# dmjovan/NeRF-Workspaces-Explorer

Hardware: AMD Instinct MI355X
Metric: ray-samples/sec (800x800, 192 samples, 8x256 MLP) (higher is better)
Workload: dtype f16x3 (split-fp16 MFMA, fp32 accumulate)

## Files before the change

include/nwe.h:

```cpp
#ifndef NWE_H
#define NWE_H

#include <stdint.h>

#ifdef __cplusplus
extern "C" {
#endif

typedef struct nwe_ctx nwe_ctx;

enum {
    NWE_OK = 0,
    NWE_ERR_INVALID = 1,
    NWE_ERR_UNSUPPORTED = 2,
    NWE_ERR_HIP = 3,
    NWE_ERR_STATE = 4
};

enum { NWE_NET_COARSE = 0, NWE_NET_FINE = 1 };

enum {
    NWE_PREC_F16X3 = 0,
    NWE_PREC_F16X1 = 1,
    NWE_PREC_F32 = 2
// ... 63 lines not shown
    float *raw;
    float *sigma;
    uint32_t *flags;
} nwe_point_outputs;

int nwe_query_points(nwe_ctx *ctx, int which, const float *points_dev, int64_t n_points, const float *dirs_dev,
                     int64_t points_per_dir, int precision, const nwe_point_outputs *out, void *stream);
float nwe_last_query_ms(nwe_ctx *ctx);
int nwe_debug_set_query_steps(nwe_ctx *ctx, int steps);

int nwe_to8b(nwe_ctx *ctx, const float *rgb_dev, uint8_t *out_dev, int64_t n, void *stream);

int64_t nwe_flops_per_eval(const nwe_ctx *ctx, int which);

float nwe_last_kernel_ms(nwe_ctx *ctx);

int nwe_last_launch_parts(nwe_ctx *ctx, float *ms2, int64_t *rays2);


int64_t nwe_packed_bytes(const nwe_ctx *ctx, int which);
int nwe_packed_copy(const nwe_ctx *ctx, int which, void *host_dst, int64_t bytes);
int64_t nwe_packed_bias_count(const nwe_ctx *ctx, int which);
int nwe_packed_bias_copy(const nwe_ctx *ctx, int which, float *host_dst, int64_t count);
float nwe_packed_scale(const nwe_ctx *ctx, int which);
int nwe_packed_colour_finite(const nwe_ctx *ctx, int which);

int nwe_debug_set_fine_depths(nwe_ctx *ctx, const float *z_dev);

int nwe_debug_set_raw(nwe_ctx *ctx, const float *raw_coarse_dev, const float *raw_fine_dev);
int nwe_debug_set_coarse_weights(nwe_ctx *ctx, const float *weights_dev);

int nwe_debug_set_fold(nwe_ctx *ctx, int on);

int nwe_set_white_background(nwe_ctx *ctx, int on);

int nwe_set_early_termination(nwe_ctx *ctx, float min_transmittance);
float nwe_get_early_termination(const nwe_ctx *ctx);

int nwe_set_shared_coarse(nwe_ctx *ctx, int k);
int nwe_get_shared_coarse(const nwe_ctx *ctx);

int nwe_set_separate_passes(nwe_ctx *ctx, int on);
int nwe_get_separate_passes(const nwe_ctx *ctx);

int nwe_set_occupancy(nwe_ctx *ctx, const float *lo, const float *hi, const int *res, const uint32_t *bits, int bits_on_device);
int nwe_clear_occupancy(nwe_ctx *ctx);
int nwe_get_occupancy(const nwe_ctx *ctx, float *lo, float *hi, int *res, float *inv, int64_t *occupied_cells);
int nwe_occupancy_copy(const nwe_ctx *ctx, uint32_t *host_words, int64_t n_words);
int nwe_build_occupancy(nwe_ctx *ctx, const float *lo, const float *hi, const int *res, int probes, float threshold, int dilate,
                        int precision, void *stream);

int nwe_set_coarse_grid(nwe_ctx *ctx, const float *lo, const float *hi, const int *res, const float *sigma, int on_device);
int nwe_clear_coarse_grid(nwe_ctx *ctx);
int nwe_get_coarse_grid(const nwe_ctx *ctx, float *lo, float *hi, int *res, float *inv);
int nwe_coarse_grid_copy(nwe_ctx *ctx, float *host_values, int64_t n_values);
int nwe_bake_coarse_grid(nwe_ctx *ctx, const float *lo, const float *hi, const int *res, int precision, void *stream);
int nwe_coarse_grid_weights(nwe_ctx *ctx, const float *c2w, int n_poses, int H, int W, float fx, float fy, float cx, float cy,
                            float near, float far, int row_begin, int row_end, float *sigma_out_dev, float *weights_out_dev,
                            void *stream);

typedef struct nwe_grid_outputs {
    uint64_t struct_bytes;
    float *rgb;
    float *depth;
    float *acc;
    float *weights_coarse;
    float *z_fine;
    float *raw_fine;
    uint32_t *flags;
} nwe_grid_outputs;
int nwe_set_radiance_grid(nwe_ctx *ctx, const float *lo, const float *hi, const int *res, const float *raw, int on_device);
int nwe_clear_radiance_grid(nwe_ctx *ctx);
int nwe_get_radiance_grid(const nwe_ctx *ctx, float *lo, float *hi, int *res, float *inv);
int nwe_radiance_grid_copy(nwe_ctx *ctx, float *host_values, int64_t n_values);
int nwe_bake_radiance_grid(nwe_ctx *ctx, const float *lo, const float *hi, const int *res, int which, const float *dir3_host,
                           int precision, void *stream);
int nwe_render_grid(nwe_ctx *ctx, const float *c2w, int n_poses, int H, int W, float fx, float fy, float cx, float cy, float near,
                    float far, int row_begin, int row_end, const nwe_grid_outputs *out, void *stream);
float nwe_last_grid_ms(nwe_ctx *ctx);

typedef struct nwe_sparse_outputs {
    uint64_t struct_bytes;
    float *rgb;
    float *depth;
    float *acc;
    float *weights_coarse;
    float *z_fine;
    float *weights_grid;
    uint8_t *selected;
    float *raw_fine;
    uint32_t *flags;
} nwe_sparse_outputs;
int nwe_render_sparse(nwe_ctx *ctx, const float *c2w, int n_poses, int H, int W, float fx, float fy, float cx, float cy, float near,
                      float far, int row_begin, int row_end, int which, int precision, float min_weight, int dilate,
                      const nwe_sparse_outputs *out, void *stream);
int nwe_debug_set_sparse_chunk(nwe_ctx *ctx, int rays);
float nwe_last_sparse_ms(nwe_ctx *ctx);
int nwe_last_sparse_samples(nwe_ctx *ctx, int64_t *out2);

int nwe_last_coarse_launch(nwe_ctx *ctx, float *ms, int64_t *rays);

int nwe_last_ray_evaluations(nwe_ctx *ctx, int64_t *out2);

int nwe_set_train_tables(nwe_ctx *ctx, const float *t_rand_dev, const float *noise_coarse_dev, const float *noise_fine_dev,
                         const float *u_sorted_dev);

int nwe_debug_set_decomposition(nwe_ctx *ctx, int mode);
int nwe_debug_last_plan(const nwe_ctx *ctx);

int nwe_debug_set_work_queue(nwe_ctx *ctx, int mode);
int nwe_debug_get_work_queue(const nwe_ctx *ctx);
int nwe_debug_get_work_queue_backfill(const nwe_ctx *ctx);
unsigned nwe_debug_queue_grid(unsigned items);
#define NWE_PLAN_HOOK_COARSE_WEIGHTS 1u
#define NWE_PLAN_HOOK_OTHER 2u
typedef struct nwe_plan_stage {
    int32_t active;
    int32_t role;
    int64_t n_rays;
    int32_t n_importance;
    int32_t net;
    int32_t variant;
    int32_t plan;
    int32_t n_launches;
    int32_t fork;
    int64_t ray_first[2], rays[2];
    int32_t split[2];
    uint32_t items[2], grid[2];
    int32_t tail;
    uint32_t tail_items;
} nwe_plan_stage;
typedef struct nwe_plan_report {
    uint64_t struct_bytes;
    int32_t separate, share, full;
    int32_t coarse_launch;
    int32_t may_queue, need_side;
    int32_t need_evals, coarse_flags;
    int32_t share_k, reserved;
    int64_t table_elems;
    int64_t evals_full, evals_run;
    int64_t share_rays;
    nwe_plan_stage coarse, main;
} nwe_plan_report;
int nwe_debug_plan(nwe_ctx *ctx, int n_poses, int H, int W, int row_begin, int row_end, int64_t n_rays, const nwe_outputs *out,
                   unsigned hooks, int precision, int cus, nwe_plan_report *report);
int nwe_debug_last_queue(nwe_ctx *ctx, unsigned *items2, unsigned *grid2, unsigned *taken2, int *side_stream);
int nwe_debug_get_work_queue_tail(const nwe_ctx *ctx);
int nwe_debug_last_tail(nwe_ctx *ctx, unsigned *stolen);
int nwe_debug_last_tail_rest(nwe_ctx *ctx, unsigned *rendered);

int nwe_debug_set_colour_skip(nwe_ctx *ctx, int mode);
int nwe_debug_get_colour_skip(const nwe_ctx *ctx);

int nwe_debug_set_packet_blocks(nwe_ctx *ctx, int on);
int nwe_debug_last_packet_blocks(const nwe_ctx *ctx);
int nwe_debug_packet_pixels(int64_t first, int64_t n, int W, int32_t *pixels);

int nwe_debug_set_stamps(nwe_ctx *ctx, unsigned long long *per_wave_dev);

int nwe_selftest(nwe_ctx *ctx, int32_t *report8);

#ifdef __cplusplus
}
#endif
#endif
```

nerf-workspaces-explorer_amd/_lib.py:

```python
from __future__ import annotations

import ctypes as C
import os

_HERE = os.path.dirname(os.path.abspath(__file__))
LIB_PATH = os.environ.get("NWE_LIB") or os.path.join(_HERE, "libnwe_hip.so")

NWE_OK, NWE_ERR_INVALID, NWE_ERR_UNSUPPORTED, NWE_ERR_HIP, NWE_ERR_STATE = 0, 1, 2, 3, 4
NET_COARSE, NET_FINE = 0, 1
PREC_F16X3, PREC_F16X1, PREC_F32 = 0, 1, 2
PRECISIONS = {"f16x3": PREC_F16X3, "f16x1": PREC_F16X1, "f32": PREC_F32}

OUTPUT_FIELDS = ("rgb", "depth", "acc", "disp", "z_std", "rgb_coarse", "depth_coarse", "acc_coarse", "disp_coarse",
                 "raw_coarse", "raw_fine", "z_fine", "weights_coarse", "sample_cond", "sample_amp", "sample_switch", "feat_map", "flags")

SYMBOLS = ("nwe_create", "nwe_destroy", "nwe_last_error", "nwe_set_network", "nwe_set_sampling", "nwe_render", "nwe_render_tiled",
           "nwe_create_rays", "nwe_render_rays", "nwe_to8b", "nwe_flops_per_eval", "nwe_last_kernel_ms", "nwe_packed_bytes",
           "nwe_packed_copy", "nwe_packed_bias_count", "nwe_packed_bias_copy", "nwe_packed_scale",
           "nwe_debug_set_fine_depths", "nwe_debug_set_raw", "nwe_debug_set_coarse_weights", "nwe_debug_set_fold", "nwe_set_train_tables", "nwe_set_white_background", "nwe_debug_set_decomposition", "nwe_debug_last_plan", "nwe_debug_set_stamps", "nwe_selftest",
           "nwe_last_warning", "nwe_debug_peer_access", "nwe_set_network_no_view_dirs", "nwe_last_launch_parts",
           "nwe_set_early_termination", "nwe_get_early_termination", "nwe_last_ray_evaluations",
           "nwe_set_shared_coarse", "nwe_get_shared_coarse", "nwe_last_coarse_launch",
           "nwe_set_separate_passes", "nwe_get_separate_passes",
           "nwe_debug_set_work_queue", "nwe_debug_get_work_queue", "nwe_debug_get_work_queue_backfill", "nwe_debug_queue_grid", "nwe_debug_last_queue",
           "nwe_debug_get_work_queue_tail", "nwe_debug_last_tail", "nwe_debug_last_tail_rest",
           "nwe_query_points", "nwe_last_query_ms", "nwe_debug_set_query_steps",
           "nwe_packed_colour_finite", "nwe_debug_set_colour_skip", "nwe_debug_get_colour_skip", "nwe_debug_plan",
           "nwe_set_occupancy", "nwe_clear_occupancy", "nwe_get_occupancy", "nwe_occupancy_copy", "nwe_build_occupancy",
           "nwe_set_coarse_grid", "nwe_clear_coarse_grid", "nwe_get_coarse_grid", "nwe_coarse_grid_copy", "nwe_bake_coarse_grid",
           "nwe_coarse_grid_weights",
           "nwe_set_radiance_grid", "nwe_clear_radiance_grid", "nwe_get_radiance_grid", "nwe_radiance_grid_copy", "nwe_bake_radiance_grid",
           "nwe_render_grid", "nwe_last_grid_ms",
           "nwe_render_sparse", "nwe_debug_set_sparse_chunk", "nwe_last_sparse_ms", "nwe_last_sparse_samples",
           "nwe_debug_set_packet_blocks", "nwe_debug_last_packet_blocks", "nwe_debug_packet_pixels")


class Outputs(C.Structure):
    _fields_ = [("struct_bytes", C.c_uint64)] + [(name, C.c_void_p) for name in OUTPUT_FIELDS]

    def __init__(self, **kw):
        super().__init__(struct_bytes=C.sizeof(Outputs), **kw)


POINT_OUTPUT_FIELDS = ("raw", "sigma", "flags")
NWE_FLAG_RAW = 1 << 8


class PointOutputs(C.Structure):
    _fields_ = [("struct_bytes", C.c_uint64)] + [(name, C.c_void_p) for name in POINT_OUTPUT_FIELDS]

    def __init__(self, **kw):
        super().__init__(struct_bytes=C.sizeof(PointOutputs), **kw)


GRID_OUTPUT_FIELDS = ("rgb", "depth", "acc", "weights_coarse", "z_fine", "raw_fine", "flags")


class GridOutputs(C.Structure):
    _fields_ = [("struct_bytes", C.c_uint64)] + [(name, C.c_void_p) for name in GRID_OUTPUT_FIELDS]

    def __init__(self, **kw):
        super().__init__(struct_bytes=C.sizeof(GridOutputs), **kw)


SPARSE_OUTPUT_FIELDS = ("rgb", "depth", "acc", "weights_coarse", "z_fine", "weights_grid", "selected", "raw_fine", "flags")


class SparseOutputs(C.Structure):
    _fields_ = [("struct_bytes", C.c_uint64)] + [(name, C.c_void_p) for name in SPARSE_OUTPUT_FIELDS]

    def __init__(self, **kw):
        super().__init__(struct_bytes=C.sizeof(SparseOutputs), **kw)


PLAN_HOOK_COARSE_WEIGHTS, PLAN_HOOK_OTHER = 1, 2


class PlanStage(C.Structure):
    _fields_ = [("active", C.c_int32), ("role", C.c_int32), ("n_rays", C.c_int64), ("n_importance", C.c_int32), ("net", C.c_int32),
                ("variant", C.c_int32), ("plan", C.c_int32), ("n_launches", C.c_int32), ("fork", C.c_int32),
                ("ray_first", C.c_int64 * 2), ("rays", C.c_int64 * 2), ("split", C.c_int32 * 2), ("items", C.c_uint32 * 2),
                ("grid", C.c_uint32 * 2), ("tail", C.c_int32), ("tail_items", C.c_uint32)]


class PlanReport(C.Structure):
    _fields_ = [("struct_bytes", C.c_uint64)] + [(name, C.c_int32) for name in (
        "separate", "share", "full", "coarse_launch", "may_queue", "need_side", "need_evals", "coarse_flags", "share_k", "reserved")] + [
        (name, C.c_int64) for name in ("table_elems", "evals_full", "evals_run", "share_rays")] + [("coarse", PlanStage), ("main", PlanStage)]

    def __init__(self):
        super().__init__(struct_bytes=C.sizeof(PlanReport))


_lib = None


def build_hint() -> str:
    return ("build it with `make -C nerf-workspaces-explorer_amd/csrc` (or `python -c 'import __graft_entry__ as g; "
            "g.build()'`); the render path has no CPU or torch fallback")


def load() -> C.CDLL:
    global _lib
    if _lib is not None:
        return _lib
    if not os.path.exists(LIB_PATH):
        raise RuntimeError(f"HIP extension {LIB_PATH} is missing: {build_hint()}")
    lib = C.CDLL(LIB_PATH)
    P, I, F, I64 = C.c_void_p, C.c_int, C.c_float, C.c_int64
    sig = {
        "nwe_create": (I, [C.POINTER(P), I]),
        "nwe_destroy": (None, [P]),
        "nwe_last_error": (C.c_char_p, [P]),
        "nwe_set_network": (I, [P, I, I, I, I, I, I, C.POINTER(P), C.POINTER(P)]),
        "nwe_set_network_no_view_dirs": (I, [P, I, I, I, I, I, I, C.POINTER(P), C.POINTER(P)]),
        "nwe_set_sampling": (I, [P, P, P, I, P, I]),
        "nwe_render": (I, [P, P, I, I, I, F, F, F, F, F, F, I, I, I, C.POINTER(Outputs), P]),
        "nwe_render_tiled": (I, [C.POINTER(P), I, P, I, I, I, F, F, F, F, F, F, I, P, P, P, P, P]),
        "nwe_create_rays": (I, [P, P, I, I, I, F, F, F, F, F, F, I, I, P, P]),
        "nwe_render_rays": (I, [P, P, I64, I, C.POINTER(Outputs), P]),
        "nwe_to8b": (I, [P, P, P, I64, P]),
        "nwe_flops_per_eval": (I64, [P, I]),
        "nwe_last_kernel_ms": (F, [P]),
        "nwe_last_launch_parts": (I, [P, C.POINTER(F), C.POINTER(I64)]),
        "nwe_packed_bytes": (I64, [P, I]),
        "nwe_packed_copy": (I, [P, I, P, I64]),
        "nwe_packed_bias_count": (I64, [P, I]),
        "nwe_packed_bias_copy": (I, [P, I, P, I64]),
        "nwe_packed_scale": (F, [P, I]),
        "nwe_debug_set_fine_depths": (I, [P, P]),
        "nwe_debug_set_raw": (I, [P, P, P]),
        "nwe_debug_set_coarse_weights": (I, [P, P]),
        "nwe_debug_set_fold": (I, [P, I]),
        "nwe_set_train_tables": (I, [P, P, P, P, P]),
        "nwe_set_white_background": (I, [P, I]),
        "nwe_debug_set_decomposition": (I, [P, I]),
        "nwe_debug_last_plan": (I, [P]),
        "nwe_debug_set_stamps": (I, [P, P]),
        "nwe_selftest": (I, [P, C.POINTER(C.c_int32)]),
        "nwe_last_warning": (C.c_char_p, [P]),
        "nwe_debug_peer_access": (I, [P, P]),
        "nwe_set_early_termination": (I, [P, F]),
        "nwe_get_early_termination": (F, [P]),
        "nwe_last_ray_evaluations": (I, [P, C.POINTER(I64)]),
        "nwe_set_shared_coarse": (I, [P, I]),
        "nwe_get_shared_coarse": (I, [P]),
        "nwe_last_coarse_launch": (I, [P, C.POINTER(F), C.POINTER(I64)]),
        "nwe_set_separate_passes": (I, [P, I]),
        "nwe_get_separate_passes": (I, [P]),
        "nwe_debug_set_work_queue": (I, [P, I]),
        "nwe_debug_get_work_queue": (I, [P]),
        "nwe_debug_get_work_queue_backfill": (I, [P]),
        "nwe_debug_queue_grid": (C.c_uint, [C.c_uint]),
        "nwe_debug_last_queue": (I, [P, C.POINTER(C.c_uint), C.POINTER(C.c_uint), C.POINTER(C.c_uint), C.POINTER(I)]),
        "nwe_debug_get_work_queue_tail": (I, [P]),
        "nwe_debug_last_tail": (I, [P, C.POINTER(C.c_uint)]),
        "nwe_debug_last_tail_rest": (I, [P, C.POINTER(C.c_uint)]),
        "nwe_query_points": (I, [P, I, P, I64, P, I64, I, C.POINTER(PointOutputs), P]),
        "nwe_last_query_ms": (F, [P]),
        "nwe_debug_set_query_steps": (I, [P, I]),
        "nwe_packed_colour_finite": (I, [P, I]),
        "nwe_debug_set_colour_skip": (I, [P, I]),
        "nwe_debug_get_colour_skip": (I, [P]),
        "nwe_debug_set_packet_blocks": (I, [P, I]),
        "nwe_debug_last_packet_blocks": (I, [P]),
        "nwe_debug_packet_pixels": (I, [I64, I64, I, P]),
        "nwe_debug_plan": (I, [P, I, I, I, I, I, I64, C.POINTER(Outputs), C.c_uint, I, I, C.POINTER(PlanReport)]),
        "nwe_set_occupancy": (I, [P, C.POINTER(F), C.POINTER(F), C.POINTER(I), P, I]),
        "nwe_clear_occupancy": (I, [P]),
        "nwe_get_occupancy": (I, [P, C.POINTER(F), C.POINTER(F), C.POINTER(I), C.POINTER(F), C.POINTER(I64)]),
        "nwe_occupancy_copy": (I, [P, P, I64]),
        "nwe_build_occupancy": (I, [P, C.POINTER(F), C.POINTER(F), C.POINTER(I), I, F, I, I, P]),
        "nwe_set_coarse_grid": (I, [P, C.POINTER(F), C.POINTER(F), C.POINTER(I), P, I]),
        "nwe_clear_coarse_grid": (I, [P]),
        "nwe_get_coarse_grid": (I, [P, C.POINTER(F), C.POINTER(F), C.POINTER(I), C.POINTER(F)]),
        "nwe_coarse_grid_copy": (I, [P, P, I64]),
        "nwe_bake_coarse_grid": (I, [P, C.POINTER(F), C.POINTER(F), C.POINTER(I), I, P]),
        "nwe_coarse_grid_weights": (I, [P, P, I, I, I, F, F, F, F, F, F, I, I, P, P, P]),
        "nwe_set_radiance_grid": (I, [P, C.POINTER(F), C.POINTER(F), C.POINTER(I), P, I]),
        "nwe_clear_radiance_grid": (I, [P]),
        "nwe_get_radiance_grid": (I, [P, C.POINTER(F), C.POINTER(F), C.POINTER(I), C.POINTER(F)]),
        "nwe_radiance_grid_copy": (I, [P, P, I64]),
        "nwe_bake_radiance_grid": (I, [P, C.POINTER(F), C.POINTER(F), C.POINTER(I), I, C.POINTER(F), I, P]),
        "nwe_render_grid": (I, [P, P, I, I, I, F, F, F, F, F, F, I, I, C.POINTER(GridOutputs), P]),
        "nwe_last_grid_ms": (F, [P]),
        "nwe_render_sparse": (I, [P, P, I, I, I, F, F, F, F, F, F, I, I, I, I, F, I, C.POINTER(SparseOutputs), P]),
        "nwe_debug_set_sparse_chunk": (I, [P, I]),
        "nwe_last_sparse_ms": (F, [P]),
        "nwe_last_sparse_samples": (I, [P, C.POINTER(I64)]),
    }
    for name, (res, args) in sig.items():
        fn = getattr(lib, name)
        fn.restype, fn.argtypes = res, args
    _lib = lib
    return lib
```

nerf-workspaces-explorer_amd/csrc/nwe_abi.hip:

```cpp
#include <algorithm>
#include <cmath>
#include <cstdlib>
#include <cstring>
#include <string>
#include <vector>

#include "nwe_check.h"
#include "nwe_host.h"
#include "nwe_pack.h"

using namespace nwe;

namespace {

template <class H, hipError_t (*Release)(H)>
struct Owned {
    H h = nullptr;
    Owned() = default;
    Owned(Owned&& o) noexcept : h(o.h) { o.h = nullptr; }
    ~Owned() { reset(); }
    void reset() { if (h) (void)Release(h); h = nullptr; }
    operator H() const { return h; }
};
using Event = Owned<hipEvent_t, hipEventDestroy>;
using Stream = Owned<hipStream_t, hipStreamDestroy>;

template <class T>
struct DevBuf {
    Owned<void*, hipFree> mem;
    size_t cap = 0;
    T* get() const { return static_cast<T*>(mem.h); }
    hipError_t reserve(size_t count) {
        if (count <= cap) return hipSuccess;
        mem.reset(); cap = 0;
        const hipError_t e = hipMalloc(&mem.h, count * sizeof(T));
        if (e == hipSuccess) cap = count; else mem.h = nullptr;
        return e;
    }
};

struct NetState : NetDesc {
    int64_t flops = 0;
    Packed p;
    NetF32 f32 = {};
    NetMfma mf = {};
    DevBuf<float> d_blob, d_bias;
    DevBuf<uint8_t> d_stream;
};

struct Slot {
    DevBuf<float> poses;
    Event ev0, ev1;
    bool used = false;
};

struct RenderSlot : Slot {
    Event ev_mid;
    bool has_mid = false;
    int64_t rays_first = 0, rays_total = 0;
    DevBuf<unsigned long long> evals;
    bool term = false;
    int64_t evals_full = 0;
    DevBuf<float> share_w;
    DevBuf<uint32_t> coarse_flags;
    Event ev_share;
    bool has_share = false;
    int64_t share_rays = 0, evals_run = 0;
    DevBuf<unsigned> queue;
    Stream side;
    Event ev_fork, ev_join;
    unsigned q_items[2] = {0, 0}, q_grid[2] = {0, 0};
    bool side_used = false;
    unsigned tail_items = 0;
};

struct GridBox {
    float lo[3] = {}, hi[3] = {}, inv[3] = {};
    int res[3] = {};
    int64_t cells = 0;
    GridBox() = default;
    GridBox(const float* lo_, const float* hi_, const int* res_) : cells((int64_t)res_[0] * res_[1] * res_[2]) {
        for (int i = 0; i < 3; ++i) {
            lo[i] = lo_[i]; hi[i] = hi_[i]; res[i] = res_[i];
            inv[i] = (float)res[i] / (hi[i] - lo[i]);
        }
    }
    void read(float* lo_, float* hi_, int* res_, float* inv_) const {
        for (int i = 0; i < 3; ++i) {
            if (lo_) lo_[i] = lo[i];
            if (hi_) hi_[i] = hi[i];
            if (res_) res_[i] = res[i];
            if (inv_) inv_[i] = inv[i];
        }
    }
};

struct Occupancy {
    bool set = false;
    GridBox box;
    int64_t occupied = 0;
    std::vector<uint32_t> bits;
};

struct CoarseGridState {
    bool set = false;
    GridBox box;
    std::vector<float> host;
};

using RadianceGridState = CoarseGridState;

thread_local std::string g_create_error;

}

struct nwe_ctx {
    int device = -1;
    bool host_only = false;
    int cus = 256;
    NetState net[2];
    DevBuf<float> d_t;
    int ns = 0, ni = 0;
    static constexpr int kSlots = 4;
    RenderSlot slots[kSlots];
    Slot rays_slot;
    int next_slot = 0, last_slot = -1;
    Slot query_slots[kSlots];
    int next_query = 0, last_query = -1;
    int query_steps = 0;
    Slot grid_slots[kSlots];
    int next_grid = 0, last_grid = -1;
    Slot sparse_slots[kSlots];
    int next_sparse = 0, last_sparse = -1;
    int64_t sparse_selected = 0, sparse_total = 0;
    int sparse_chunk = 0;
    DevBuf<uint8_t> d_sparse_scratch;
    Owned<void*, hipHostFree> sparse_word;
    const float* dbg_z_fine = nullptr;
    const float *dbg_raw_c = nullptr, *dbg_raw_f = nullptr, *dbg_w = nullptr;
    int fold = 1;
    DevBuf<float> tile_buf;
    DevBuf<uint32_t> tile_flags;
    Stream tile_stream;
    Event tile_done;
    Event frame_ready;
    DevBuf<uint32_t> flag_parts;
    int peer_access = -2;
    std::string warn;
    int white_bkgd = 0;
    float min_trans = 0.f;
    int share_k = 1;
    int separate = 0;
    Occupancy occ;
    DevBuf<uint32_t> d_occ_bits, d_occ_tmp;
    DevBuf<OccGrid> d_occ;
    DevBuf<float> d_occ_scratch;
    CoarseGridState cgrid;
    DevBuf<float> d_cgrid;
    RadianceGridState rgrid;
    DevBuf<float> d_rgrid;
    int decomposition = -1;
    int work_queue = -1;
    bool backfill = true;
    bool tail = true;
    int colour_skip = 1;
    int last_plan = -1;
    bool packet_blocks = true;
    int last_packet_blocks = 0;
    unsigned long long* stamps = nullptr;
    const float *trn_t = nullptr, *trn_nc = nullptr, *trn_nf = nullptr, *trn_u = nullptr;
    std::string err;
};

namespace {

int fail(nwe_ctx* c, int code, const std::string& msg) {
    if (c) c->err = msg; else g_create_error = msg;
    return code;
}

struct DeviceGuard {
    int prev = -1;
    DeviceGuard() { if (hipGetDevice(&prev) != hipSuccess) { prev = -1; (void)hipGetLastError(); } }
    ~DeviceGuard() { if (prev >= 0) (void)hipSetDevice(prev); }
    DeviceGuard(const DeviceGuard&) = delete;
    DeviceGuard& operator=(const DeviceGuard&) = delete;
};

#define HIPCHK(ctx, expr)                                                                                       \
    do {                                                                                                        \
        const hipError_t e_ = (expr);                                                                           \
        if (e_ != hipSuccess) return fail(ctx, NWE_ERR_HIP, std::string(#expr) + ": " + hipGetErrorString(e_)); \
    } while (0)
#define ON_DEVICE(c) DeviceGuard guard; HIPCHK(c, hipSetDevice(c->device))
#define TRY(call) do { const int rc_ = (call); if (rc_) return rc_; } while (0)
#define CHECK(c, check) do { const Refusal r_ = (check); if (r_) return fail(c, r_.code, r_.text); } while (0)

ContextDesc describe_context(const nwe_ctx* c) {
    ContextDesc d;
    for (int i = 0; i < 2; ++i) d.net[i] = c->net[i];
    d.ns = c->ns; d.ni = c->ni; d.host_only = c->host_only;
    d.min_trans = c->min_trans; d.share_k = c->share_k; d.separate = c->separate != 0;
    d.occ.set = c->occ.set; d.cgrid.set = c->cgrid.set; d.rgrid.set = c->rgrid.set;
    for (int i = 0; i < 3; ++i) { d.occ.res[i] = c->occ.box.res[i]; d.cgrid.res[i] = c->cgrid.box.res[i]; d.rgrid.res[i] = c->rgrid.box.res[i]; }
    d.stamps = c->stamps != nullptr;
    d.decomposition = c->decomposition; d.queue_mode = c->work_queue;
    d.backfill = c->backfill; d.tail = c->tail; d.packet_blocks = c->packet_blocks;
    return d;
}
struct MaybeContext {
    ContextDesc d;
    const ContextDesc* p = nullptr;
    explicit MaybeContext(const nwe_ctx* c) { if (c) { d = describe_context(c); p = &d; } }
};

__global__ void to8b_kernel(const float* __restrict__ x, uint8_t* __restrict__ y, int64_t n) {
    const int64_t i = (int64_t)blockIdx.x * blockDim.x + threadIdx.x;
    if (i < n) {
        const float v = 255.f * fminf(fmaxf(x[i], 0.f), 1.f);
        y[i] = (uint8_t)(int)v;
    }
}

__global__ void or_flags_kernel(const uint32_t* __restrict__ parts, int n, uint32_t* __restrict__ out) {
    uint32_t f = 0;
    for (int i = 0; i < n; ++i) f |= parts[i];
    if (f) atomicOr(out, f);
}

__global__ void or_masked_flags_kernel(const uint32_t* __restrict__ word, uint32_t mask, uint32_t* __restrict__ out) {
    const uint32_t f = *word & mask;
    if (f) atomicOr(out, f);
}

__global__ void create_rays_kernel(RenderArgs a, float* __restrict__ out) {
    const int64_t i = (int64_t)blockIdx.x * blockDim.x + threadIdx.x;
    if (i >= a.n_rays) return;
    const Ray r = load_ray(a, i);
    float* o = out + i * 11;
    o[0] = r.ox; o[1] = r.oy; o[2] = r.oz; o[3] = r.dx; o[4] = r.dy; o[5] = r.dz;
    o[6] = r.near; o[7] = r.far; o[8] = r.vx; o[9] = r.vy; o[10] = r.vz;
}

int prepare_slot(nwe_ctx* c, Slot& s) {
    if (!s.ev0)
        for (Event* e : {&s.ev0, &s.ev1}) HIPCHK(c, hipEventCreate(&e->h));
    if (s.used) HIPCHK(c, hipEventSynchronize(s.ev1));
    s.used = false;
    return NWE_OK;
}
int prepare_slot(nwe_ctx* c, RenderSlot& s) {
    if (!s.ev_mid)
        for (Event* e : {&s.ev_mid, &s.ev_share}) HIPCHK(c, hipEventCreate(&e->h));
    s.has_mid = s.has_share = false;
    return prepare_slot(c, static_cast<Slot&>(s));
}

template <class Queue>
int record_launch(nwe_ctx* c, Slot& s, hipStream_t stream, Queue&& queue) {
    HIPCHK(c, hipEventRecord(s.ev0, stream));
    TRY(queue());
    HIPCHK(c, hipGetLastError());
    HIPCHK(c, hipEventRecord(s.ev1, stream));
    s.used = true;
    return NWE_OK;
}

int wait_for_launches(nwe_ctx* c) {
    for (RenderSlot& s : c->slots)
        if (s.used) HIPCHK(c, hipEventSynchronize(s.ev1));
    if (c->rays_slot.used) HIPCHK(c, hipEventSynchronize(c->rays_slot.ev1));
    for (Slot& s : c->query_slots)
        if (s.used) HIPCHK(c, hipEventSynchronize(s.ev1));
    for (Slot& s : c->grid_slots)
        if (s.used) HIPCHK(c, hipEventSynchronize(s.ev1));
    for (Slot& s : c->sparse_slots)
        if (s.used) HIPCHK(c, hipEventSynchronize(s.ev1));
    return NWE_OK;
}

struct HookReset {
    nwe_ctx* c;
    ~HookReset() {
        if (!c) return;
        c->dbg_z_fine = c->dbg_raw_c = c->dbg_raw_f = c->dbg_w = nullptr;
        c->trn_t = c->trn_nc = c->trn_nf = c->trn_u = nullptr;
    }
};

int upload_poses(nwe_ctx* c, Slot& s, const float* c2w, int n_poses, hipStream_t stream) {
    HIPCHK(c, s.poses.reserve((size_t)std::max(n_poses, 64) * 16));
    HIPCHK(c, hipMemcpyAsync(s.poses.get(), c2w, (size_t)n_poses * 16 * sizeof(float), hipMemcpyHostToDevice, stream));
    return NWE_OK;
}

RenderArgs camera_args(const Camera& m, const float* poses_dev) {
    RenderArgs a = {};
    a.poses = poses_dev;
    a.H = m.H; a.W = m.W; a.row_begin = m.row_begin; a.rows = m.row_end - m.row_begin;
    a.n_rays = (int64_t)m.n_poses * a.rows * m.W;
    a.fx = m.fx; a.fy = m.fy; a.cx = m.cx; a.cy = m.cy; a.near = m.near; a.far = m.far;
    return a;
}

#ifdef NWE_STAMPS
constexpr bool kStampedBuild = true;
#else
constexpr bool kStampedBuild = false;
#endif

void context_args(const nwe_ctx* ctx, RenderArgs& a) {
    a.white_bkgd = ctx->white_bkgd;
    a.t_vals = ctx->d_t.get();
    if (a.t_vals) { a.omt_vals = a.t_vals + kMaxSamples; a.u_vals = a.omt_vals + kMaxSamples; }
    a.n_samples = ctx->ns; a.n_importance = ctx->ni;
    a.stamps = ctx->stamps;
    a.min_trans = ctx->min_trans;
}

CallDesc describe_call(const ContextDesc& ctx, const RenderArgs& a, int precision) {
    CallDesc d;
    d.n_rays = a.n_rays;
    RenderArgs consumer = a;
    consumer.share = kShareConsumer | ctx.share_k << 8;
    d.n_rep = share_n_rep(consumer, share_grid(consumer));
    d.n_samples = a.n_samples; d.n_importance = a.n_importance;
    d.mfma = precision != NWE_PREC_F32;
    d.term = a.min_trans > 0.f;
    d.occ = ctx.occ.set;
    d.share_k = ctx.share_k; d.separate = ctx.separate;
    d.baked = ctx.cgrid.set;
    RenderArgs unstamped = a;
    unstamped.stamps = nullptr;
    d.lean = mfma_is_lean(unstamped); d.stamps = a.stamps != nullptr; d.stamped_build = kStampedBuild;
    d.w_in = a.w_in != nullptr;
    d.want_weights_coarse = a.out.weights_coarse != nullptr; d.want_flags = a.out.flags != nullptr;
    for (int i = 0; i < 2; ++i)
        for (int v = 0; v < kVariants; ++v) d.built[i][v] = ctx.net[i].set && ctx.net[i].mfma_ok && ctx.net[i].built[v];
    d.decomposition = ctx.decomposition; d.queue_mode = ctx.queue_mode;
    d.backfill = ctx.backfill; d.tail = ctx.tail;
    if (!a.rays) { d.rows = a.rows; d.width = a.W; }
    d.packet_blocks = ctx.packet_blocks;
    return d;
}

int provide(nwe_ctx* ctx, RenderSlot& slot, const CallPlan& p, hipStream_t stream) {
    if (p.need_evals) {
        HIPCHK(ctx, slot.evals.reserve(1));
        HIPCHK(ctx, hipMemsetAsync(slot.evals.get(), 0, sizeof(unsigned long long), stream));
    }
    HIPCHK(ctx, slot.share_w.reserve((size_t)p.table_elems));
    if (p.coarse_flags) {
        HIPCHK(ctx, slot.coarse_flags.reserve(1));
        HIPCHK(ctx, hipMemsetAsync(slot.coarse_flags.get(), 0, sizeof(uint32_t), stream));
    }
    if (p.may_queue) HIPCHK(ctx, slot.queue.reserve(4));
    for (RenderSlot& s : ctx->slots) {
        if (!p.need_side || s.side) continue;
        int least = 0, greatest = 0;
        HIPCHK(ctx, hipDeviceGetStreamPriorityRange(&least, &greatest));
        HIPCHK(ctx, hipStreamCreateWithPriority(&s.side.h, hipStreamNonBlocking, least));
        for (Event* e : {&s.ev_fork, &s.ev_join}) HIPCHK(ctx, hipEventCreateWithFlags(&e->h, hipEventDisableTiming));
    }
    return NWE_OK;
}

RenderArgs stage_args(const CallPlan& p, const RenderSlot& slot, RenderArgs& a) {
    RenderArgs prod = {};
    if (p.need_evals) a.evals = slot.evals.get();
    if (p.main.role != kShareOff) a.share = p.main.role | p.share_k << 8;
    if (p.share) a.share_w = slot.share_w.get();
    if (p.coarse.active) {
        prod = a;
        prod.share = p.coarse.role | p.share_k << 8; prod.n_rays = p.coarse.n_rays; prod.n_importance = p.coarse.n_importance;
        prod.out = {};
        if (p.share) {
            if (p.share_k == 1) prod.out.flags = a.out.flags;
        } else {
            float* table = a.out.weights_coarse ? a.out.weights_coarse : slot.share_w.get();
            prod.z_fine_in = prod.raw_in_f = prod.noise_f = prod.u_rand = nullptr;
            prod.out.struct_bytes = a.out.struct_bytes;
            prod.out.raw_coarse = a.out.raw_coarse; prod.out.weights_coarse = table;
            prod.out.rgb_coarse = a.out.rgb_coarse; prod.out.depth_coarse = a.out.depth_coarse;
            prod.out.acc_coarse = a.out.acc_coarse; prod.out.disp_coarse = a.out.disp_coarse;
            if (p.coarse_flags) prod.out.flags = slot.coarse_flags.get();
            a.w_in = table;
        }
    }
    if (p.full) {
        a.raw_in_c = a.noise_c = nullptr;
        a.out.raw_coarse = a.out.weights_coarse = a.out.rgb_coarse = a.out.depth_coarse = a.out.acc_coarse = a.out.disp_coarse = nullptr;
    }
    return prod;
}

CoarseGrid coarse_grid_args(const nwe_ctx* ctx) {
    CoarseGrid g = {};
    const GridBox& box = ctx->cgrid.box;
    for (int i = 0; i < 3; ++i) { g.lo[i] = box.lo[i]; g.inv[i] = box.inv[i]; g.res[i] = box.res[i]; }
    g.sigma = ctx->d_cgrid.get();
    return g;
}

int launch(nwe_ctx* ctx, const ContextDesc& desc, RenderSlot& slot, RenderArgs& a, int precision, hipStream_t stream) {
    context_args(ctx, a);
    if (a.n_rays <= 0) return NWE_OK;
    const CallPlan p = plan_call(describe_call(desc, a, precision), ctx->cus);
    const bool mfma = precision != NWE_PREC_F32, three_pass = precision == NWE_PREC_F16X3;
    TRY(provide(ctx, slot, p, stream));
    const RenderArgs prod = stage_args(p, slot, a);
    if (p.occ) a.occ = ctx->d_occ.get();
    if (p.blocks) a.ray_cols |= kPacketBlocksBit;
    ctx->last_packet_blocks = p.blocks ? 1 : 0;
    const NetState &nc = ctx->net[0], &nf = ctx->net[ctx->ni > 0 ? 1 : 0];
    const auto with_skip = [&](const NetState& n) {
        NetMfma m = n.mf;
        m.colour_skip = ctx->colour_skip == 2 || (ctx->colour_skip == 1 && n.p.colour_finite) ? 1 : 0;
        return m;
    };
    const NetMfma mf[2] = {with_skip(nc), with_skip(nf)};
    const auto run = [&](const StagePlan& s, const RenderArgs& args, const LaunchResources& res, LaunchReport* report) {
        if (!mfma) {
            if (p.occ) launch_render_f32_occ(args, nc.f32, nf.f32, stream); else launch_render_f32(args, nc.f32, nf.f32, stream);
            return true;
        }
        return launch_render_mfma(args, mf[s.net < 0 ? 0 : s.net], mf[s.net < 0 ? 1 : s.net], three_pass, s.pass, res, stream, report);
    };
    const int rc = record_launch(ctx, slot, stream, [&]() -> int {
        const PassPlan& pass = p.main.pass;
        slot.has_mid = false; slot.rays_total = a.n_rays;
        slot.rays_first = mfma ? pass.launch[0].rays : a.n_rays;
        for (int i = 0; i < 2; ++i) { slot.q_grid[i] = pass.launch[i].grid; slot.q_items[i] = pass.launch[i].grid ? pass.launch[i].items : 0; }
        slot.side_used = false; slot.tail_items = pass.tail_items;
        slot.term = p.need_evals;
        slot.evals_full = p.evals_full; slot.evals_run = p.evals_run; slot.share_rays = p.share_rays;
        const char* shapes_differ = "coarse and fine networks must have the same shape for the MFMA kernel";
        LaunchReport report;
        if (p.baked) {
            launch_coarse_grid_weights(a, coarse_grid_args(ctx), slot.share_w.get(), nullptr, nullptr, stream);
            HIPCHK(ctx, hipEventRecord(slot.ev_share, stream));
            slot.has_share = true;
        } else if (p.coarse.active) {
            if (!run(p.coarse, prod, LaunchResources{}, &report)) return fail(ctx, NWE_ERR_UNSUPPORTED, shapes_differ);
            if (p.full && prod.out.flags)
                hipLaunchKernelGGL(or_masked_flags_kernel, dim3(1), dim3(1), 0, stream, prod.out.flags,
                                   ~(uint32_t)(NWE_FLAG_RGB | NWE_FLAG_DEPTH | NWE_FLAG_ACC | NWE_FLAG_DISP), a.out.flags);
            HIPCHK(ctx, hipEventRecord(slot.ev_share, stream));
            slot.has_share = true;
        }
        LaunchResources res;
        res.mid = slot.ev_mid;
        if (p.may_queue) {
            HIPCHK(ctx, hipMemsetAsync(slot.queue.get(), 0, 4 * sizeof(unsigned), stream));
            res.counters = slot.queue.get();
            res.side = slot.side; res.fork = slot.ev_fork; res.join = slot.ev_join;
        }
        report = {};
        if (!run(p.main, a, res, &report)) {
            if (!report.side_used) return fail(ctx, NWE_ERR_UNSUPPORTED, shapes_differ);
            (void)hipStreamSynchronize(slot.side);
            return fail(ctx, NWE_ERR_HIP, std::string("work queue: joining the side stream: ") + hipGetErrorString(hipGetLastError()));
        }
        if (mfma) ctx->last_plan = pass.plan;
        slot.side_used = report.side_used; slot.has_mid = report.mid_recorded;
        return NWE_OK;
    });
    if (rc) return rc;
    ctx->last_slot = (int)(&slot - ctx->slots);
    ctx->next_slot = (ctx->last_slot + 1) % nwe_ctx::kSlots;
    return NWE_OK;
}

int render_rows(nwe_ctx* c, const Camera& m, int precision, const nwe_outputs* out, hipStream_t stream) {
    const MaybeContext desc(c);
    CHECK(c, check_ready(desc.p, out, precision, true));
    CHECK(c, check_camera(m));
    ON_DEVICE(c);
    RenderSlot& slot = c->slots[c->next_slot];
    TRY(prepare_slot(c, slot));
    TRY(upload_poses(c, slot, m.c2w, m.n_poses, stream));
    RenderArgs a = camera_args(m, slot.poses.get());
    CHECK(c, check_ray_count(a.n_rays, false));
    a.out = *out;
    return launch(c, desc.d, slot, a, precision, stream);
}

int can_access_peer(int from, int to, hipError_t* err = nullptr) {
    int can = 0;
    const hipError_t e = hipDeviceCanAccessPeer(&can, from, to);
    if (err) *err = e;
    if (e != hipSuccess) { (void)hipGetLastError(); return -1; }
    return can ? 1 : 0;
}


int tile_resources(nwe_ctx* c, size_t floats) {
    if (!c->tile_stream) {
        HIPCHK(c, hipStreamCreateWithFlags(&c->tile_stream.h, hipStreamNonBlocking));
        HIPCHK(c, hipEventCreateWithFlags(&c->tile_done.h, hipEventDisableTiming));
        HIPCHK(c, c->tile_flags.reserve(1));
    }
    if (c->tile_buf.cap < floats) HIPCHK(c, hipStreamSynchronize(c->tile_stream));
    HIPCHK(c, c->tile_buf.reserve(floats));
    return NWE_OK;
}

void probe_peer_access(nwe_ctx* c, nwe_ctx* c0, int i) {
    if (c->peer_access != -2) return;
    c->peer_access = 1;
    if (c->device == c0->device) return;
    hipError_t e = hipSuccess;
    const int can = can_access_peer(c->device, c0->device, &e);
    if (can == 1) {
        e = hipDeviceEnablePeerAccess(c0->device, 0);
        if (e == hipErrorPeerAccessAlreadyEnabled) { (void)hipGetLastError(); e = hipSuccess; }
    }
    const std::string tile = "tile " + std::to_string(i) + ": ", from = std::to_string(c->device), to = std::to_string(c0->device);
    if (e != hipSuccess) {
        (void)hipGetLastError();
        c->peer_access = -1;
        c0->warn += tile + "peer access device " + from + " -> " + to + " not enabled (" + hipGetErrorString(e) + "), copies are staged; ";
    } else if (can == 0) {
        c->peer_access = 0;
        c0->warn += tile + "device " + from + " cannot access device " + to + " directly, copies are staged; ";
    }
}

struct Frame { float *rgb, *depth, *acc; };

struct RecordOnExit {
    nwe_ctx* c;
    ~RecordOnExit() { if (c->tile_done && c->tile_stream && hipEventRecord(c->tile_done, c->tile_stream) != hipSuccess) (void)hipGetLastError(); }
};

int queue_tile(nwe_ctx* c, nwe_ctx* c0, int i, const Camera& m, int precision, const Frame& f) {
    HIPCHK(c, hipSetDevice(c->device));
    RecordOnExit record_on_exit{c};
    const size_t px = (size_t)(m.row_end - m.row_begin) * m.W;
    TRY(tile_resources(c, (size_t)m.n_poses * px * 5));
    probe_peer_access(c, c0, i);
    HIPCHK(c, hipStreamWaitEvent(c->tile_stream, c0->frame_ready, 0));
    if (px == 0) return NWE_OK;
    HIPCHK(c, hipMemsetAsync(c->tile_flags.get(), 0, sizeof(uint32_t), c->tile_stream));
    float* t_rgb = c->tile_buf.get();
    float* t_depth = t_rgb + (size_t)m.n_poses * px * 3;
    float* t_acc = t_depth + (size_t)m.n_poses * px;
    nwe_outputs o = {};
    o.struct_bytes = sizeof(nwe_outputs);
    o.rgb = f.rgb ? t_rgb : nullptr; o.depth = f.depth ? t_depth : nullptr; o.acc = f.acc ? t_acc : nullptr;
    o.flags = c->tile_flags.get();
    TRY(render_rows(c, m, precision, &o, c->tile_stream));
    auto copy = [&](void* dst, const void* src, size_t bytes) { return hipMemcpyPeerAsync(dst, c0->device, src, c->device, bytes, c->tile_stream); };
    for (int p = 0; p < m.n_poses; ++p) {
        const size_t dst_px = ((size_t)p * m.H + m.row_begin) * m.W, src_px = (size_t)p * px;
        if (f.rgb) HIPCHK(c, copy(f.rgb + dst_px * 3, t_rgb + src_px * 3, px * 3 * sizeof(float)));
        if (f.depth) HIPCHK(c, copy(f.depth + dst_px, t_depth + src_px, px * sizeof(float)));
        if (f.acc) HIPCHK(c, copy(f.acc + dst_px, t_acc + src_px, px * sizeof(float)));
    }
    HIPCHK(c, copy(c0->flag_parts.get() + i, c->tile_flags.get(), sizeof(uint32_t)));
    return NWE_OK;
}

template <class T>
int upload(nwe_ctx* c, DevBuf<T>& dst, const std::vector<T>& src) {
    HIPCHK(c, dst.reserve(src.size()));
    HIPCHK(c, hipMemcpy(dst.get(), src.data(), src.size() * sizeof(T), hipMemcpyHostToDevice));
    return NWE_OK;
}

int set_network(nwe_ctx* c, int which, const NetShape& shape, const float* const* w, const float* const* b) {
    NetState& n = c->net[which];
    n.set = false;
    static_cast<NetShape&>(n) = shape;
    if (n.skip < -1 || n.skip >= n.D - 1) n.skip = -1;
    n.flops = algo_flops(n);
    pack_f32(n.p, n, w, b);
    n.f32 = n.p.f32;
    n.form = n.in_dir == 0 ? kFormNoViewDirs : (c->fold != 0 ? kFormFolded : kFormReference);
    n.mfma_ok = mfma_supported(n.D, n.W, n.in_xyz, n.in_dir, n.skip, n.form);
    for (int v = 0; v < kVariants; ++v) n.built[v] = mfma_variant_built(n.D, n.W, n.skip, n.form, v);
    if (n.mfma_ok) pack_mfma(n.p, n, n.form, w, b); else { n.p.stream.clear(); n.p.bias_tab.clear(); n.p.n_chunks = 0; }
    n.mf = {};
    n.mf.D = n.D; n.mf.W = n.W; n.mf.skip = n.skip; n.mf.form = n.form;
    n.mf.n_tiles = (int)(n.p.stream.size() / kTileBytes);
    n.mf.n_chunks = n.mfma_ok ? n.p.n_chunks : 0;
    n.mf.inv_scale = 1.f / n.p.w_scale;
    if (!c->host_only) {
        ON_DEVICE(c);
        TRY(wait_for_launches(c));
        TRY(upload(c, n.d_blob, n.p.blob));
        if (n.mfma_ok) {
            TRY(upload(c, n.d_stream, n.p.stream));
            TRY(upload(c, n.d_bias, n.p.bias_tab));
        }
        n.f32.blob = n.d_blob.get();
        n.mf.stream = n.mfma_ok ? n.d_stream.get() : nullptr;
        n.mf.bias = n.mfma_ok ? n.d_bias.get() : nullptr;
    }
    n.set = true;
    c->occ.set = false;
    if (which == NWE_NET_COARSE) c->cgrid = CoarseGridState{};
    c->rgrid = RadianceGridState{};
    return NWE_OK;
}

const NetState* set_net(const nwe_ctx* c, int which) { return c && which >= 0 && which <= 1 && c->net[which].set ? &c->net[which] : nullptr; }

template <class T>
int copy_out(const std::vector<T>* v, void* host_dst, int64_t count) {
    if (!v || !host_dst || count != (int64_t)v->size()) return NWE_ERR_INVALID;
    std::memcpy(host_dst, v->data(), (size_t)count * sizeof(T));
    return NWE_OK;
}

template <class Set>
int set_on(nwe_ctx* c, Set&& set) { if (!c) return NWE_ERR_INVALID; set(); return NWE_OK; }

constexpr float kMinPartMs = 1e-5f;

const RenderSlot* last_render(const nwe_ctx* c) { return c->host_only || c->last_slot < 0 || !c->slots[c->last_slot].used ? nullptr : &c->slots[c->last_slot]; }


int64_t occ_words(int64_t cells) { return (cells + 31) / 32; }

int install_occupancy(nwe_ctx* c, const GridBox& box, std::vector<uint32_t>&& words) {
    Occupancy g;
    g.box = box;
    if (box.cells & 31) words.back() &= (1u << (box.cells & 31)) - 1u;
    for (const uint32_t w : words) g.occupied += __builtin_popcount(w);
    g.bits = std::move(words);
    if (!c->host_only) {
        c->occ.set = false;
        HIPCHK(c, c->d_occ_bits.reserve(g.bits.size()));
        HIPCHK(c, c->d_occ.reserve(1));
        HIPCHK(c, hipMemcpy(c->d_occ_bits.get(), g.bits.data(), g.bits.size() * sizeof(uint32_t), hipMemcpyHostToDevice));
        OccGrid d = {};
        for (int i = 0; i < 3; ++i) { d.lo[i] = box.lo[i]; d.inv[i] = box.inv[i]; d.res[i] = box.res[i]; }
        d.bits = c->d_occ_bits.get();
        HIPCHK(c, hipMemcpy(c->d_occ.get(), &d, sizeof(d), hipMemcpyHostToDevice));
    }
    g.set = true;
    c->occ = std::move(g);
    return NWE_OK;
}


void install_grid(CoarseGridState& slot, const GridBox& box, std::vector<float>&& host) {
    CoarseGridState g;
    g.box = box;
    g.host = std::move(host);
    g.set = true;
    slot = std::move(g);
}
void install_coarse_grid(nwe_ctx* c, const GridBox& box, std::vector<float>&& host) { install_grid(c->cgrid, box, std::move(host)); }

int set_values_grid(nwe_ctx* c, CoarseGridState& slot, DevBuf<float>& dev, const GridBox& box, int per_cell, const float* values, bool on_device) {
    const size_t count = (size_t)box.cells * per_cell;
    if (c->host_only) {
        install_grid(slot, box, std::vector<float>(values, values + count));
        return NWE_OK;
    }
    ON_DEVICE(c);
    TRY(wait_for_launches(c));
    slot = CoarseGridState{};
    HIPCHK(c, dev.reserve(count));
    HIPCHK(c, hipMemcpy(dev.get(), values, count * sizeof(float), on_device ? hipMemcpyDeviceToDevice : hipMemcpyHostToDevice));
    install_grid(slot, box, {});
    return NWE_OK;
}
int clear_values_grid(nwe_ctx* c, CoarseGridState& slot) {
    if (!c->host_only && slot.set) {
        ON_DEVICE(c);
        TRY(wait_for_launches(c));
    }
    slot = CoarseGridState{};
    return NWE_OK;
}
int copy_values_grid(nwe_ctx* c, const CoarseGridState& slot, const DevBuf<float>& dev, float* host_values, int64_t n_values) {
    if (c->host_only) return copy_out(&slot.host, host_values, n_values);
    ON_DEVICE(c);
    HIPCHK(c, hipMemcpy(host_values, dev.get(), (size_t)n_values * sizeof(float), hipMemcpyDeviceToHost));
    return NWE_OK;
}

RadianceGrid radiance_grid_args(const nwe_ctx* ctx) {
    RadianceGrid g = {};
    const GridBox& box = ctx->rgrid.box;
    for (int i = 0; i < 3; ++i) { g.lo[i] = box.lo[i]; g.inv[i] = box.inv[i]; g.res[i] = box.res[i]; }
    g.rows = reinterpret_cast<const float4*>(ctx->d_rgrid.get());
    return g;
}


struct Lattice {
    OccBuild b;
    int per_cell;
    int chunk_cells;
};

Lattice probe_lattice(const GridBox& box, int probes) {
    Lattice l = {};
    for (int i = 0; i < 3; ++i) {
        l.b.lo[i] = box.lo[i]; l.b.res[i] = box.res[i];
        l.b.step[i] = (float)(((double)box.hi[i] - (double)box.lo[i]) / (double)box.res[i]);
    }
    l.b.probes = probes;
    l.per_cell = probes * probes * probes;
    l.chunk_cells = (int)std::min<int64_t>(box.cells, std::max(1, (1 << 20) / l.per_cell));
    return l;
}

template <class SigmaOf, class Done>
int query_lattice(nwe_ctx* c, const NetState& n, const Lattice& l, int64_t cells, float* points, int precision, hipStream_t stream,
                  SigmaOf&& sigma_of, Done&& done) {
    for (int64_t first = 0; first < cells; first += l.chunk_cells) {
        const int count = (int)std::min<int64_t>(l.chunk_cells, cells - first);
        launch_occ_probe_points(l.b, first, count, points, stream);
        QueryArgs q = {};
        q.points = points; q.sigma = sigma_of(first); q.n_points = count * l.per_cell; q.points_per_dir = 1; q.density_only = 1;
        if (precision == NWE_PREC_F32) launch_query_f32(q, n.f32, c->query_steps, c->cus, stream);
        else if (!launch_query_mfma(q, n.mf, precision == NWE_PREC_F16X3, c->query_steps, c->cus, stream))
            return fail(c, NWE_ERR_UNSUPPORTED, "no MFMA query kernel in this build for this network shape; use NWE_PREC_F32");
        done(q.sigma, first, count);
    }
    return NWE_OK;
}

float elapsed_ms(nwe_ctx* c, const Slot& s, const char* who) {
    DeviceGuard guard;
    hipError_t e = hipSetDevice(c->device);
    if (e == hipSuccess) e = hipEventSynchronize(s.ev1);
    float ms = -1.f;
    if (e == hipSuccess) e = hipEventElapsedTime(&ms, s.ev0, s.ev1);
    if (e != hipSuccess) { c->err = std::string(who) + ": " + hipGetErrorString(e); (void)hipGetLastError(); return -1.f; }
    return ms;
}

int env_switch(const char* name) {
    const char* e = std::getenv(name);
    return e && (e[0] == '0' || e[0] == '1') && !e[1] ? e[0] - '0' : -1;
}

}

extern "C" {

int nwe_create(nwe_ctx** out, int device) {
    if (!out) return fail(nullptr, NWE_ERR_INVALID, "out is null");
    nwe_ctx* c = new nwe_ctx();
    c->device = device;
    c->host_only = device < 0;
    if (const int v = env_switch("NWE_WORK_QUEUE"); v >= 0) c->work_queue = v;
    if (env_switch("NWE_WORK_QUEUE_BACKFILL") == 0) c->backfill = false;
    if (const int v = env_switch("NWE_WORK_QUEUE_TAIL"); v >= 0) c->tail = v == 1;
    if (const int v = env_switch("NWE_COLOUR_SKIP"); v >= 0) c->colour_skip = v;
    if (const int v = env_switch("NWE_PACKET_BLOCKS"); v >= 0) c->packet_blocks = v == 1;
    if (!c->host_only) {
        const hipError_t e = hipSetDevice(device);
        if (e != hipSuccess) { delete c; return fail(nullptr, NWE_ERR_HIP, std::string("nwe_create: ") + hipGetErrorString(e)); }
        int cus = 0;
        if (hipDeviceGetAttribute(&cus, hipDeviceAttributeMultiprocessorCount, device) == hipSuccess && cus > 0) c->cus = cus;
        else (void)hipGetLastError();
    }
    *out = c;
    return NWE_OK;
}

void nwe_destroy(nwe_ctx* c) {
    if (!c) return;
    if (c->host_only) { delete c; return; }
    DeviceGuard guard;
    (void)hipSetDevice(c->device);
    (void)wait_for_launches(c);
    if (c->tile_stream) (void)hipStreamSynchronize(c->tile_stream);
    delete c;
}

const char* nwe_last_error(const nwe_ctx* c) { return c ? c->err.c_str() : g_create_error.c_str(); }

int nwe_set_network(nwe_ctx* c, int which, int depth, int width, int in_xyz, int in_dir, int skip_layer,
                    const float* const* w, const float* const* b) {
    CHECK(c, check_network(!c || !w || !b, which, depth, width, in_xyz, in_dir, 0, true, w, b));
    return set_network(c, which, NetShape{depth, width, in_xyz, in_dir, skip_layer, 0}, w, b);
}

int nwe_set_network_no_view_dirs(nwe_ctx* c, int which, int depth, int width, int in_xyz, int skip_layer, int output_ch,
                                 const float* const* w, const float* const* b) {
    CHECK(c, check_network(!c || !w || !b, which, depth, width, in_xyz, 0, output_ch, false, w, b));
    return set_network(c, which, NetShape{depth, width, in_xyz, 0, skip_layer, output_ch}, w, b);
}

int nwe_set_sampling(nwe_ctx* c, const float* t_vals, const float* one_minus_t, int n_samples, const float* u,
                     int n_importance) {
    CHECK(c, check_sampling(!c, t_vals, one_minus_t, n_samples, u, n_importance));
    c->ns = n_samples; c->ni = n_importance;
    if (c->host_only) return NWE_OK;
    ON_DEVICE(c);
    HIPCHK(c, c->d_t.reserve(2 * kMaxSamples + kMaxImportance));
    TRY(wait_for_launches(c));
    float* d_t = c->d_t.get();
    HIPCHK(c, hipMemcpy(d_t, t_vals, n_samples * sizeof(float), hipMemcpyHostToDevice));
    HIPCHK(c, hipMemcpy(d_t + kMaxSamples, one_minus_t, n_samples * sizeof(float), hipMemcpyHostToDevice));
    if (n_importance > 0) HIPCHK(c, hipMemcpy(d_t + 2 * kMaxSamples, u, n_importance * sizeof(float), hipMemcpyHostToDevice));
    return NWE_OK;
}

int nwe_render(nwe_ctx* c, const float* c2w, int n_poses, int H, int W, float fx, float fy, float cx, float cy, float near,
               float far, int row_begin, int row_end, int precision, const nwe_outputs* out, void* stream) {
    return render_rows(c, Camera{c2w, n_poses, H, W, fx, fy, cx, cy, near, far, row_begin, row_end}, precision, out, (hipStream_t)stream);
}

int nwe_render_tiled(nwe_ctx* const* ctxs, int n_ctx, const float* c2w, int n_poses, int H, int W, float fx, float fy, float cx,
                     float cy, float near, float far, int precision, float* rgb_dev, float* depth_dev, float* acc_dev,
                     uint32_t* flags_dev, void* stream_) {
    if (!ctxs || n_ctx < 1 || !ctxs[0]) return fail(nullptr, NWE_ERR_INVALID, "nwe_render_tiled: no contexts");
    nwe_ctx* c0 = ctxs[0];
    for (int i = 0; i < n_ctx; ++i)
        if (!ctxs[i] || ctxs[i]->host_only) return fail(c0, NWE_ERR_INVALID, "nwe_render_tiled: null or host-only context");
    Camera m{c2w, n_poses, H, W, fx, fy, cx, cy, near, far, 0, H};
    CHECK(c0, check_camera(m, kCameraOfTiled));
    m.row_end = 0;
    hipStream_t stream0 = (hipStream_t)stream_;
    DeviceGuard guard;
    c0->warn.clear();
    HIPCHK(c0, hipSetDevice(c0->device));
    if (!c0->frame_ready) HIPCHK(c0, hipEventCreateWithFlags(&c0->frame_ready.h, hipEventDisableTiming));
    HIPCHK(c0, c0->flag_parts.reserve(n_ctx));
    HIPCHK(c0, hipMemsetAsync(c0->flag_parts.get(), 0, (size_t)n_ctx * sizeof(uint32_t), stream0));
    HIPCHK(c0, hipEventRecord(c0->frame_ready, stream0));
    const int base = H / n_ctx, extra = H % n_ctx;
    int rc_all = NWE_OK;
    for (int i = 0; i < n_ctx && rc_all == NWE_OK; ++i) {
        m.row_begin = m.row_end;
        m.row_end += base + (i < extra ? 1 : 0);
        rc_all = queue_tile(ctxs[i], c0, i, m, precision, Frame{rgb_dev, depth_dev, acc_dev});
        if (rc_all != NWE_OK && ctxs[i] != c0) c0->err = "tile " + std::to_string(i) + ": " + ctxs[i]->err;
    }
    (void)hipSetDevice(c0->device);
    for (int i = 0; i < n_ctx; ++i)
        if (ctxs[i]->tile_done) (void)hipStreamWaitEvent(stream0, ctxs[i]->tile_done, 0);
    if (rc_all != NWE_OK) return rc_all;
    if (flags_dev) {
        hipLaunchKernelGGL(or_flags_kernel, dim3(1), dim3(1), 0, stream0, c0->flag_parts.get(), n_ctx, flags_dev);
        HIPCHK(c0, hipGetLastError());
    }
    return NWE_OK;
}

int nwe_create_rays(nwe_ctx* c, const float* c2w, int n_poses, int H, int W, float fx, float fy, float cx, float cy, float near,
                    float far, int row_begin, int row_end, float* rays_out_dev, void* stream_) {
    CHECK(c, check_on_device(c && !c->host_only));
    const Camera m{c2w, n_poses, H, W, fx, fy, cx, cy, near, far, row_begin, row_end};
    if (!rays_out_dev) return fail(c, NWE_ERR_INVALID, "bad pose / image / row range");
    CHECK(c, check_camera(m, kCameraOfCreateRays));
    hipStream_t stream = (hipStream_t)stream_;
    ON_DEVICE(c);
    Slot& slot = c->rays_slot;
    TRY(prepare_slot(c, slot));
    TRY(upload_poses(c, slot, c2w, n_poses, stream));
    const RenderArgs a = camera_args(m, slot.poses.get());
    if (a.n_rays == 0) return NWE_OK;
    return record_launch(c, slot, stream, [&]() -> int {
        hipLaunchKernelGGL(create_rays_kernel, dim3((unsigned)((a.n_rays + 255) / 256)), dim3(256), 0, stream, a, rays_out_dev);
        return NWE_OK;
    });
}

int nwe_query_points(nwe_ctx* c, int which, const float* points_dev, int64_t n_points, const float* dirs_dev, int64_t points_per_dir,
                     int precision, const nwe_point_outputs* out, void* stream_) {
    CHECK(c, check_query(MaybeContext(c).p, which, points_dev, n_points, dirs_dev, points_per_dir, precision, out));
    const NetState& net = c->net[which];
    if (n_points == 0) return NWE_OK;
    hipStream_t stream = (hipStream_t)stream_;
    ON_DEVICE(c);
    Slot& slot = c->query_slots[c->next_query];
    TRY(prepare_slot(c, slot));
    QueryArgs a = {};
    a.points = points_dev; a.dirs = dirs_dev; a.raw = out->raw; a.sigma = out->sigma; a.flags = out->flags;
    a.n_points = (int)n_points;
    a.points_per_dir = (int)std::min(points_per_dir, n_points);
    a.density_only = out->raw ? 0 : 1;
    TRY(record_launch(c, slot, stream, [&]() -> int {
        if (precision == NWE_PREC_F32) launch_query_f32(a, net.f32, c->query_steps, c->cus, stream);
        else if (!launch_query_mfma(a, net.mf, precision == NWE_PREC_F16X3, c->query_steps, c->cus, stream))
            return fail(c, NWE_ERR_UNSUPPORTED, "no MFMA query kernel in this build for this network shape; use NWE_PREC_F32");
        return NWE_OK;
    }));
    c->last_query = (int)(&slot - c->query_slots);
    c->next_query = (c->last_query + 1) % nwe_ctx::kSlots;
    return NWE_OK;
}

float nwe_last_query_ms(nwe_ctx* c) {
    if (!c || c->host_only || c->last_query < 0 || !c->query_slots[c->last_query].used) return -1.f;
    return elapsed_ms(c, c->query_slots[c->last_query], "nwe_last_query_ms");
}

int nwe_debug_set_query_steps(nwe_ctx* c, int steps) { return set_on(steps < 0 || steps > kQueryMaxSteps ? nullptr : c, [&] { c->query_steps = steps; }); }

int nwe_render_rays(nwe_ctx* c, const float* rays_dev, int64_t n_rays, int precision, const nwe_outputs* out, void* stream) {
    HookReset hooks{c};
    const MaybeContext desc(c);
    CHECK(c, check_ready(desc.p, out, precision, false));
    CHECK(c, check_ray_count(n_rays, true, !rays_dev));
    if (n_rays == 0) return NWE_OK;
    ON_DEVICE(c);
    RenderSlot& slot = c->slots[c->next_slot];
    TRY(prepare_slot(c, slot));
    RenderArgs a = {};
    a.rays = rays_dev; a.n_rays = n_rays; a.W = 1; a.rows = 1;
    a.ray_cols = c->net[0].in_dir == 0 ? 8 : 11;
    a.z_fine_in = c->dbg_z_fine; a.raw_in_c = c->dbg_raw_c; a.raw_in_f = c->dbg_raw_f; a.w_in = c->dbg_w;
    a.t_rand = c->trn_t; a.noise_c = c->trn_nc; a.noise_f = c->trn_nf; a.u_rand = c->trn_u;
    a.out = *out;
    return launch(c, desc.d, slot, a, precision, (hipStream_t)stream);
}

int nwe_to8b(nwe_ctx* c, const float* rgb_dev, uint8_t* out_dev, int64_t n, void* stream) {
    if (!c || c->host_only || !rgb_dev || !out_dev || n < 0) return fail(c, NWE_ERR_INVALID, "bad argument");
    if (n == 0) return NWE_OK;
    ON_DEVICE(c);
    hipLaunchKernelGGL(to8b_kernel, dim3((unsigned)((n + 255) / 256)), dim3(256), 0, (hipStream_t)stream, rgb_dev, out_dev, n);
    HIPCHK(c, hipGetLastError());
    return NWE_OK;
}

float nwe_last_kernel_ms(nwe_ctx* c) {
    const RenderSlot* s = c ? last_render(c) : nullptr;
    return s ? elapsed_ms(c, *s, "nwe_last_kernel_ms") : -1.f;
}

int nwe_last_launch_parts(nwe_ctx* c, float* ms2, int64_t* rays2) {
    if (!c || !ms2 || !rays2) return NWE_ERR_INVALID;
    ms2[0] = ms2[1] = -1.f; rays2[0] = rays2[1] = 0;
    const RenderSlot* s = last_render(c);
    if (!s) return fail(c, NWE_ERR_STATE, "nothing has been launched");
    ON_DEVICE(c);
    HIPCHK(c, hipEventSynchronize(s->ev1));
    rays2[0] = s->rays_first; rays2[1] = s->rays_total - s->rays_first;
    const hipEvent_t begin = s->has_share ? s->ev_share : s->ev0;
    if (s->has_mid) {
        HIPCHK(c, hipEventElapsedTime(&ms2[0], begin, s->ev_mid));
        HIPCHK(c, hipEventElapsedTime(&ms2[1], s->ev_mid, s->ev1));
        for (int i = 0; i < 2; ++i) ms2[i] = std::max(ms2[i], kMinPartMs);
    } else {
        HIPCHK(c, hipEventElapsedTime(&ms2[0], begin, s->ev1));
    }
    return NWE_OK;
}

int nwe_last_coarse_launch(nwe_ctx* c, float* ms, int64_t* rays) {
    if (!c || !ms || !rays) return NWE_ERR_INVALID;
    *ms = -1.f; *rays = 0;
    const RenderSlot* s = last_render(c);
    if (!s) return fail(c, NWE_ERR_STATE, "nothing has been launched");
    if (!s->has_share) return NWE_OK;
    ON_DEVICE(c);
    HIPCHK(c, hipEventSynchronize(s->ev1));
    HIPCHK(c, hipEventElapsedTime(ms, s->ev0, s->ev_share));
    *rays = s->share_rays;
    return NWE_OK;
}

int nwe_last_ray_evaluations(nwe_ctx* c, int64_t* out2) {
    if (!c || !out2) return NWE_ERR_INVALID;
    out2[0] = out2[1] = 0;
    const RenderSlot* s = last_render(c);
    if (!s) return fail(c, NWE_ERR_STATE, "nothing has been launched");
    ON_DEVICE(c);
    HIPCHK(c, hipEventSynchronize(s->ev1));
    out2[0] = s->evals_run; out2[1] = s->evals_full;
    if (s->term) {
        unsigned long long ran = 0;
        HIPCHK(c, hipMemcpy(&ran, s->evals.get(), sizeof(ran), hipMemcpyDeviceToHost));
        out2[0] = (int64_t)ran;
    }
    return NWE_OK;
}

int64_t nwe_flops_per_eval(const nwe_ctx* c, int which) { const NetState* n = set_net(c, which); return n ? n->flops : 0; }
int64_t nwe_packed_bytes(const nwe_ctx* c, int which) { const NetState* n = set_net(c, which); return n ? (int64_t)n->p.stream.size() : 0; }
int64_t nwe_packed_bias_count(const nwe_ctx* c, int which) { const NetState* n = set_net(c, which); return n ? (int64_t)n->p.bias_tab.size() : 0; }
float nwe_packed_scale(const nwe_ctx* c, int which) { const NetState* n = set_net(c, which); return n ? n->p.w_scale : 0.f; }
int nwe_packed_colour_finite(const nwe_ctx* c, int which) { const NetState* n = set_net(c, which); return n ? (n->p.colour_finite ? 1 : 0) : -1; }

int nwe_packed_copy(const nwe_ctx* c, int which, void* host_dst, int64_t bytes) { const NetState* n = set_net(c, which); return copy_out(n ? &n->p.stream : nullptr, host_dst, bytes); }
int nwe_packed_bias_copy(const nwe_ctx* c, int which, float* host_dst, int64_t count) { const NetState* n = set_net(c, which); return copy_out(n ? &n->p.bias_tab : nullptr, host_dst, count); }

int nwe_debug_set_fine_depths(nwe_ctx* c, const float* z_dev) { return set_on(c, [&] { c->dbg_z_fine = z_dev; }); }
int nwe_debug_set_raw(nwe_ctx* c, const float* raw_coarse_dev, const float* raw_fine_dev) { return set_on(c, [&] { c->dbg_raw_c = raw_coarse_dev; c->dbg_raw_f = raw_fine_dev; }); }
int nwe_debug_set_coarse_weights(nwe_ctx* c, const float* weights_dev) { return set_on(c, [&] { c->dbg_w = weights_dev; }); }
int nwe_debug_set_fold(nwe_ctx* c, int on) { return set_on(c, [&] { c->fold = on ? 1 : 0; }); }
int nwe_debug_set_decomposition(nwe_ctx* c, int mode) { return set_on(mode < -1 || mode > 2 ? nullptr : c, [&] { c->decomposition = mode; }); }
int nwe_debug_set_work_queue(nwe_ctx* c, int mode) { return set_on(mode < -1 || mode > 1 ? nullptr : c, [&] { c->work_queue = mode; }); }
int nwe_debug_get_work_queue(const nwe_ctx* c) { return c ? c->work_queue : -2; }
int nwe_debug_set_colour_skip(nwe_ctx* c, int mode) { return set_on(mode < 0 || mode > 2 ? nullptr : c, [&] { c->colour_skip = mode; }); }
int nwe_debug_get_colour_skip(const nwe_ctx* c) { return c ? c->colour_skip : -1; }
int nwe_debug_set_packet_blocks(nwe_ctx* c, int on) { return set_on(on < 0 || on > 1 ? nullptr : c, [&] { c->packet_blocks = on != 0; }); }
int nwe_debug_last_packet_blocks(const nwe_ctx* c) { return c ? c->last_packet_blocks : -1; }
int nwe_debug_packet_pixels(int64_t first, int64_t n, int W, int32_t* pixels) {
    if (first < 0 || n < 0 || first + n > INT32_MAX || W < 1 || W > (INT32_MAX / kBlockH) || (n > 0 && !pixels)) return NWE_ERR_INVALID;
    for (int64_t i = 0; i < n; ++i) pixels[i] = packet_block_pixel((int)(first + i), W);
    return NWE_OK;
}
int nwe_debug_get_work_queue_backfill(const nwe_ctx* c) { return c ? (c->backfill ? 1 : 0) : -1; }
unsigned nwe_debug_queue_grid(unsigned items) { return queue_grid(items); }
int nwe_debug_plan(nwe_ctx* c, int n_poses, int H, int W, int row_begin, int row_end, int64_t n_rays, const nwe_outputs* out,
                   unsigned hooks, int precision, int cus, nwe_plan_report* report) {
    const bool pinhole = n_rays < 0;
    const MaybeContext desc(c);
    CHECK(c, check_ready(desc.p, out, precision, pinhole, true));
    if (!report || report->struct_bytes != sizeof(nwe_plan_report))
        return fail(c, NWE_ERR_INVALID, "nwe_plan_report.struct_bytes != sizeof(nwe_plan_report): the caller was built against another version of include/nwe.h");
    if (cus < 1) return fail(c, NWE_ERR_INVALID, "cus must be at least 1");
    *report = {};
    report->struct_bytes = sizeof(nwe_plan_report);
    static const float somewhere = 0.f;
    RenderArgs a = {};
    if (pinhole) {
        const Camera m{&somewhere, n_poses, H, W, 1.f, 1.f, 0.f, 0.f, 0.f, 0.f, row_begin, row_end};
        CHECK(c, check_camera(m));
        a = camera_args(m, &somewhere);
    } else {
        a.rays = &somewhere; a.n_rays = n_rays; a.W = 1; a.rows = 1;
        if (hooks & NWE_PLAN_HOOK_COARSE_WEIGHTS) a.w_in = &somewhere;
        if (hooks & NWE_PLAN_HOOK_OTHER) a.z_fine_in = &somewhere;
    }
    CHECK(c, check_ray_count(a.n_rays, !pinhole));
    a.out = *out;
    context_args(c, a);
    if (a.n_rays <= 0) return NWE_OK;
    const CallPlan p = plan_call(describe_call(desc.d, a, precision), cus);
    c->last_packet_blocks = p.blocks ? 1 : 0;
    report->separate = p.separate; report->share = p.share; report->full = p.full; report->coarse_launch = p.coarse_launch;
    report->may_queue = p.may_queue; report->need_side = p.need_side; report->need_evals = p.need_evals;
    report->coarse_flags = p.coarse_flags; report->share_k = p.share_k;
    report->table_elems = p.table_elems; report->evals_full = p.evals_full; report->evals_run = p.evals_run; report->share_rays = p.share_rays;
    const StagePlan* stages[2] = {&p.coarse, &p.main};
    for (int i = 0; i < 2; ++i) {
        const StagePlan& s = *stages[i];
        nwe_plan_stage& r = i == 0 ? report->coarse : report->main;
        if (!s.active) continue;
        r.active = 1; r.role = s.role; r.n_rays = s.n_rays; r.n_importance = s.n_importance; r.net = s.net;
        if (p.baked && i == 0) {
            r.variant = r.plan = -1; r.n_launches = 1;
            continue;
        }
        if (precision == NWE_PREC_F32) continue;
        const NetState &nc = c->net[0], &nf = c->net[1];
        if (!s.pass.ok || (s.net < 0 && s.n_importance > 0 && (nf.D != nc.D || nf.W != nc.W || nf.skip != nc.skip || nf.form != nc.form)))
            return fail(c, NWE_ERR_UNSUPPORTED, "coarse and fine networks must have the same shape for the MFMA kernel");
        r.variant = s.pass.variant; r.plan = s.pass.plan; r.n_launches = s.pass.n_launches;
        for (int l = 0; l < 2; ++l) {
            const LaunchPlan& q = s.pass.launch[l];
            r.ray_first[l] = q.ray_first; r.rays[l] = q.rays; r.split[l] = q.split; r.items[l] = q.items; r.grid[l] = q.grid;
        }
        r.fork = s.pass.fork; r.tail = s.pass.tail; r.tail_items = s.pass.tail_items;
    }
    return NWE_OK;
}
int nwe_debug_last_queue(nwe_ctx* c, unsigned* items2, unsigned* grid2, unsigned* taken2, int* side_stream) {
    if (!c || !items2 || !grid2 || !taken2) return NWE_ERR_INVALID;
    for (int i = 0; i < 2; ++i) items2[i] = grid2[i] = taken2[i] = 0;
    if (side_stream) *side_stream = 0;
    const RenderSlot* s = last_render(c);
    if (!s) return fail(c, NWE_ERR_STATE, "nothing has been launched");
    ON_DEVICE(c);
    HIPCHK(c, hipEventSynchronize(s->ev1));
    unsigned taken[2] = {0, 0};
    if (s->q_grid[0] || s->q_grid[1]) HIPCHK(c, hipMemcpy(taken, s->queue.get(), sizeof(taken), hipMemcpyDeviceToHost));
    for (int i = 0; i < 2; ++i) { items2[i] = s->q_items[i]; grid2[i] = s->q_grid[i]; taken2[i] = s->q_grid[i] ? taken[i] : 0; }
    if (side_stream) *side_stream = s->side_used ? 1 : 0;
    return NWE_OK;
}
int nwe_debug_get_work_queue_tail(const nwe_ctx* c) { return c ? (c->tail ? 1 : 0) : -1; }
static int last_tail(nwe_ctx* c, unsigned* out, int which) {
    if (!c || !out) return NWE_ERR_INVALID;
    *out = 0;
    const RenderSlot* s = last_render(c);
    if (!s) return fail(c, NWE_ERR_STATE, "nothing has been launched");
    if (!s->tail_items) return NWE_OK;
    ON_DEVICE(c);
    HIPCHK(c, hipEventSynchronize(s->ev1));
    unsigned word = 0;
    HIPCHK(c, hipMemcpy(&word, s->queue.get() + 2 + which, sizeof(word), hipMemcpyDeviceToHost));
    *out = which == 0 ? std::min(word, s->tail_items) : word;
    return NWE_OK;
}
int nwe_debug_last_tail(nwe_ctx* c, unsigned* stolen) { return last_tail(c, stolen, 0); }
int nwe_debug_last_tail_rest(nwe_ctx* c, unsigned* rendered) { return last_tail(c, rendered, 1); }
int nwe_debug_set_stamps(nwe_ctx* c, unsigned long long* per_wave_dev) { return set_on(c, [&] { c->stamps = per_wave_dev; }); }
int nwe_set_white_background(nwe_ctx* c, int on) { return set_on(c, [&] { c->white_bkgd = on ? 1 : 0; }); }
int nwe_set_early_termination(nwe_ctx* c, float min_transmittance) {
    if (!c) return NWE_ERR_INVALID;
    CHECK(c, check_early_termination(min_transmittance));
    c->min_trans = min_transmittance > 0.f ? min_transmittance : 0.f;
    return NWE_OK;
}
float nwe_get_early_termination(const nwe_ctx* c) { return c ? c->min_trans : -1.f; }
int nwe_set_shared_coarse(nwe_ctx* c, int k) {
    if (!c) return NWE_ERR_INVALID;
    CHECK(c, check_shared_coarse(k));
    c->share_k = k;
    return NWE_OK;
}
int nwe_get_shared_coarse(const nwe_ctx* c) { return c ? c->share_k : -1; }
int nwe_set_separate_passes(nwe_ctx* c, int on) {
    if (!c) return NWE_ERR_INVALID;
    CHECK(c, check_separate_passes(on));
    c->separate = on;
    return NWE_OK;
}
int nwe_get_separate_passes(const nwe_ctx* c) { return c ? c->separate : -1; }
int nwe_set_occupancy(nwe_ctx* c, const float* lo, const float* hi, const int* res, const uint32_t* bits, int bits_on_device) {
    if (!c) return NWE_ERR_INVALID;
    CHECK(c, check_set_grid(kOccupancyGrid, lo, hi, res, bits, bits_on_device != 0, c->host_only));
    const GridBox box(lo, hi, res);
    std::vector<uint32_t> words((size_t)occ_words(box.cells));
    if (c->host_only) {
        std::memcpy(words.data(), bits, words.size() * sizeof(uint32_t));
        return install_occupancy(c, box, std::move(words));
    }
    ON_DEVICE(c);
    TRY(wait_for_launches(c));
    if (bits_on_device) HIPCHK(c, hipMemcpy(words.data(), bits, words.size() * sizeof(uint32_t), hipMemcpyDeviceToHost));
    else std::memcpy(words.data(), bits, words.size() * sizeof(uint32_t));
    return install_occupancy(c, box, std::move(words));
}

int nwe_clear_occupancy(nwe_ctx* c) {
    if (!c) return NWE_ERR_INVALID;
    if (!c->host_only && c->occ.set) {
        ON_DEVICE(c);
        TRY(wait_for_launches(c));
    }
    c->occ = Occupancy{};
    return NWE_OK;
}

int nwe_get_occupancy(const nwe_ctx* c, float* lo, float* hi, int* res, float* inv, int64_t* occupied_cells) {
    if (!c) return NWE_ERR_INVALID;
    if (!c->occ.set) return NWE_ERR_STATE;
    c->occ.box.read(lo, hi, res, inv);
    if (occupied_cells) *occupied_cells = c->occ.occupied;
    return NWE_OK;
}

int nwe_occupancy_copy(const nwe_ctx* c, uint32_t* host_words, int64_t n_words) {
    if (!c) return NWE_ERR_INVALID;
    if (!c->occ.set) return NWE_ERR_STATE;
    return copy_out(&c->occ.bits, host_words, n_words);
}

int nwe_build_occupancy(nwe_ctx* c, const float* lo, const float* hi, const int* res, int probes, float threshold, int dilate,
                        int precision, void* stream_) {
    CHECK(c, check_build_occupancy(MaybeContext(c).p, lo, hi, res, probes, threshold, dilate, precision));
    hipStream_t stream = (hipStream_t)stream_;
    ON_DEVICE(c);
    TRY(wait_for_launches(c));
    const GridBox box(lo, hi, res);
    const Lattice l = probe_lattice(box, probes);
    const int64_t words = occ_words(box.cells);
    HIPCHK(c, c->d_occ_scratch.reserve((size_t)l.chunk_cells * l.per_cell * 4));
    HIPCHK(c, c->d_occ_tmp.reserve((size_t)words * 2));
    float* points = c->d_occ_scratch.get();
    float* sigma = points + (size_t)l.chunk_cells * l.per_cell * 3;
    uint32_t* buf[2] = {c->d_occ_tmp.get(), c->d_occ_tmp.get() + words};
    HIPCHK(c, hipMemsetAsync(buf[0], 0, (size_t)words * sizeof(uint32_t), stream));
    for (const NetState& n : c->net)
        if (n.set)
            TRY(query_lattice(c, n, l, box.cells, points, precision, stream, [&](int64_t) { return sigma; }, [&](const float* s, int64_t first, int count) {
                launch_occ_reduce_bits(s, first, count, l.per_cell, threshold, buf[0], stream);
            }));
    int cur = 0;
    for (int d = 0; d < dilate; ++d, cur ^= 1)
        launch_occ_dilate(buf[cur], buf[cur ^ 1], res, stream);
    HIPCHK(c, hipGetLastError());
    std::vector<uint32_t> host((size_t)words);
    HIPCHK(c, hipMemcpyAsync(host.data(), buf[cur], (size_t)words * sizeof(uint32_t), hipMemcpyDeviceToHost, stream));
    HIPCHK(c, hipStreamSynchronize(stream));
    return install_occupancy(c, box, std::move(host));
}

int nwe_set_coarse_grid(nwe_ctx* c, const float* lo, const float* hi, const int* res, const float* sigma, int on_device) {
    if (!c) return NWE_ERR_INVALID;
    CHECK(c, check_set_grid(kCoarseGrid, lo, hi, res, sigma, on_device != 0, c->host_only));
// ... 262 lines not shown
```

nerf-workspaces-explorer_amd/csrc/nwe_check.h:

```cpp
#pragma once
#include <stdint.h>
#include <string>

#include "../../include/nwe.h"
#include "nwe_pack.h"
#include "nwe_plan.h"

namespace nwe {

struct Refusal {
    int code = NWE_OK;
    std::string text;
    explicit operator bool() const { return code != NWE_OK; }
};


struct NetDesc : NetShape {
    bool set = false;
    int form = kFormFolded;
    bool mfma_ok = false;
    bool built[kVariants] = {};
};

struct GridDesc {
    bool set = false;
    int res[3] = {};
};

struct ContextDesc {
    NetDesc net[2];
    int ns = 0, ni = 0;
    bool host_only = false;
    float min_trans = 0.f;
    int share_k = 1;
    bool separate = false;
    GridDesc occ, cgrid;
    GridDesc rgrid;
    bool stamps = false;
    int decomposition = -1, queue_mode = -1;
    bool backfill = true, tail = true, packet_blocks = true;
};


Refusal check_ready(const ContextDesc* d, const nwe_outputs* out, int precision, bool pinhole, bool planning = false);

struct Camera { const float* c2w; int n_poses, H, W; float fx, fy, cx, cy, near, far; int row_begin, row_end; };
enum CameraOf { kCameraOfRender, kCameraOfTiled, kCameraOfCreateRays };
Refusal check_camera(const Camera& m, CameraOf entry = kCameraOfRender);

Refusal check_ray_count(int64_t n_rays, bool ray_list, bool null_rays = false);

Refusal check_precision(int precision);
Refusal no_mfma_kernel();
Refusal check_on_device(bool have_device);


Refusal check_network(bool null_args, int which, int depth, int width, int in_xyz, int in_dir, int output_ch, bool view_dirs,
                      const float* const* w, const float* const* b);
Refusal check_sampling(bool null_ctx, const float* t_vals, const float* one_minus_t, int n_samples, const float* u, int n_importance);
Refusal check_early_termination(float min_transmittance);
Refusal check_shared_coarse(int k);
Refusal check_separate_passes(int on);

Refusal check_query(const ContextDesc* d, int which, const float* points, int64_t n_points, const float* dirs, int64_t points_per_dir,
                    int precision, const nwe_point_outputs* out);


struct GridKind {
    const char* word;
    int max_res;
    bool finite_inv;
    const char* values;
    const char* from_host;
};
extern const GridKind kOccupancyGrid, kCoarseGrid, kRadianceGrid;

Refusal check_grid_box(const GridKind& kind, const float* lo, const float* hi, const int* res);
Refusal check_set_grid(const GridKind& kind, const float* lo, const float* hi, const int* res, const void* values, bool on_device, bool host_only);
Refusal check_build_occupancy(const ContextDesc* d, const float* lo, const float* hi, const int* res, int probes, float threshold, int dilate,
                              int precision);
Refusal check_bake_coarse_grid(const ContextDesc* d, const float* lo, const float* hi, const int* res, int precision);
Refusal check_bake_radiance_grid(const ContextDesc* d, const float* lo, const float* hi, const int* res, int which, const float* dir3,
                                 int precision);
Refusal check_render_grid(const ContextDesc* d, const nwe_grid_outputs* out, const Camera& m);
Refusal check_render_sparse(const ContextDesc* d, const nwe_sparse_outputs* out, const Camera& m, int which, int precision, float min_weight,
                            int dilate);
constexpr int kSparseMaxDilate = 8;

}
```

nerf-workspaces-explorer_amd/csrc/nwe_device.h:

```cpp
#pragma once
#include <hip/hip_runtime.h>
#include <stdint.h>

#include "../../include/nwe.h"
#include "nwe_plan.h"

namespace nwe {

struct OccGrid {
    float lo[3], inv[3];
    int res[3];
    int pad;
    const uint32_t* bits;
};

struct RenderArgs {
    const float* rays;
    int ray_cols;
    unsigned queue_items;
    const float* poses;
    int64_t n_rays;
    int64_t ray_first;
    int H, W, row_begin, rows;
    float fx, fy, cx, cy, near, far;
    const float* t_vals;
    const float* omt_vals;
    const float* u_vals;
    const float* z_fine_in;
    const float* raw_in_c;
    const float* raw_in_f;
    union {
        const float* w_in;
        unsigned* tail;
    };
    const float* t_rand;
    const float* noise_c;
    const float* noise_f;
    const float* u_rand;
    int white_bkgd;
    int n_samples, n_importance;
    union {
        unsigned long long* stamps;
        const OccGrid* occ;
    };
    nwe_outputs out;
    float min_trans;
    int share;
    union {
        unsigned long long* evals;
        float* share_w;
        unsigned* queue;
    };
};
static_assert(sizeof(RenderArgs) == 360, "RenderArgs must not grow: every kernel's argument offsets and scalar loads depend on it");

constexpr int kStampWords = 14;

__host__ __device__ inline int share_role(const RenderArgs& a) { return a.share & 0xff; }

struct ShareGrid { int k, br0, nbr, nbc; };
__host__ __device__ inline ShareGrid share_grid(const RenderArgs& a) {
    ShareGrid g;
    g.k = a.share >> 8;
    g.br0 = a.row_begin / g.k;
    g.nbr = (a.row_begin + a.rows - 1) / g.k - g.br0 + 1;
    g.nbc = (a.W + g.k - 1) / g.k;
    return g;
}
__host__ __device__ inline int share_n_rep(const RenderArgs& a, const ShareGrid& g) {
    return share_role(a) == kShareProducer ? (int)a.n_rays : (int)(a.n_rays / ((int64_t)a.rows * a.W)) * g.nbr * g.nbc;
}

struct Ray {
    float ox, oy, oz, dx, dy, dz, near, far, vx, vy, vz, dnorm;
};

__device__ __forceinline__ float norm3(float x, float y, float z) {
    return __builtin_sqrtf(__fmaf_rn(z, z, __fmaf_rn(y, y, __fmul_rn(x, x))));
}

struct RaySeed {
    int pose;
    float x, y;
};

__device__ __forceinline__ RaySeed seed_ray(const RenderArgs& a, int64_t idx) {
    RaySeed s;
    if (a.rays) { s.pose = (int)idx; s.x = s.y = 0.f; return s; }
    const int per_pose = a.rows * a.W;
    s.pose = (int)(idx / per_pose);
    const int rem = (int)(idx - (int64_t)s.pose * per_pose);
    const int h = a.row_begin + rem / a.W, w = rem % a.W;
    s.x = __fdiv_rn(__fsub_rn((float)w, a.cx), a.fx);
    s.y = __fdiv_rn(__fsub_rn((float)h, a.cy), a.fy);
    return s;
}

__host__ __device__ inline void share_rep_pixel(const RenderArgs& a, int64_t idx, int* pose, int* h, int* w) {
    const ShareGrid g = share_grid(a);
    const int per_pose = g.nbr * g.nbc;
    *pose = (int)(idx / per_pose);
    const int rem = (int)(idx - (int64_t)*pose * per_pose);
    const int br = g.br0 + rem / g.nbc, bc = rem % g.nbc;
    const int rh = br * g.k + g.k / 2, rw = bc * g.k + g.k / 2;
    *h = rh < a.H - 1 ? rh : a.H - 1;
    *w = rw < a.W - 1 ? rw : a.W - 1;
}
__device__ __forceinline__ RaySeed seed_rep_ray(const RenderArgs& a, int64_t idx) {
    RaySeed s;
    int h, w;
    share_rep_pixel(a, idx, &s.pose, &h, &w);
    s.x = __fdiv_rn(__fsub_rn((float)w, a.cx), a.fx);
    s.y = __fdiv_rn(__fsub_rn((float)h, a.cy), a.fy);
    return s;
}

template <bool SHARE>
__device__ __forceinline__ RaySeed seed_of(const RenderArgs& a, int64_t idx) {
    if constexpr (SHARE) {
        if (share_role(a) == kShareProducer) return seed_rep_ray(a, idx);
    }
    return seed_ray(a, idx);
}

__host__ __device__ inline int share_rep_of(const RenderArgs& a, int64_t idx) {
    const ShareGrid g = share_grid(a);
    const int per_pose = a.rows * a.W;
    const int pose = (int)(idx / per_pose);
    const int rem = (int)(idx - (int64_t)pose * per_pose);
    const int h = a.row_begin + rem / a.W, w = rem % a.W;
    return (pose * g.nbr + (h / g.k - g.br0)) * g.nbc + w / g.k;
}

template <bool VIEW>
__device__ __forceinline__ Ray make_ray(const RenderArgs& a, const RaySeed& s) {
    Ray r;
    r.vx = r.vy = r.vz = 0.f;
    if (a.rays) {
        const float* p = a.rays + (int64_t)s.pose * a.ray_cols;
        r.ox = p[0]; r.oy = p[1]; r.oz = p[2];
        r.dx = p[3]; r.dy = p[4]; r.dz = p[5];
        r.near = p[6]; r.far = p[7];
        if (VIEW && a.ray_cols > 8) { r.vx = p[8]; r.vy = p[9]; r.vz = p[10]; }
    } else {
        const float* m = a.poses + s.pose * 16;
        r.dx = __fadd_rn(__fadd_rn(__fadd_rn(__fmul_rn(m[0], s.x), __fmul_rn(m[1], s.y)), m[2]), 0.f);
        r.dy = __fadd_rn(__fadd_rn(__fadd_rn(__fmul_rn(m[4], s.x), __fmul_rn(m[5], s.y)), m[6]), 0.f);
        r.dz = __fadd_rn(__fadd_rn(__fadd_rn(__fmul_rn(m[8], s.x), __fmul_rn(m[9], s.y)), m[10]), 0.f);
        r.ox = m[3]; r.oy = m[7]; r.oz = m[11];
        r.near = a.near; r.far = a.far;
        if (VIEW) {
            const float n = norm3(r.dx, r.dy, r.dz);
            r.vx = __fdiv_rn(r.dx, n); r.vy = __fdiv_rn(r.dy, n); r.vz = __fdiv_rn(r.dz, n);
        }
    }
    r.dnorm = norm3(r.dx, r.dy, r.dz);
    return r;
}

__device__ __forceinline__ Ray load_ray(const RenderArgs& a, int64_t idx) { return make_ray<true>(a, seed_ray(a, idx)); }

__device__ __forceinline__ float coarse_z(const Ray& r, float t, float omt) {
    return __fadd_rn(__fmul_rn(r.near, omt), __fmul_rn(r.far, t));
}

struct CoarseDepths {
    const float* t_tab; const float* omt_tab;
    const float* jitter;
    int row;
    int ns;
    __device__ __forceinline__ float base(const Ray& r, int i) const { return coarse_z(r, t_tab[i], omt_tab[i]); }
    __device__ __forceinline__ float z(const Ray& r, int i) const {
        const float zi = base(r, i);
        if (!jitter) return zi;
        const float lower = i > 0 ? __fmul_rn(.5f, __fadd_rn(zi, base(r, i - 1))) : zi;
        const float upper = i + 1 < ns ? __fmul_rn(.5f, __fadd_rn(base(r, i + 1), zi)) : zi;
        return __fadd_rn(lower, __fmul_rn(__fsub_rn(upper, lower), jitter[(int64_t)row * ns + i]));
    }
};

__device__ __forceinline__ void point_at(const Ray& r, float z, float& px, float& py, float& pz) {
    px = __fadd_rn(r.ox, __fmul_rn(r.dx, z));
    py = __fadd_rn(r.oy, __fmul_rn(r.dy, z));
    pz = __fadd_rn(r.oz, __fmul_rn(r.dz, z));
}

__device__ __forceinline__ bool occ_empty(const OccGrid* g, float px, float py, float pz) {
    const float cx = floorf(__fmul_rn(__fsub_rn(px, g->lo[0]), g->inv[0]));
    const float cy = floorf(__fmul_rn(__fsub_rn(py, g->lo[1]), g->inv[1]));
    const float cz = floorf(__fmul_rn(__fsub_rn(pz, g->lo[2]), g->inv[2]));
    const int rx = g->res[0], ry = g->res[1], rz = g->res[2];
    bool empty = false;
    if (cx >= 0.f && cx < (float)rx && cy >= 0.f && cy < (float)ry && cz >= 0.f && cz < (float)rz) {
        const int cell = ((int)cx * ry + (int)cy) * rz + (int)cz;
        empty = ((g->bits[cell >> 5] >> (cell & 31)) & 1u) == 0u;
    }
// ... 239 lines not shown
```

nerf-workspaces-explorer_amd/csrc/nwe_host.h:

```cpp
#pragma once
#include <hip/hip_runtime.h>
#include <stdint.h>

#include "nwe_device.h"
#include "nwe_pack.h"
#include "nwe_plan.h"

namespace nwe {

void launch_render_f32(const RenderArgs& a, const NetF32& nc, const NetF32& nf, hipStream_t stream);
void launch_render_f32_occ(const RenderArgs& a, const NetF32& nc, const NetF32& nf, hipStream_t stream);

bool mfma_supported(int D, int W, int in_xyz, int in_dir, int skip, int form);
struct LaunchResources {
    hipEvent_t mid = nullptr;
    unsigned* counters = nullptr;
    hipStream_t side = nullptr;
    hipEvent_t fork = nullptr, join = nullptr;
};
struct LaunchReport {
    bool mid_recorded = false, side_used = false;
};
bool launch_render_mfma(const RenderArgs& a, const NetMfma& nc, const NetMfma& nf, bool three_pass, const PassPlan& plan,
                        const LaunchResources& res, hipStream_t stream, LaunchReport* out);

bool mfma_variant_built(int D, int W, int skip, int form, int variant);

bool mfma_is_lean(const RenderArgs& a);

struct QueryArgs {
    const float* points;
    const float* dirs;
    float* raw;
    float* sigma;
    uint32_t* flags;
    int n_points;
    int points_per_dir;
    int steps;
    int density_only;
};

constexpr int kQueryPacket = 128;
constexpr int kQueryPacketF32 = 16;
constexpr int kQueryMaxSteps = 256;

int query_steps(int64_t packets, int forced, int cus);
void launch_query_f32(const QueryArgs& a, const NetF32& net, int forced_steps, int cus, hipStream_t stream);
bool launch_query_mfma(const QueryArgs& a, const NetMfma& net, bool three_pass, int forced_steps, int cus, hipStream_t stream);

struct OccBuild {
    float lo[3], step[3];
    int res[3];
    int probes;
};
void launch_occ_probe_points(const OccBuild& b, int64_t first, int n_cells, float* points, hipStream_t stream);
void launch_occ_reduce_bits(const float* sigma, int64_t first, int n_cells, int per_cell, float threshold, uint32_t* bits, hipStream_t stream);
void launch_occ_dilate(const uint32_t* src, uint32_t* dst, const int* res, hipStream_t stream);

struct CoarseGrid {
    float lo[3], inv[3];
    int res[3];
    int pad;
    const float* sigma;
};
void launch_coarse_grid_weights(const RenderArgs& a, const CoarseGrid& g, float* table, float* sigma, float* weights, hipStream_t stream);

struct RadianceGrid {
    float lo[3], inv[3];
    int res[3];
    int pad;
    const float4* rows;
};
constexpr int kGridThreads = 64;
void launch_radiance_grid_render(const RenderArgs& a, const RadianceGrid& g, hipStream_t stream);

constexpr int64_t kSparseChunkSamples = (int64_t)1 << 22;
struct SparseChunk {
    int64_t first;
    int count;
    int S;
    float min_weight;
    int dilate;
    float* z;
    float4* row_grid;
    uint8_t* mask;
    uint32_t* offsets;
    uint32_t* total;
    float* points;
    float* dirs;
    const float4* rows;
    float *weights_coarse, *z_fine, *weights_grid, *raw_fine;
    uint8_t* selected;
};
void launch_sparse_mark(const RenderArgs& a, const RadianceGrid& g, const SparseChunk& c, hipStream_t stream);
void launch_sparse_scan(const SparseChunk& c, hipStream_t stream);
void launch_sparse_emit(const RenderArgs& a, const SparseChunk& c, hipStream_t stream);
void launch_sparse_composite(const RenderArgs& a, const SparseChunk& c, hipStream_t stream);

int run_selftest(int32_t* report8, hipStream_t stream);

}
```

nerf-workspaces-explorer_amd/csrc/nwe_kernel_mfma.hip:

```cpp
#include "nwe_mfma_kernels.h"
#include "nwe_mfma_query.h"

namespace nwe {

#define NWE_DECLARE_SHAPE(W_, D_, SKIP_, FORM_)                                                                                   \
    NWE_EXTERN_SHAPE_LAUNCHER(W_, D_, SKIP_, FORM_, kVariantPlain) NWE_EXTERN_SHAPE_LAUNCHER(W_, D_, SKIP_, FORM_, kVariantTerm)   \
    NWE_EXTERN_SHAPE_LAUNCHER(W_, D_, SKIP_, FORM_, kVariantShare) NWE_EXTERN_SHAPE_LAUNCHER(W_, D_, SKIP_, FORM_, kVariantOcc)    \
    NWE_EXTERN_SHAPE_LAUNCHER(W_, D_, SKIP_, FORM_, kVariantTail)                                                                \
    NWE_EXTERN_SHAPE_QUERY_LAUNCHER(W_, D_, SKIP_, FORM_)
NWE_SHAPES(NWE_DECLARE_SHAPE)
#undef NWE_DECLARE_SHAPE

constexpr bool linked(int variant) {
#if !defined(NWE_ONLY_HEADLINE)
    return true;
#elif defined(NWE_DIAG_TAIL)
    return variant == kVariantPlain || variant == kVariantTail;
#else
    return variant == kVariantPlain;
#endif
}
#ifdef NWE_ONLY_HEADLINE
constexpr bool kQueryLinked = false;
#else
constexpr bool kQueryLinked = true;
#endif

using QueryLauncher = void (*)(QueryArgs, const NetMfma&, bool, unsigned, hipStream_t);

template <int W, int D, int SKIP, int FORM, int VARIANT>
constexpr RenderLauncher render_launcher() {
    if constexpr (linked(VARIANT) && variant_built(VARIANT, FORM)) return launch_one<W, D, SKIP, FORM, VARIANT>;
    else return nullptr;
}
template <int W, int D, int SKIP, int FORM>
constexpr QueryLauncher query_launcher() {
    if constexpr (kQueryLinked) return launch_one_query<W, D, SKIP, FORM>;
    else return nullptr;
}

struct ShapeRow {
    int W, D, skip, form, n_chunks;
    RenderLauncher render[kVariants];
    QueryLauncher query;
};
#define NWE_SHAPE_ROW(W_, D_, SKIP_, FORM_)                                                                                  \
    {W_, D_, SKIP_, FORM_, Shape<W_, D_>::n_chunks(FORM_),                                                                   \
     {render_launcher<W_, D_, SKIP_, FORM_, kVariantPlain>(), render_launcher<W_, D_, SKIP_, FORM_, kVariantTerm>(),         \
      render_launcher<W_, D_, SKIP_, FORM_, kVariantShare>(), render_launcher<W_, D_, SKIP_, FORM_, kVariantOcc>(),          \
      render_launcher<W_, D_, SKIP_, FORM_, kVariantTail>()},                                                               \
     query_launcher<W_, D_, SKIP_, FORM_>()},
static_assert(kVariantPlain == 0 && kVariantTerm == 1 && kVariantShare == 2 && kVariantOcc == 3 && kVariantTail == 4 && kVariants == 5,
              "a row lists its launchers in the order of Variant");
static const ShapeRow kShapes[] = {NWE_SHAPES(NWE_SHAPE_ROW)};
#undef NWE_SHAPE_ROW

static const ShapeRow* find_shape(int D, int W, int skip, int form) {
    for (const ShapeRow& r : kShapes)
        if (r.W == W && r.D == D && r.skip == skip && r.form == form) return &r;
    return nullptr;
}

bool mfma_supported(int D, int W, int in_xyz, int in_dir, int skip, int form) {
    if (in_xyz != 63 || in_dir != (form == kFormNoViewDirs ? 0 : 27)) return false;
    return find_shape(D, W, skip, form) != nullptr;
}

bool mfma_variant_built(int D, int W, int skip, int form, int variant) {
    const ShapeRow* shape = find_shape(D, W, skip, form);
    return shape && variant >= 0 && variant < kVariants && shape->render[variant];
}

bool mfma_is_lean(const RenderArgs& a) { return is_lean(a); }

bool launch_render_mfma(const RenderArgs& a, const NetMfma& nc, const NetMfma& nf, bool three_pass, const PassPlan& p,
                        const LaunchResources& res, hipStream_t stream, LaunchReport* out) {
    if (!p.ok) return false;
    if (a.n_importance > 0 && (nf.D != nc.D || nf.W != nc.W || nf.skip != nc.skip || nf.form != nc.form)) return false;
    if (a.n_samples > kSplitMaxSamples) return false;
    const ShapeRow* shape = find_shape(nc.D, nc.W, nc.skip, nc.form);
    if (!shape) return false;
    const RenderLauncher launch = shape->render[p.tail ? kVariantTail : p.variant];
    if (!launch) return false;
    if (nc.n_chunks != shape->n_chunks || (a.n_importance > 0 && nf.n_chunks != shape->n_chunks)) return false;
    const auto dealt = [&](int i) {
        RenderArgs q = a;
        if (p.launch[i].grid) q.queue = res.counters + i;
        return q;
    };
    const auto issue = [&](const RenderArgs& q, int i, hipStream_t s) {
        launch(q, nc, nf, three_pass, p.launch[i].split, p.launch[i].ray_first, p.launch[i].rays, s);
    };
    if (p.n_launches == 1) {
        issue(dealt(0), 0, stream);
        return true;
    }
    RenderArgs first = dealt(0), second = dealt(1);
#ifdef NWE_STAMPS
    if (second.stamps) second.stamps += (size_t)p.launch[0].items * kWaves * kStampWords;
#endif
    if (p.tail) {
        first.tail = second.tail = res.counters + 2;
        second.share = kTailSecond;
    }
    hipStream_t second_stream = stream;
    const auto fork = [&] {
        if (res.side && hipEventRecord(res.fork, stream) == hipSuccess && hipStreamWaitEvent(res.side, res.fork, 0) == hipSuccess)
            second_stream = res.side;
    };
    if (p.fork == kForkFront) fork();
    issue(first, 0, stream);
    if (res.mid) out->mid_recorded = hipEventRecord(res.mid, stream) == hipSuccess;
    if (p.fork == kForkBehind) fork();
    issue(second, 1, second_stream);
    if (second_stream != stream) {
        out->side_used = true;
        if (hipEventRecord(res.join, second_stream) != hipSuccess || hipStreamWaitEvent(stream, res.join, 0) != hipSuccess) return false;
    }
    return true;
}


int query_steps(int64_t packets, int forced, int cus) {
    if (forced > 0) return forced < kQueryMaxSteps ? forced : kQueryMaxSteps;
    const int64_t steps = packets / (8 * (int64_t)cus);
    return (int)(steps < 1 ? 1 : (steps > kQueryMaxSteps ? kQueryMaxSteps : steps));
}

bool launch_query_mfma(const QueryArgs& a_in, const NetMfma& net, bool three_pass, int forced_steps, int cus, hipStream_t stream) {
    const ShapeRow* shape = find_shape(net.D, net.W, net.skip, net.form);
    if (!shape || !shape->query || net.n_chunks != shape->n_chunks) return false;
    if (a_in.n_points <= 0) return true;
    QueryArgs a = a_in;
    const int64_t packets = ((int64_t)a.n_points + kQueryPacket - 1) / kQueryPacket;
    a.steps = query_steps(packets, forced_steps, cus);
    shape->query(a, net, three_pass, (unsigned)((packets + a.steps - 1) / a.steps), stream);
    return true;
}

}
```

nerf-workspaces-explorer_amd/csrc/nwe_mfma_render.h:

```cpp
#pragma once
#include "nwe_mfma_eval.h"

namespace nwe {

template <int W, int D, bool SPLIT>
struct Smem {
    using S = Shape<W, D>;
    static constexpr int WBYTES = (SPLIT ? kSplitMaxSamples : kWaves * kPacketMaxSamples) * kRaysPerWave * 4;
    static constexpr int CHUNKS = 2 * S::CHUNK_BYTES;
    static constexpr int BOFF = CHUNKS;
    static constexpr int BIAS_BYTES = ((S::N_CHUNKS * 32 * 4 + 255) / 256) * 256;
    static constexpr int WOFF = BOFF + 2 * BIAS_BYTES;
    static constexpr int TOFF = WOFF + WBYTES;
    static constexpr int XOFF = TOFF + (2 * kMaxSamples + kMaxImportance) * 4;
    static constexpr int LOFF = XOFF + (SPLIT ? 2 * kWaves * kRaysPerWave * 16 : 0);
    static constexpr int GOFF = LOFF + 3 * 2 * kTileBytes;
    static constexpr int KOFF = GOFF + kWaves * 2 * S::KD * kTileBytes;
    static constexpr int TOTAL = KOFF + kWaves * 4;
    static_assert(XOFF % 16 == 0 && LOFF % 16 == 0 && GOFF % 16 == 0 && KOFF % 16 == 0 && TOTAL % 16 == 0 && TOTAL <= 160 * 1024, "LDS budget");
};

__host__ __device__ inline bool is_lean(const RenderArgs& a) {
    const nwe_outputs& o = a.out;
    return !o.raw_coarse && !o.raw_fine && !o.z_fine && !o.weights_coarse && !o.disp && !o.z_std && !o.rgb_coarse && !o.depth_coarse &&
           !o.acc_coarse && !o.disp_coarse && !o.sample_cond && !o.sample_amp && !o.sample_switch && !o.feat_map && !a.z_fine_in && !a.raw_in_c &&
           !a.raw_in_f && !a.w_in && !a.t_rand && !a.noise_c && !a.noise_f && !a.u_rand && !a.stamps && !a.rays;
}

__device__ __forceinline__ bool store_raw(float* raw, float rr, float rg, float rb, float rs) {
    *reinterpret_cast<float4*>(raw) = make_float4(rr, rg, rb, rs);
    return bad(rr) || bad(rg) || bad(rb) || bad(rs);
}
__device__ __forceinline__ void read_raw(const float* raw_in, int64_t at, float& rr, float& rg, float& rb, float& rs) {
    const float4 v = *reinterpret_cast<const float4*>(raw_in + at * 4);
    rr = v.x; rg = v.y; rb = v.z; rs = v.w;
}

#define NWE_PRIME_STREAM()                                                   \
    {                                                                        \
        wk.start(net.stream, bias);                                          \
        wk.begin(S::N_L0, 0, 0);                                             \
        _Pragma("unroll") for (int i = 0; i < S::N_L0; ++i) wk.piece(i);     \
        wk.begin(S::N_L0, 1, 1);                                             \
        _Pragma("unroll") for (int i = 0; i < S::N_L0; ++i) wk.piece(i);     \
    }
#define NWE_EVAL_POINT(Z, BEHIND_READS)                                                                                            \
    {                                                                                                                              \
        float px, py, pz;                                                                                                          \
        point_at(ray, Z, px, py, pz);                                                                                              \
        h8 Ghi[S::KG], Glo[S::KG];                                                                                                 \
                                                         \
        encode<5, S::KG, X3>(__fdiv_rn(px, 10.f), __fdiv_rn(py, 10.f), __fdiv_rn(pz, 10.f), half, Ghi, Glo);                       \
        NWE_STAMP(const unsigned long long t1 = __builtin_amdgcn_s_memtime(); st_enc += t1 - t0;)                                  \
        wk.template sync<false>();                                                                                                 \
        Frags F;                                                                                                                   \
        _Pragma("unroll") for (int k = 0; k < PD; ++k) {                                                                           \
            F.hi[k] = *reinterpret_cast<const h8*>(wk.cur() + lane * 16 + (2 * k) * kTileBytes);                                   \
            if (X3) F.lo[k] = *reinterpret_cast<const h8*>(wk.cur() + lane * 16 + (2 * k + 1) * kTileBytes);                       \
        }                                                                                                                          \
        BEHIND_READS                                                                                                               \
        NWE_STAMP(const unsigned long long t2 = __builtin_amdgcn_s_memtime(); wk.st_t0 = t2; st_sync += t2 - t1;)                  \
        mlp_eval<W, D, SKIP, X3, FORM, CSKIP>(wk, F, lane, net.inv_scale, Ghi, Glo, gd_lds, dot_tab, density_only, rr, rg, rb, rs, \
                                              skip_word);                                                                          \
        NWE_STAMP(st_mlp += __builtin_amdgcn_s_memtime() - t2;)                                                                    \
    }

constexpr int kVoteBytes = 2 * kWaves * 4;

template <int W, int D, int SKIP, bool X3, bool SPLIT, int FORM, bool LEAN, bool TERM = false, bool SHARE = false>
__global__ void __launch_bounds__(256) render_mfma_kernel(RenderArgs a_in, NetMfma nc, NetMfma nf) {
    static_assert(!TERM || (LEAN && FORM != kFormReference), "early termination: lean kernels of the product formulations only");
    static_assert(!SHARE || (LEAN && !TERM && FORM != kFormReference), "shared coarse pass: lean kernels of the product formulations, not with TERM");
    RenderArgs a = a_in;
    if constexpr (LEAN) {
        a.out.raw_coarse = a.out.raw_fine = a.out.z_fine = a.out.weights_coarse = nullptr;
        a.out.disp = a.out.z_std = a.out.rgb_coarse = a.out.depth_coarse = a.out.acc_coarse = a.out.disp_coarse = nullptr;
        a.out.sample_cond = a.out.sample_amp = a.out.sample_switch = a.out.feat_map = nullptr;
        a.z_fine_in = a.raw_in_c = a.raw_in_f = a.w_in = a.t_rand = a.noise_c = a.noise_f = a.u_rand = nullptr;
        a.stamps = nullptr; a.rays = nullptr;
    }
    using S = Shape<W, D>;
    using SM = Smem<W, D, SPLIT>;
    __shared__ __attribute__((aligned(16))) char smem[SM::TOTAL + (TERM && !SPLIT ? kVoteBytes : 0)];

    static_assert(SM::CHUNKS >= 4 && SM::BOFF >= SM::CHUNKS && SM::WOFF > SM::BOFF && SM::TOFF > SM::BOFF && SM::GOFF > SM::BOFF,
                  "the ticket's word lies in the chunk buffers, below every region the prologue writes in front of its barrier");
    unsigned item = blockIdx.x;
    if constexpr (!TERM && !SHARE) {
        if (a.queue) {
            unsigned* s_item = reinterpret_cast<unsigned*>(smem);
            if (threadIdx.x == 0) *s_item = atomicAdd(a.queue, 1u);
            __syncthreads();
            const unsigned ticket = *s_item;
            if (ticket >= a.queue_items) return;
            item = __builtin_amdgcn_readfirstlane(ticket);
        }
    }

    NWE_STAMP(const unsigned stamp_item = item;)
#include "nwe_mfma_render_item.h"
}

constexpr int kTailOff = 0, kTailSecond = 3;
constexpr unsigned kTailSplit = 0x80000000u, kTailNone = ~0u;
template <int W, int D, int SKIP, bool X3, int FORM, bool LEAN>
__global__ void __launch_bounds__(256) render_mfma_tail_kernel(RenderArgs a_in, NetMfma nc, NetMfma nf) {
    RenderArgs a = a_in;
    unsigned* const tail = a.tail;
    const bool second = a.share == kTailSecond;
    a.w_in = nullptr; a.share = kShareOff;
    if constexpr (LEAN) {
        a.out.raw_coarse = a.out.raw_fine = a.out.z_fine = a.out.weights_coarse = nullptr;
        a.out.disp = a.out.z_std = a.out.rgb_coarse = a.out.depth_coarse = a.out.acc_coarse = a.out.disp_coarse = nullptr;
        a.out.sample_cond = a.out.sample_amp = a.out.sample_switch = a.out.feat_map = nullptr;
        a.z_fine_in = a.raw_in_c = a.raw_in_f = a.t_rand = a.noise_c = a.noise_f = a.u_rand = nullptr;
        a.stamps = nullptr; a.rays = nullptr;
    }
    using SP = Smem<W, D, false>;
    using SS = Smem<W, D, true>;
    __shared__ __attribute__((aligned(16))) char smem[SP::TOTAL > SS::TOTAL ? SP::TOTAL : SS::TOTAL];
    static_assert(SS::CHUNKS >= 4 && SS::BOFF >= SS::CHUNKS && SS::WOFF > SS::BOFF && SS::TOFF > SS::BOFF && SS::GOFF > SS::BOFF &&
                  SP::CHUNKS >= 4 && SP::BOFF >= SP::CHUNKS && SP::WOFF > SP::BOFF && SP::TOFF > SP::BOFF && SP::GOFF > SP::BOFF,
                  "the ticket's word lies in the chunk buffers, below every region either prologue writes in front of its barrier");

    const int64_t split_first = second ? a.ray_first : a.ray_first + (int64_t)a.queue_items * (kWaves * kRaysPerWave);
    unsigned* s_item = reinterpret_cast<unsigned*>(smem);
    if (threadIdx.x == 0) {
        unsigned t;
        if (!second) {
            t = atomicAdd(a.queue, 1u);
            if (t >= a.queue_items) {
                const unsigned items1 = (unsigned)((a.n_rays - split_first + kRaysPerWave - 1) / kRaysPerWave);
                const unsigned s = atomicAdd(tail, 1u);
                t = s < items1 ? kTailSplit | s : kTailNone;
            }
        } else {
            t = a.queue ? atomicAdd(a.queue, 1u) : blockIdx.x;
            const unsigned n = a.queue ? a.queue_items : gridDim.x;
            t = t < n && t >= *tail ? kTailSplit | t : kTailNone;
            if (t != kTailNone) atomicAdd(tail + 1, 1u);
        }
        *s_item = t;
    }
    __syncthreads();
    const unsigned ticket = *s_item;
    if (ticket == kTailNone) return;
    const unsigned t = __builtin_amdgcn_readfirstlane(ticket);
    using S = Shape<W, D>;
    constexpr bool TERM = false, SHARE = false;
    if (t & kTailSplit) {
        constexpr bool SPLIT = true;
        using SM = SS;
        const unsigned item = t & ~kTailSplit;
        NWE_STAMP(const unsigned stamp_item = second ? item : a.queue_items + item;)
        a.ray_first = split_first;
#include "nwe_mfma_render_item.h"
    } else {
        constexpr bool SPLIT = false;
        using SM = SP;
        const unsigned item = t;
        NWE_STAMP(const unsigned stamp_item = item;)
#include "nwe_mfma_render_item.h"
    }
}
template <int W, int D, int SKIP, bool X3, bool SPLIT, int FORM>
__global__ void __launch_bounds__(256) render_mfma_occ_kernel(RenderArgs a_in, NetMfma nc, NetMfma nf) {
    static_assert(FORM != kFormReference, "occupancy grid: lean kernels of the product formulations only");
    constexpr bool LEAN = true, TERM = false, SHARE = false;
    RenderArgs a = a_in;
    const OccGrid* const occ = a_in.occ;
    a.out.raw_coarse = a.out.raw_fine = a.out.z_fine = a.out.weights_coarse = nullptr;
    a.out.disp = a.out.z_std = a.out.rgb_coarse = a.out.depth_coarse = a.out.acc_coarse = a.out.disp_coarse = nullptr;
    a.out.sample_cond = a.out.sample_amp = a.out.sample_switch = a.out.feat_map = nullptr;
    a.z_fine_in = a.raw_in_c = a.raw_in_f = a.w_in = a.t_rand = a.noise_c = a.noise_f = a.u_rand = nullptr;
    a.stamps = nullptr; a.rays = nullptr;
    using S = Shape<W, D>;
    using SM = Smem<W, D, SPLIT>;
    __shared__ __attribute__((aligned(16))) char smem[SM::TOTAL + kVoteBytes];
    const unsigned item = blockIdx.x;
    NWE_STAMP(const unsigned stamp_item = item;)
#define NWE_ITEM_OCC
#include "nwe_mfma_render_item.h"
#undef NWE_ITEM_OCC
}
#undef NWE_PRIME_STREAM
#undef NWE_EVAL_POINT

#ifdef NWE_STAMPS
constexpr bool kTailLean = false;
#else
constexpr bool kTailLean = true;
#endif

using RenderKernel = void (*)(RenderArgs, NetMfma, NetMfma);
using RenderLauncher = void (*)(RenderArgs, const NetMfma&, const NetMfma&, bool, bool, int64_t, int64_t, hipStream_t);

template <int W, int D, int SKIP, int FORM, int VARIANT>
void launch_one(RenderArgs a, const NetMfma& nc, const NetMfma& nf, bool three_pass, bool split, int64_t ray_first, int64_t rays,
                hipStream_t stream) {
    if constexpr (variant_built(VARIANT, FORM)) {
        if (rays <= 0) return;
        a.ray_first = ray_first;
        const unsigned items = mfma_workgroups(rays, split);
        const bool queued = (VARIANT == kVariantPlain || VARIANT == kVariantTail) && a.queue;
        if (queued) a.queue_items = items;
        const unsigned grid = queued ? queue_grid(items) : items;
        RenderKernel kernel;
        if constexpr (VARIANT == kVariantPlain) {
#define NWE_KERNEL(X3_, SPLIT_, LEAN_) render_mfma_kernel<W, D, SKIP, X3_, SPLIT_, FORM, LEAN_>
            const RenderKernel kernels[8] = {
                NWE_KERNEL(true, true, true),  NWE_KERNEL(true, true, false),  NWE_KERNEL(true, false, true),  NWE_KERNEL(true, false, false),
                NWE_KERNEL(false, true, true), NWE_KERNEL(false, true, false), NWE_KERNEL(false, false, true), NWE_KERNEL(false, false, false)};
#undef NWE_KERNEL
            kernel = kernels[(three_pass ? 0 : 4) + (split ? 0 : 2) + (is_lean(a) ? 0 : 1)];
        } else if constexpr (VARIANT == kVariantTail) {
            const RenderKernel kernels[2] = {render_mfma_tail_kernel<W, D, SKIP, true, FORM, kTailLean>,
                                             render_mfma_tail_kernel<W, D, SKIP, false, FORM, kTailLean>};
            kernel = kernels[three_pass ? 0 : 1];
        } else if constexpr (VARIANT == kVariantOcc) {
#define NWE_KERNEL(X3_, SPLIT_) render_mfma_occ_kernel<W, D, SKIP, X3_, SPLIT_, FORM>
            const RenderKernel kernels[4] = {NWE_KERNEL(true, true), NWE_KERNEL(true, false), NWE_KERNEL(false, true), NWE_KERNEL(false, false)};
#undef NWE_KERNEL
            kernel = kernels[(three_pass ? 0 : 2) + (split ? 0 : 1)];
        } else {
#define NWE_KERNEL(X3_, SPLIT_) render_mfma_kernel<W, D, SKIP, X3_, SPLIT_, FORM, true, VARIANT == kVariantTerm, VARIANT == kVariantShare>
            const RenderKernel kernels[4] = {NWE_KERNEL(true, true), NWE_KERNEL(true, false), NWE_KERNEL(false, true), NWE_KERNEL(false, false)};
#undef NWE_KERNEL
            kernel = kernels[(three_pass ? 0 : 2) + (split ? 0 : 1)];
        }
        hipLaunchKernelGGL(kernel, dim3(grid), dim3(256), 0, stream, a, nc, nf);
    }
}

}
```

nerf-workspaces-explorer_amd/csrc/nwe_mfma_render_item.h:

```cpp
    const int lane = threadIdx.x & 63;
    const int wave = __builtin_amdgcn_readfirstlane(threadIdx.x >> 6);
    const int half = lane >> 5;
    const int ns = a.n_samples, ni = a.n_importance;

    float* s_t = reinterpret_cast<float*>(smem + SM::TOFF);
    float* s_omt = s_t + kMaxSamples;
    float* s_u = s_omt + kMaxSamples;
    for (int i = threadIdx.x; i < ns; i += 256) { s_t[i] = a.t_vals[i]; s_omt[i] = a.omt_vals[i]; }
    for (int i = threadIdx.x; i < ni; i += 256) s_u[i] = a.u_vals[i];
    float* s_bias = reinterpret_cast<float*>(smem + SM::BOFF);
    constexpr int NCH = S::n_chunks(FORM);
    constexpr int NROWS = S::n_bias_rows(FORM);
    static_assert(NROWS * 32 * 4 <= SM::BIAS_BYTES, "bias table too small for the dot rows");
    for (int i = threadIdx.x; i < NROWS * 32; i += 256) {
        s_bias[i] = nc.bias[i];
        if (ni > 0) s_bias[SM::BIAS_BYTES / 4 + i] = nf.bias[i];
    }

    const int64_t packet = SPLIT ? (int64_t)item : (int64_t)item * kWaves + wave;
    const int64_t ridx64 = a.ray_first + packet * kRaysPerWave + (lane & 31);
    const bool lane_live = ridx64 < a.n_rays && half == 0;
    const bool live = lane_live && (!SPLIT || wave == 0);
    const bool gone = ridx64 >= a.n_rays;
    int row_of = (int)(ridx64 < a.n_rays ? ridx64 : a.n_rays - 1);
// ... 66 lines not shown
    for (int pass = 0; pass < (ni > 0 ? 2 : 1); ++pass) {
        const NetMfma& net = pass == 0 ? nc : nf;
        const float* bias = s_bias + (pass == 0 ? 0 : SM::BIAS_BYTES / 4);
        const float* dot_tab = bias + NCH * 32;
        const int Stot = pass == 0 ? ns : ns + ni;
        const bool density_only = LEAN && density_only_built<D, SKIP>(FORM) && pass == 0 && ni > 0;
        const float* noise = pass == 0 ? a.noise_c : a.noise_f;
        const float* raw_in = pass == 0 ? a.raw_in_c : a.raw_in_f;
        if (pass == 0 && a.w_in) {
            if (wc_writer) for (int s = 0; s < ns; ++s) fs.wc[s * kRaysPerWave] = a.w_in[rclamp * ns + s];
            continue;
        }
        if constexpr (SHARE) {
            if (pass == 0 && consumer) {
                const float* col = a.share_w + share_rep_of(a, rclamp);
                const int n_rep = share_n_rep(a, share_grid(a));
                if (wc_writer) for (int s = 0; s < ns; ++s) fs.wc[s * kRaysPerWave] = col[(int64_t)s * n_rep];
                continue;
            }
        }
        comp.reset();
        const bool stops = TERM && (pass == 1 || ni == 0);
        const float eps = stops ? a.min_trans : 0.f;
        if constexpr (SPLIT) {
            int produced = 0;
            auto gen = [&](const Ray& ray) -> float {
                const int i = produced++;
                if (i >= Stot) return 0.f;
                if (pass == 0) return fs.cd.z(ray, i);
                return a.z_fine_in ? a.z_fine_in[rclamp * Stot + i] : fs.next(ray);
            };
            float zq[5], zp[4];
            {
                const Ray ray = fresh_ray();
                if (pass == 1) {
                    if (wc_writer) fs.build_cdf();
                    __syncthreads();
                    fs.start(ray);
                    if (wants_survey(a.out)) {
                        const SampleSurvey sv = fs.survey(ray);
                        if (live) flags |= store_survey(a.out, ridx, sv);
                    }
                }
#pragma unroll
                for (int k = 0; k < 5; ++k) zq[k] = gen(ray);
            }
            float4* xch = reinterpret_cast<float4*>(smem + SM::XOFF);
            const int n_it = (Stot + 3) / 4;
            auto drain = [&](int it) {
                const float4* x = xch + (it & 1) * (kWaves * kRaysPerWave) + (lane & 31);
#pragma unroll
                for (int k = 0; k < 4; ++k) {
                    const int si = 4 * it + k;
                    if (si < Stot) {
                        const float w = TERM ? comp.accumulate_above(x[k * kRaysPerWave], zp[k], eps) : comp.accumulate(x[k * kRaysPerWave], zp[k]);
                        if (pass == 0) {
                            if (wc_writer) fs.wc[si * kRaysPerWave] = w;
                            if constexpr (SHARE) { if (producer && live) a.share_w[si * a.n_rays + row] = w; }
                            if (live && a.out.weights_coarse) a.out.weights_coarse[ridx * ns + si] = w;
                        }
                    }
                }
            };
            [[maybe_unused]] int it_end = n_it;
            for (int it = 0; it < n_it; ++it) {
                if constexpr (TERM) {
                    if (stops && it > 0 && __all(gone || comp.below(eps))) { it_end = it; break; }
                }
#ifdef NWE_ITEM_OCC
                unsigned long long occ_mask = 0;
                bool occ_skip = false;
                {
                    const OccGrid* g = occ;
                    asm volatile("" : "+s"(g));
                    const Ray ray = fresh_ray();
                    float zo = zq[0];
                    if (wave == 1) zo = zq[1];
                    if (wave == 2) zo = zq[2];
                    if (wave == 3) zo = zq[3];
                    float px, py, pz;
                    point_at(ray, zo, px, py, pz);
                    const bool empty = occ_empty(g, px, py, pz);
                    occ_mask = __ballot(empty);
                    const int mine = __all(gone || 4 * it + wave >= Stot || empty);
                    int* vote = reinterpret_cast<int*>(smem + SM::TOTAL);
                    if (lane == 0) vote[(it & 1) * kWaves + wave] = mine;
                    __syncthreads();
                    const int* v = vote + (it & 1) * kWaves;
                    occ_skip = __builtin_amdgcn_readfirstlane(v[0] & v[1] & v[2] & v[3]) != 0;
                    if (!occ_skip) occ_evals += Stot - 4 * it < 4 ? Stot - 4 * it : 4;
                }
#endif
                NWE_STAMP(const unsigned long long t0 = __builtin_amdgcn_s_memtime();)
#ifdef NWE_ITEM_OCC
                if (!occ_skip)
#endif
                if (!raw_in) NWE_PRIME_STREAM();
                const Ray ray = fresh_ray();
                const int s_own = 4 * it + wave;
                const bool own_valid = s_own < Stot;
                float z_own = zq[0], z_nxt = zq[1];
                if (wave == 1) { z_own = zq[1]; z_nxt = zq[2]; }
                if (wave == 2) { z_own = zq[2]; z_nxt = zq[3]; }
                if (wave == 3) { z_own = zq[3]; z_nxt = zq[4]; }
                float nz[4];
#pragma unroll
                for (int k = 0; k < 4; ++k) nz[k] = gen(ray);
                float rr, rg, rb, rs;
                if (raw_in) {
                    __syncthreads();
                    if (it > 0) drain(it - 1);
#pragma unroll
                    for (int k = 0; k < 4; ++k) zp[k] = zq[k];
                    read_raw(raw_in, rclamp * Stot + (own_valid ? s_own : Stot - 1), rr, rg, rb, rs);
#ifdef NWE_ITEM_OCC
                } else if (occ_skip) {
                    if (it > 0) drain(it - 1);
#pragma unroll
                    for (int k = 0; k < 4; ++k) zp[k] = zq[k];
                    rr = rg = rb = rs = 0.f;
#endif
                } else {
                    NWE_EVAL_POINT(z_own, if (it > 0) drain(it - 1); _Pragma("unroll") for (int k = 0; k < 4; ++k) zp[k] = zq[k];);
#ifdef NWE_ITEM_OCC
                    if ((occ_mask >> lane) & 1) rr = rg = rb = rs = 0.f;
#endif
                }
                NWE_STAMP(const unsigned long long t3 = __builtin_amdgcn_s_memtime();)
                if (own_valid) {
                    xch[(it & 1) * (kWaves * kRaysPerWave) + wave * kRaysPerWave + (lane & 31)] =
                        Composite::shade(rr, rg, rb, rs, z_own, z_nxt, s_own + 1 == Stot, ray.dnorm, noise ? noise[rclamp * Stot + s_own] : 0.f);
                    if (lane_live) {
                        float* raw = pass == 0 ? a.out.raw_coarse : a.out.raw_fine;
                        if (raw && store_raw(raw + (ridx * Stot + s_own) * 4, rr, rg, rb, rs)) flags |= NWE_FLAG_RAW;
                        if (pass == 1 && a.out.z_fine) a.out.z_fine[ridx * Stot + s_own] = z_own;
                    }
                }
                zq[0] = zq[4];
#pragma unroll
                for (int k = 0; k < 4; ++k) zq[k + 1] = nz[k];
                NWE_STAMP(st_comp += __builtin_amdgcn_s_memtime() - t3;)
            }
            __syncthreads();
            drain(TERM ? it_end - 1 : n_it - 1);
            __syncthreads();
            if constexpr (TERM) {
                if (stops) {
                    const unsigned long long mine = __popcll(__ballot(lane_live));
                    const int walked = (ni > 0 ? ns : 0) + (4 * it_end < Stot ? 4 * it_end : Stot);
                    if (wave == 0 && lane == 0) atomicAdd(a.evals, mine * (unsigned long long)walked);
                }
            }
        } else {
            float z_cur, z_next = 0.f;
            {
                const Ray ray = fresh_ray();
                if (pass == 0) z_cur = fs.cd.z(ray, 0);
                else {
                    fs.prepare(ray);
                    if (wants_survey(a.out)) {
                        const SampleSurvey sv = fs.survey(ray);
                        if (live) flags |= store_survey(a.out, ridx, sv);
                    }
                    z_cur = a.z_fine_in ? a.z_fine_in[rclamp * Stot] : fs.next(ray);
                }
            }
            [[maybe_unused]] int s_end = Stot;
            for (int s = 0; s < Stot; ++s) {
                if constexpr (TERM) {
                    if (stops) {
                        int* vote = reinterpret_cast<int*>(smem + SM::TOTAL);
                        const int mine = __all(gone || comp.below(eps));
                        if (lane == 0) vote[(s & 1) * kWaves + wave] = mine;
                        if (s > 0) {
                            const int* v = vote + ((s - 1) & 1) * kWaves;
                            if (__builtin_amdgcn_readfirstlane(v[0] & v[1] & v[2] & v[3])) { s_end = s; break; }
                        }
                    }
                }
#ifdef NWE_ITEM_OCC
                unsigned long long occ_mask = 0;
                bool occ_skip = false;
                {
                    const OccGrid* g = occ;
                    asm volatile("" : "+s"(g));
                    const Ray ray = fresh_ray();
                    float px, py, pz;
                    point_at(ray, z_cur, px, py, pz);
                    const bool empty = occ_empty(g, px, py, pz);
                    occ_mask = __ballot(empty);
                    const int mine = __all(gone || empty);
                    const int n = pass == 0 ? s : ns + s;
                    int* vote = reinterpret_cast<int*>(smem + SM::TOTAL);
                    if (lane == 0) vote[(n & 1) * kWaves + wave] = mine;
                    __syncthreads();
                    const int* v = vote + (n & 1) * kWaves;
                    occ_skip = __builtin_amdgcn_readfirstlane(v[0] & v[1] & v[2] & v[3]) != 0;
                    if (!occ_skip) ++occ_evals;
                }
#endif
                NWE_STAMP(const unsigned long long t0 = __builtin_amdgcn_s_memtime();)
#ifdef NWE_ITEM_OCC
                if (!occ_skip)
#endif
                if (!raw_in) NWE_PRIME_STREAM();
                const Ray ray = fresh_ray();
                if (s + 1 < Stot) {
                    if (pass == 0) z_next = fs.cd.z(ray, s + 1);
                    else z_next = a.z_fine_in ? a.z_fine_in[rclamp * Stot + s + 1] : fs.next(ray);
                }
                float rr, rg, rb, rs;
                if (raw_in) {
                    read_raw(raw_in, rclamp * Stot + s, rr, rg, rb, rs);
#ifdef NWE_ITEM_OCC
                } else if (occ_skip) {
                    rr = rg = rb = rs = 0.f;
#endif
                } else {
                    NWE_EVAL_POINT(z_cur, );
#ifdef NWE_ITEM_OCC
                    if ((occ_mask >> lane) & 1) rr = rg = rb = rs = 0.f;
#endif
                }
                NWE_STAMP(const unsigned long long t3 = __builtin_amdgcn_s_memtime();)
                const float4 shaded = Composite::shade(rr, rg, rb, rs, z_cur, z_next, s + 1 == Stot, ray.dnorm, noise ? noise[rclamp * Stot + s] : 0.f);
                const float w = TERM ? comp.accumulate_above(shaded, z_cur, eps) : comp.accumulate(shaded, z_cur);
                if (pass == 0) fs.wc[s * kRaysPerWave] = w;
                if constexpr (SHARE) { if (producer && lane_live) a.share_w[s * a.n_rays + row] = w; }
                if (lane_live) {
                    if (pass == 0 && a.out.weights_coarse) a.out.weights_coarse[ridx * ns + s] = w;
                    float* raw = pass == 0 ? a.out.raw_coarse : a.out.raw_fine;
                    if (raw && store_raw(raw + (ridx * Stot + s) * 4, rr, rg, rb, rs)) flags |= NWE_FLAG_RAW;
                    if (pass == 1 && a.out.z_fine) a.out.z_fine[ridx * Stot + s] = z_cur;
                }
                z_cur = z_next;
                NWE_STAMP(st_comp += __builtin_amdgcn_s_memtime() - t3;)
            }
            if constexpr (TERM) {
                if (stops) {
                    const unsigned long long mine = __popcll(__ballot(lane_live));
                    if (lane == 0 && mine) atomicAdd(a.evals, mine * (unsigned long long)((ni > 0 ? ns : 0) + s_end));
                }
            }
        }
        if (live) {
            flags |= store_ray(a.out, ridx, comp, pass == 1, a.white_bkgd != 0) & (density_only ? ~(uint32_t)NWE_FLAG_RGB_COARSE : ~0u);
            if (ni == 0) flags |= store_ray(a.out, ridx, comp, true, a.white_bkgd != 0);
        }
        if (producer) break;
    }
#ifdef NWE_ITEM_OCC
    {
        const unsigned long long mine = __popcll(__ballot(lane_live));
        if (lane == 0 && mine && (!SPLIT || wave == 0)) atomicAdd(a.evals, mine * (unsigned long long)occ_evals);
    }
#endif
    if (flags && a.out.flags) atomicOr(a.out.flags, flags);
#ifdef NWE_STAMPS
    if (a.stamps && lane == 0) {
        unsigned long long* o = a.stamps + ((size_t)stamp_item * kWaves + wave) * kStampWords;
        o[0] = st_enc; o[1] = st_sync; o[2] = st_mlp; o[3] = st_comp; o[4] = __builtin_amdgcn_s_memtime() - st_begin;
        o[5] = wk.st_pre; o[6] = wk.st_wait; o[7] = wk.st_post;
        const unsigned long long st_real_end = __builtin_amdgcn_s_memrealtime();
        o[8] = st_real_end - st_real; o[9] = st_begin;
        o[10] = (unsigned long long)__builtin_amdgcn_s_getreg((31 << 11) | 20) | (unsigned long long)__builtin_amdgcn_s_getreg((31 << 11) | 4) << 32;
        o[11] = stamp_item; o[12] = st_real; o[13] = st_real_end;
    }
#endif
```

nerf-workspaces-explorer_amd/csrc/nwe_plan.cpp:

```cpp
#include "nwe_plan.h"

namespace nwe {

static int plan_launch(const PassDesc& a, int cus, int64_t* full_out) {
    const int64_t rays_wg = kWaves * kRaysPerWave;
    const int s_coarse = a.role == kShareConsumer ? 0 : a.n_samples;
    const int s_fine = a.role == kShareProducer || a.n_importance <= 0 ? 0 : a.n_samples + a.n_importance;
    const double its = (double)(s_coarse + s_fine);
    const double its_split = 1.06 * (double)((s_coarse + 3) / 4 + (s_fine + 3) / 4);
    const auto rounds = [&](int64_t rays, int64_t per_wg) { return (double)(((rays + per_wg - 1) / per_wg + cus - 1) / cus); };
    const int64_t full = (a.n_rays / rays_wg / cus) * cus * rays_wg;
    const double t_packet = rounds(a.n_rays, rays_wg) * its;
    const double t_split = rounds(a.n_rays, kRaysPerWave) * its_split;
    const double t_hybrid = full > 0 && full < a.n_rays ? (double)(full / rays_wg / cus) * its + rounds(a.n_rays - full, kRaysPerWave) * its_split : 1e300;
    const double t_single = t_packet <= t_split ? t_packet : t_split;
    int plan = t_hybrid < 0.992 * t_single ? 2 : (t_packet <= t_split ? 0 : 1);
    if (a.decomposition >= 0) plan = a.decomposition;
    if (a.n_samples > kPacketMaxSamples) plan = 1;
    *full_out = full;
    return plan;
}

PassPlan plan_pass(const PassDesc& d, int cus) {
    PassPlan p;
    if (d.variant < 0) return p;
    p.ok = true;
    p.variant = d.variant;
    int64_t full = 0;
    p.plan = plan_launch(d, cus, &full);
    const auto deal = [&](LaunchPlan& l, int64_t ray_first, int64_t rays, bool split) {
        l.ray_first = ray_first; l.rays = rays; l.split = split;
        l.items = mfma_workgroups(rays, split);
        if (d.may_queue && rays > 0 && (d.queue_mode == 1 || l.items > (unsigned)cus)) l.grid = queue_grid(l.items);
    };
    if (p.plan != 2) {
        p.n_launches = 1;
        deal(p.launch[0], 0, d.n_rays, p.plan == 1);
        return p;
    }
    p.n_launches = 2;
    deal(p.launch[0], 0, full, false);
    deal(p.launch[1], full, d.n_rays - full, true);
    if (!d.side || !p.queued()) return p;
    const bool lean = d.lean && (d.stamped_build || !d.stamps);
    p.tail = p.launch[0].grid && d.tail && lean && d.tail_built && d.n_rays > full &&
             p.launch[0].grid - p.launch[0].items >= p.launch[1].items;
    p.tail_items = p.tail ? p.launch[1].items : 0;
    p.fork = p.tail ? kForkBehind : kForkFront;
    return p;
}

static int stage_variant(const CallDesc& c, int role, bool lean, int n_importance, bool w_in, int net) {
    const bool share = role != kShareOff && lean;
    int v = kVariantPlain;
    if (c.occ) v = lean && role == kShareOff && !c.term ? kVariantOcc : -1;
    else if (c.term) v = lean && !share ? kVariantTerm : -1;
    else if (share) v = n_importance > 0 ? kVariantShare : -1;
    else if (role != kShareOff && (role == kShareProducer ? n_importance != 0 : !w_in)) v = -1;
    return v >= 0 && c.built[net][v] ? v : -1;
}

CallPlan plan_call(const CallDesc& c, int cus) {
    CallPlan p;
    const bool lean = c.lean && !c.stamps;
    p.baked = c.baked && c.n_importance > 0;
    p.separate = c.separate && c.mfma && c.n_importance > 0;
    p.share = c.n_importance > 0 && (p.baked || c.share_k > 1 || (p.separate && lean && c.built[0][kVariantShare] && c.built[1][kVariantShare]));
    p.full = p.separate && !p.share;
    p.coarse_launch = p.share || (p.full && !c.w_in);
    p.share_k = p.share ? c.share_k : 1;
    p.occ = c.occ;
    p.need_evals = c.term || c.occ;
    if (p.baked) p.table_elems = c.n_rays * c.n_samples;
    else if (p.share) p.table_elems = c.n_rep * c.n_samples;
    else if (p.full && p.coarse_launch && !c.want_weights_coarse) p.table_elems = c.n_rays * c.n_samples;
    p.coarse_flags = p.full && p.coarse_launch && c.want_flags;

    StagePlan& m = p.main;
    m.active = true;
    m.role = p.share || p.full ? kShareConsumer : kShareOff;
    m.n_rays = c.n_rays; m.n_importance = c.n_importance;
    m.net = p.separate || p.baked ? 1 : -1;
    StagePlan& k = p.coarse;
    if (p.coarse_launch) {
        k.active = true;
        k.role = kShareProducer;
        k.n_rays = p.share && !p.baked ? c.n_rep : c.n_rays;
        k.n_importance = p.share && !p.baked ? c.n_importance : 0;
        k.net = p.separate || p.baked ? 0 : -1;
    }
    p.evals_full = c.n_rays * (int64_t)(c.n_samples + (c.n_importance > 0 ? c.n_samples + c.n_importance : 0));
    if (p.baked) p.evals_run = c.n_rays * (int64_t)(c.n_samples + c.n_importance);
    else p.evals_run = p.coarse_launch ? k.n_rays * c.n_samples + c.n_rays * (int64_t)(c.n_samples + c.n_importance) : p.evals_full;
    p.share_rays = p.coarse_launch ? k.n_rays : 0;
    if (!c.mfma) return p;

    const bool plain_only = !p.separate && !p.share && !c.term && !c.occ;
    const auto describe = [&](const StagePlan& s, bool stage_lean, bool w_in) {
        PassDesc d;
        d.n_rays = s.n_rays; d.n_samples = c.n_samples; d.n_importance = s.n_importance;
        d.role = s.role;
        d.lean = stage_lean && c.lean; d.stamps = c.stamps; d.stamped_build = c.stamped_build;
        d.variant = stage_variant(c, s.role, stage_lean && lean, s.n_importance, w_in, s.net > 0 ? 1 : 0);
        d.tail_built = c.built[s.net > 0 ? 1 : 0][kVariantTail];
        d.decomposition = c.decomposition; d.queue_mode = c.queue_mode;
        return d;
    };
    if (k.active && !p.baked) k.pass = plan_pass(describe(k, !p.full, false), cus);
    PassDesc d = describe(m, !p.full, p.full || c.w_in);
    d.may_queue = plain_only && c.queue_mode != 0;
    d.side = c.backfill; d.tail = c.tail;
    m.pass = plan_pass(d, cus);
    p.may_queue = m.pass.queued();
    p.need_side = p.may_queue && c.backfill;
    p.blocks = c.packet_blocks && lean && plain_only && m.pass.ok && m.pass.variant == kVariantPlain && packet_blocks_fit(c.rows, c.width);
    return p;
}

}
```

nerf-workspaces-explorer_amd/csrc/nwe_plan.h:

```cpp
#pragma once
#include <stdint.h>

#include "nwe_pack.h"
#include "nwe_packet_blocks.h"

namespace nwe {

constexpr int kMaxSamples = 128;
constexpr int kMaxImportance = 256;

constexpr int kWaves = 4;
constexpr int kRaysPerWave = 32;
static_assert(kBlockW * kBlockH == kRaysPerWave, "a packet is one pixel block");

constexpr int kPacketMaxSamples = 64;
constexpr int kSplitMaxSamples = kMaxSamples;

constexpr int kShareOff = 0, kShareProducer = 1, kShareConsumer = 2;

enum Variant { kVariantPlain, kVariantTerm, kVariantShare, kVariantOcc, kVariantTail, kVariants };

constexpr bool variant_built(int variant, int form) {
    return variant == kVariantTerm || variant == kVariantShare || variant == kVariantOcc ? form != kFormReference : true;
}

inline unsigned queue_grid(unsigned n) { return (unsigned)(((uint64_t)n + (n + 3) / 4 + 7) / 8 * 8); }

inline unsigned mfma_workgroups(int64_t rays, bool split) {
    const int64_t per_wg = split ? kRaysPerWave : kWaves * kRaysPerWave;
    return (unsigned)((rays + per_wg - 1) / per_wg);
}


struct PassDesc {
    int64_t n_rays = 0;
    int n_samples = 0, n_importance = 0;
    int role = kShareOff;
    int variant = kVariantPlain;
    bool lean = false;
    bool stamps = false;
    bool stamped_build = false;
    bool tail_built = false;
    int decomposition = -1;
    int queue_mode = -1;
    bool may_queue = false;
    bool side = false;
    bool tail = false;
};

struct LaunchPlan {
    int64_t ray_first = 0, rays = 0;
    bool split = false;
    unsigned items = 0, grid = 0;
};

enum Fork { kForkNone, kForkFront, kForkBehind };

struct PassPlan {
    bool ok = false;
    int variant = kVariantPlain;
    int plan = -1;
    int n_launches = 0;
    LaunchPlan launch[2];
    int fork = kForkNone;
    bool tail = false;
    unsigned tail_items = 0;
    bool queued() const { return launch[0].grid || launch[1].grid; }
};

PassPlan plan_pass(const PassDesc& d, int cus);


struct CallDesc {
    int64_t n_rays = 0;
    int64_t n_rep = 0;
    int n_samples = 0, n_importance = 0;
    bool mfma = false;
    bool term = false;
    bool occ = false;
    int share_k = 1;
    bool separate = false;
    bool baked = false;
    bool lean = false, stamps = false, stamped_build = false;
    bool w_in = false;
    bool want_weights_coarse = false, want_flags = false;
    bool built[2][kVariants] = {};
    int decomposition = -1, queue_mode = -1;
    bool backfill = true, tail = true;
    int rows = 0, width = 0;
    bool packet_blocks = false;
};

struct StagePlan {
    bool active = false;
    int role = kShareOff;
    int64_t n_rays = 0;
    int n_importance = 0;
    int net = 0;
    PassPlan pass;
};

struct CallPlan {
    bool separate = false;
    bool share = false;
    bool full = false;
    bool coarse_launch = false;
    bool may_queue = false;
    bool need_side = false;
    bool need_evals = false;
    bool occ = false;
    bool baked = false;
    int share_k = 1;
    bool blocks = false;
    int64_t table_elems = 0;
    bool coarse_flags = false;
    int64_t evals_full = 0, evals_run = 0, share_rays = 0;
    StagePlan coarse, main;
};

CallPlan plan_call(const CallDesc& c, int cus);

}
```

nerf-workspaces-explorer_amd/renderer.py:

```python
from __future__ import annotations

import ctypes as C
from typing import Dict, Iterable, Mapping, Optional, Sequence, Tuple

import numpy as np
import torch

from . import _lib

LAYER_ORDER_TAIL = ("_views_linears.0", "_feature_linear", "_alpha_linear", "_rgb_linear")

_PER_RAY = {"rgb": 3, "depth": 1, "acc": 1, "disp": 1, "z_std": 1, "rgb_coarse": 3, "depth_coarse": 1,
            "acc_coarse": 1, "disp_coarse": 1, "sample_cond": 1, "sample_amp": 1, "sample_switch": 1}


def normalize_state_dict(sd: Mapping[str, object]) -> Dict[str, np.ndarray]:
    out = {}
    for k, v in sd.items():
        if isinstance(v, torch.Tensor):
            v = v.detach().cpu().numpy()
        v = np.ascontiguousarray(np.asarray(v, dtype=np.float32))
        out[k if k.startswith("_") else "_" + k] = v
    return out

# ... 110 lines not shown
            res[name] = torch.empty(shape, dtype=torch.float32, device=self.device)
        res["flags"] = torch.zeros(1, dtype=torch.int32, device=self.device)
        o = _lib.Outputs()
        for name in _lib.OUTPUT_FIELDS:
            setattr(o, name, res[name].data_ptr() if name in res else None)
        return o, res

    def render(self, c2w, H: int, W: int, *, fx: float, fy: float, cx: float, cy: float, near: float, far: float,
               rows: Optional[Tuple[int, int]] = None, precision: str = "f16x3",
               outputs: Sequence[str] = ("rgb", "depth", "acc")) -> Dict[str, torch.Tensor]:
        poses = np.ascontiguousarray(np.asarray(c2w, dtype=np.float32).reshape(-1, 4, 4))
        r0, r1 = rows if rows is not None else (0, H)
        n_rays = poses.shape[0] * (r1 - r0) * W
        with torch.cuda.device(self.device):
            o, res = self._alloc(n_rays, outputs)
            stream = torch.cuda.current_stream(self.device).cuda_stream
            rc = self._lib.nwe_render(self._ctx, poses.ctypes.data, poses.shape[0], H, W, fx, fy, cx, cy, near, far, r0, r1,
                                      _lib.PRECISIONS[precision], C.byref(o), stream)
        self._check(rc, "nwe_render")
        return res

    def create_rays(self, c2w, H: int, W: int, *, fx: float, fy: float, cx: float, cy: float, near: float, far: float,
                    rows: Optional[Tuple[int, int]] = None, use_view_dirs: bool = True) -> torch.Tensor:
        poses = np.ascontiguousarray(np.asarray(c2w, dtype=np.float32).reshape(-1, 4, 4))
        r0, r1 = rows if rows is not None else (0, H)
        with torch.cuda.device(self.device):
            out = torch.empty((poses.shape[0] * (r1 - r0) * W, 11), dtype=torch.float32, device=self.device)
            stream = torch.cuda.current_stream(self.device).cuda_stream
            rc = self._lib.nwe_create_rays(self._ctx, poses.ctypes.data, poses.shape[0], H, W, fx, fy, cx, cy, near, far, r0, r1,
                                           out.data_ptr(), stream)
        self._check(rc, "nwe_create_rays")
        return out if use_view_dirs else out[:, :8].contiguous()

    def render_rays(self, rays: torch.Tensor, *, precision: str = "f16x3",
                    outputs: Sequence[str] = ("rgb", "depth", "acc"),
                    debug_fine_depths: Optional[torch.Tensor] = None,
                    debug_raw: Optional[Tuple[Optional[torch.Tensor], Optional[torch.Tensor]]] = None,
                    debug_coarse_weights: Optional[torch.Tensor] = None,
                    train: Optional[Dict[str, Optional[torch.Tensor]]] = None) -> Dict[str, torch.Tensor]:
        if rays.dim() != 2 or rays.shape[1] != self.ray_columns or rays.dtype != torch.float32:
            raise ValueError(f"rays must be float32 [R,{self.ray_columns}] for these networks")
        rays = rays.to(self.device).contiguous()
        keep = []
        S = self.n_samples + self.n_importance
        if debug_fine_depths is not None:
            debug_fine_depths = debug_fine_depths.to(self.device, torch.float32).contiguous()
            if tuple(debug_fine_depths.shape) != (rays.shape[0], S):
                raise ValueError("debug_fine_depths must be [R, n_samples + n_importance]")
        raw_ptrs = None
        if debug_raw is not None:
            raw_ptrs = []
            for t, n in zip(debug_raw, (self.n_samples, S)):
                if t is None:
                    raw_ptrs.append(None)
                    continue
                t = t.to(self.device, torch.float32).contiguous()
                if tuple(t.shape) != (rays.shape[0], n, 4):
                    raise ValueError(f"debug_raw entries must be [R, {n}, 4]")
                keep.append(t)
                raw_ptrs.append(t.data_ptr())
        weights = None
        if debug_coarse_weights is not None:
            weights = debug_coarse_weights.to(self.device, torch.float32).contiguous()
            if tuple(weights.shape) != (rays.shape[0], self.n_samples):
                raise ValueError("debug_coarse_weights must be [R, n_samples]")
            keep.append(weights)
        train_ptrs = None
        if train:
            R, ns, ni = rays.shape[0], self.n_samples, self.n_importance
            shapes = {"t_rand": (R, ns), "noise_coarse": (R, ns), "noise_fine": (R, ns + ni), "u": (R, ni)}
            unknown = set(train) - set(shapes)
            if unknown:
                raise ValueError(f"unknown train keys {sorted(unknown)}")
            train_ptrs = []
            for key in ("t_rand", "noise_coarse", "noise_fine", "u"):
                t = train.get(key)
                if t is None:
                    train_ptrs.append(None)
                    continue
                t = t.to(self.device, torch.float32)
                if tuple(t.shape) != shapes[key]:
                    raise ValueError(f"train[{key!r}] must be {shapes[key]}")
                if key == "u":
                    t = torch.sort(t, dim=-1).values
                t = t.contiguous()
                keep.append(t)
                train_ptrs.append(t.data_ptr())
        if precision not in _lib.PRECISIONS:
            raise ValueError(f"unknown precision {precision!r}")
        with torch.cuda.device(self.device):
            o, res = self._alloc(rays.shape[0], outputs)
            stream = torch.cuda.current_stream(self.device).cuda_stream
            if debug_fine_depths is not None:
                self._lib.nwe_debug_set_fine_depths(self._ctx, debug_fine_depths.data_ptr())
            if raw_ptrs is not None:
                self._lib.nwe_debug_set_raw(self._ctx, *raw_ptrs)
            if weights is not None:
                self._lib.nwe_debug_set_coarse_weights(self._ctx, weights.data_ptr())
            if train_ptrs is not None:
                self._lib.nwe_set_train_tables(self._ctx, *train_ptrs)
            rc = self._lib.nwe_render_rays(self._ctx, rays.data_ptr(), rays.shape[0], _lib.PRECISIONS[precision], C.byref(o), stream)
        if rc != _lib.NWE_OK:
            self.disarm_hooks()
        self._check(rc, "nwe_render_rays")
        res["_keepalive_rays"] = rays
        if keep:
            res["_keepalive_train"] = keep
        if debug_fine_depths is not None:
            res["_keepalive_depths"] = debug_fine_depths
        return res

    def disarm_hooks(self) -> None:
        self._lib.nwe_debug_set_fine_depths(self._ctx, None)
        self._lib.nwe_debug_set_raw(self._ctx, None, None)
        self._lib.nwe_debug_set_coarse_weights(self._ctx, None)
        self._lib.nwe_set_train_tables(self._ctx, None, None, None, None)

    def debug_set_fold(self, on: bool) -> None:
        self._check(self._lib.nwe_debug_set_fold(self._ctx, 1 if on else 0), "nwe_debug_set_fold")

    def debug_set_decomposition(self, mode: int) -> None:
        self._check(self._lib.nwe_debug_set_decomposition(self._ctx, int(mode)), "nwe_debug_set_decomposition")

    def debug_last_plan(self) -> int:
        return int(self._lib.nwe_debug_last_plan(self._ctx))

    def debug_set_work_queue(self, mode: int) -> None:
        self._check(self._lib.nwe_debug_set_work_queue(self._ctx, int(mode)), "nwe_debug_set_work_queue")

    def debug_get_work_queue(self) -> int:
        return int(self._lib.nwe_debug_get_work_queue(self._ctx))

    def debug_last_queue(self):
        items, grid, taken, side = (C.c_uint * 2)(), (C.c_uint * 2)(), (C.c_uint * 2)(), C.c_int(0)
        self._check(self._lib.nwe_debug_last_queue(self._ctx, items, grid, taken, C.byref(side)), "nwe_debug_last_queue")
        return {"items": tuple(items), "grid": tuple(grid), "taken": tuple(taken), "side_stream": bool(side.value)}

    def debug_last_tail(self) -> int:
        stolen = C.c_uint(0)
        self._check(self._lib.nwe_debug_last_tail(self._ctx, C.byref(stolen)), "nwe_debug_last_tail")
        return int(stolen.value)

    def debug_last_tail_rest(self) -> int:
        n = C.c_uint(0)
        self._check(self._lib.nwe_debug_last_tail_rest(self._ctx, C.byref(n)), "nwe_debug_last_tail_rest")
        return int(n.value)

    def debug_set_colour_skip(self, mode: int) -> None:
        self._check(self._lib.nwe_debug_set_colour_skip(self._ctx, int(mode)), "nwe_debug_set_colour_skip")

    def debug_get_colour_skip(self) -> int:
        return int(self._lib.nwe_debug_get_colour_skip(self._ctx))

    def debug_set_packet_blocks(self, on: bool) -> None:
        self._check(self._lib.nwe_debug_set_packet_blocks(self._ctx, 1 if on else 0), "nwe_debug_set_packet_blocks")

    def debug_last_packet_blocks(self) -> int:
        return int(self._lib.nwe_debug_last_packet_blocks(self._ctx))

    def debug_get_work_queue_tail(self) -> bool:
        return bool(self._lib.nwe_debug_get_work_queue_tail(self._ctx))

    def set_white_background(self, on: bool) -> None:
        self._check(self._lib.nwe_set_white_background(self._ctx, 1 if on else 0), "nwe_set_white_background")

    def set_early_termination(self, min_transmittance: float) -> None:
        self._check(self._lib.nwe_set_early_termination(self._ctx, float(min_transmittance)), "nwe_set_early_termination")

    @property
    def early_termination(self) -> float:
        return float(self._lib.nwe_get_early_termination(self._ctx))

    def set_shared_coarse(self, k: int) -> None:
        self._check(self._lib.nwe_set_shared_coarse(self._ctx, int(k)), "nwe_set_shared_coarse")

    @property
    def shared_coarse(self) -> int:
        return int(self._lib.nwe_get_shared_coarse(self._ctx))

    def set_separate_passes(self, on: bool) -> None:
        self._check(self._lib.nwe_set_separate_passes(self._ctx, 1 if on else 0), "nwe_set_separate_passes")

    @property
    def separate_passes(self) -> bool:
        return int(self._lib.nwe_get_separate_passes(self._ctx)) == 1

    @staticmethod
    def _occupancy_box(lo, hi, resolution):
        res3 = (int(resolution),) * 3 if isinstance(resolution, (int, np.integer)) else tuple(int(r) for r in resolution)
        if len(res3) != 3 or len(lo) != 3 or len(hi) != 3:
            raise ValueError("occupancy needs lo, hi of three coordinates and a resolution of one or three ints")
        return (C.c_float * 3)(*[float(v) for v in lo]), (C.c_float * 3)(*[float(v) for v in hi]), (C.c_int * 3)(*res3), res3

    @staticmethod
    def pack_occupancy(bits) -> np.ndarray:
        if isinstance(bits, torch.Tensor):
            bits = bits.detach().cpu().numpy()
        flat = np.ascontiguousarray(bits).astype(bool).reshape(-1)
        padded = np.zeros((flat.size + 31) // 32 * 32, dtype=np.uint8)
        padded[:flat.size] = flat
        shifted = padded.reshape(-1, 32).astype(np.uint32) << np.arange(32, dtype=np.uint32)[None, :]
        return np.ascontiguousarray(np.bitwise_or.reduce(shifted, axis=1), dtype=np.uint32)

    @staticmethod
    def unpack_occupancy(words: np.ndarray, resolution) -> np.ndarray:
        rx, ry, rz = (int(r) for r in resolution)
        w = np.ascontiguousarray(words, dtype=np.uint32)
        flat = ((w[:, None] >> np.arange(32, dtype=np.uint32)[None, :]) & 1).astype(bool).reshape(-1)
        return flat[:rx * ry * rz].reshape(rx, ry, rz)

    def set_occupancy(self, bits, lo: Sequence[float], hi: Sequence[float], resolution) -> None:
        lo3, hi3, res3, res = self._occupancy_box(lo, hi, resolution)
        n_words = (res[0] * res[1] * res[2] + 31) // 32 if min(res) > 0 else 0
        if isinstance(bits, torch.Tensor) and bits.dtype != torch.bool:
            bits = bits.detach().cpu().numpy()
        arr = bits if isinstance(bits, torch.Tensor) else np.asarray(bits)
        if arr.dtype in (np.uint32, np.int32) and arr.ndim == 1:
            words = np.ascontiguousarray(arr).view(np.uint32)
        else:
            if tuple(arr.shape) != res:
                raise ValueError(f"occupancy bits must be a bool array of shape {res} or packed uint32 words, got {tuple(arr.shape)}")
            words = self.pack_occupancy(arr)
        if min(res) > 0 and words.size != n_words:
            raise ValueError(f"occupancy needs {n_words} words for resolution {res}, got {words.size}")
        self._check(self._lib.nwe_set_occupancy(self._ctx, lo3, hi3, res3, words.ctypes.data if words.size else None, 0), "nwe_set_occupancy")

    def build_occupancy(self, lo: Sequence[float], hi: Sequence[float], resolution, probes: int = 2, threshold: float = 0.0,
                        dilate: int = 1, precision: str = "f16x3") -> None:
        if precision not in _lib.PRECISIONS:
            raise ValueError(f"unknown precision {precision!r}")
        lo3, hi3, res3, _ = self._occupancy_box(lo, hi, resolution)
        stream = None
        if self.device is not None:
            stream = torch.cuda.current_stream(self.device).cuda_stream
        self._check(self._lib.nwe_build_occupancy(self._ctx, lo3, hi3, res3, int(probes), float(threshold), int(dilate),
                                                  _lib.PRECISIONS[precision], stream), "nwe_build_occupancy")

    def clear_occupancy(self) -> None:
        self._check(self._lib.nwe_clear_occupancy(self._ctx), "nwe_clear_occupancy")

    @property
    def occupancy(self) -> Optional[Dict[str, object]]:
        lo, hi, res, inv, occ = (C.c_float * 3)(), (C.c_float * 3)(), (C.c_int * 3)(), (C.c_float * 3)(), C.c_int64(0)
        if self._lib.nwe_get_occupancy(self._ctx, lo, hi, res, inv, C.byref(occ)) != _lib.NWE_OK:
            return None
        cells = res[0] * res[1] * res[2]
        return {"lo": tuple(lo), "hi": tuple(hi), "resolution": tuple(res), "inv": np.array(list(inv), dtype=np.float32),
                "occupied_cells": int(occ.value), "occupied": occ.value / cells}

    def occupancy_bits(self) -> Optional[np.ndarray]:
        g = self.occupancy
        if g is None:
            return None
        rx, ry, rz = g["resolution"]
        words = np.empty((rx * ry * rz + 31) // 32, dtype=np.uint32)
        self._check(self._lib.nwe_occupancy_copy(self._ctx, words.ctypes.data, words.size), "nwe_occupancy_copy")
        return self.unpack_occupancy(words, (rx, ry, rz))

    def set_coarse_grid(self, sigma, lo: Sequence[float], hi: Sequence[float], resolution=None) -> None:
        if resolution is None:
            resolution = tuple(sigma.shape)
        lo3, hi3, res3, res = self._occupancy_box(lo, hi, resolution)
        on_device = isinstance(sigma, torch.Tensor) and self.device is not None and sigma.device == self.device
        if on_device:
            values = sigma.detach().to(torch.float32).contiguous()
            n, ptr = values.numel(), values.data_ptr()
        else:
            if isinstance(sigma, torch.Tensor):
                sigma = sigma.detach().cpu().numpy()
            values = np.ascontiguousarray(np.asarray(sigma, dtype=np.float32))
            n, ptr = values.size, values.ctypes.data
        if min(res) > 0 and n != res[0] * res[1] * res[2]:
            raise ValueError(f"the coarse grid needs {res[0] * res[1] * res[2]} values for resolution {res}, got {n}")
        if on_device:
            torch.cuda.current_stream(self.device).synchronize()
        self._check(self._lib.nwe_set_coarse_grid(self._ctx, lo3, hi3, res3, ptr if n else None, 1 if on_device else 0), "nwe_set_coarse_grid")

    def bake_coarse_grid(self, lo: Sequence[float], hi: Sequence[float], resolution, precision: str = "f16x3") -> None:
        if precision not in _lib.PRECISIONS:
            raise ValueError(f"unknown precision {precision!r}")
        lo3, hi3, res3, _ = self._occupancy_box(lo, hi, resolution)
        stream = None
        if self.device is not None:
            stream = torch.cuda.current_stream(self.device).cuda_stream
        self._check(self._lib.nwe_bake_coarse_grid(self._ctx, lo3, hi3, res3, _lib.PRECISIONS[precision], stream), "nwe_bake_coarse_grid")

    def clear_coarse_grid(self) -> None:
        self._check(self._lib.nwe_clear_coarse_grid(self._ctx), "nwe_clear_coarse_grid")

    @property
    def coarse_grid(self) -> Optional[Dict[str, object]]:
        lo, hi, res, inv = (C.c_float * 3)(), (C.c_float * 3)(), (C.c_int * 3)(), (C.c_float * 3)()
        if self._lib.nwe_get_coarse_grid(self._ctx, lo, hi, res, inv) != _lib.NWE_OK:
            return None
        return {"lo": tuple(lo), "hi": tuple(hi), "resolution": tuple(res), "inv": np.array(list(inv), dtype=np.float32)}

    def coarse_grid_values(self) -> Optional[np.ndarray]:
        g = self.coarse_grid
        if g is None:
            return None
        rx, ry, rz = g["resolution"]
        values = np.empty(rx * ry * rz, dtype=np.float32)
        self._check(self._lib.nwe_coarse_grid_copy(self._ctx, values.ctypes.data, values.size), "nwe_coarse_grid_copy")
        return values.reshape(rx, ry, rz)

    def coarse_grid_weights(self, c2w, H: int, W: int, *, fx: float, fy: float, cx: float, cy: float, near: float, far: float,
# ... 394 lines not shown
```

Before: 374.3 million.

## Add deferred colour-head evaluation kernel variant with global scratch ring

Adds a new kernel variant that evaluates only the density trunk per sample. It stores trunk features for samples with non-negligible weight in a per-wave scratch ring in global memory, then runs the colour head on those batched samples afterwards. The aim is to skip colour-layer MFMA work for samples that contribute little to the composite, and to batch what remains. The cost is a large scratch allocation sized per work item, extra LDS, and more global traffic. It is enabled by default via the plan when the lean plain-variant path applies with importance sampling.

New measurement: 382.8 million, median of 6. 1.02x the previous value.

```diff
diff --git a/include/nwe.h b/include/nwe.h
--- a/include/nwe.h
+++ b/include/nwe.h
@@ -239,6 +239,12 @@
 int nwe_debug_set_colour_skip(nwe_ctx *ctx, int mode);
 int nwe_debug_get_colour_skip(const nwe_ctx *ctx);
 
+int nwe_debug_set_colour_defer(nwe_ctx *ctx, int mode);
+int nwe_debug_get_colour_defer(const nwe_ctx *ctx);
+int nwe_debug_last_defer(nwe_ctx *ctx, uint64_t *out4);
+int nwe_debug_last_plan_defer(const nwe_ctx *ctx, int64_t *scratch_bytes);
+int64_t nwe_debug_defer_scratch_bytes(const nwe_ctx *ctx);
+
 int nwe_debug_set_packet_blocks(nwe_ctx *ctx, int on);
 int nwe_debug_last_packet_blocks(const nwe_ctx *ctx);
 int nwe_debug_packet_pixels(int64_t first, int64_t n, int W, int32_t *pixels);
diff --git a/nerf-workspaces-explorer_amd/_lib.py b/nerf-workspaces-explorer_amd/_lib.py
--- a/nerf-workspaces-explorer_amd/_lib.py
+++ b/nerf-workspaces-explorer_amd/_lib.py
@@ -32,7 +32,9 @@
            "nwe_set_radiance_grid", "nwe_clear_radiance_grid", "nwe_get_radiance_grid", "nwe_radiance_grid_copy", "nwe_bake_radiance_grid",
            "nwe_render_grid", "nwe_last_grid_ms",
            "nwe_render_sparse", "nwe_debug_set_sparse_chunk", "nwe_last_sparse_ms", "nwe_last_sparse_samples",
-           "nwe_debug_set_packet_blocks", "nwe_debug_last_packet_blocks", "nwe_debug_packet_pixels")
+           "nwe_debug_set_packet_blocks", "nwe_debug_last_packet_blocks", "nwe_debug_packet_pixels",
+           "nwe_debug_set_colour_defer", "nwe_debug_get_colour_defer", "nwe_debug_last_defer", "nwe_debug_last_plan_defer",
+           "nwe_debug_defer_scratch_bytes")
 
 
 class Outputs(C.Structure):
@@ -162,6 +164,11 @@
         "nwe_packed_colour_finite": (I, [P, I]),
         "nwe_debug_set_colour_skip": (I, [P, I]),
         "nwe_debug_get_colour_skip": (I, [P]),
+        "nwe_debug_set_colour_defer": (I, [P, I]),
+        "nwe_debug_get_colour_defer": (I, [P]),
+        "nwe_debug_last_defer": (I, [P, C.POINTER(C.c_uint64)]),
+        "nwe_debug_last_plan_defer": (I, [P, C.POINTER(C.c_int64)]),
+        "nwe_debug_defer_scratch_bytes": (C.c_int64, [P]),
         "nwe_debug_set_packet_blocks": (I, [P, I]),
         "nwe_debug_last_packet_blocks": (I, [P]),
         "nwe_debug_packet_pixels": (I, [I64, I64, I, P]),
diff --git a/nerf-workspaces-explorer_amd/csrc/nwe_abi.hip b/nerf-workspaces-explorer_amd/csrc/nwe_abi.hip
--- a/nerf-workspaces-explorer_amd/csrc/nwe_abi.hip
+++ b/nerf-workspaces-explorer_amd/csrc/nwe_abi.hip
@@ -72,6 +72,9 @@
     unsigned q_items[2] = {0, 0}, q_grid[2] = {0, 0};
     bool side_used = false;
     unsigned tail_items = 0;
+    uint8_t* defer = nullptr;
+    int defer_region = 0;
+    uint64_t defer_seq = 0;
 };
 
 struct GridBox {
@@ -164,9 +167,18 @@
     bool backfill = true;
     bool tail = true;
     int colour_skip = 1;
+    int colour_defer = 1;
+    struct DeferRegion {
+        DevBuf<uint8_t> buf;
+        const RenderSlot* user = nullptr;
+        hipStream_t stream = nullptr;
+        uint64_t seq = 0;
+    };
+    DeferRegion defer_regions[kSlots];
     int last_plan = -1;
     bool packet_blocks = true;
     int last_packet_blocks = 0;
+    int64_t last_plan_defer = -1;
     unsigned long long* stamps = nullptr;
     const float *trn_t = nullptr, *trn_nc = nullptr, *trn_nf = nullptr, *trn_u = nullptr;
     std::string err;
@@ -206,6 +218,7 @@
     d.stamps = c->stamps != nullptr;
     d.decomposition = c->decomposition; d.queue_mode = c->work_queue;
     d.backfill = c->backfill; d.tail = c->tail; d.packet_blocks = c->packet_blocks;
+    d.colour_skip = c->colour_skip; d.colour_defer = c->colour_defer;
     return d;
 }
 struct MaybeContext {
@@ -341,7 +354,32 @@
     d.backfill = ctx.backfill; d.tail = ctx.tail;
     if (!a.rays) { d.rows = a.rows; d.width = a.W; }
     d.packet_blocks = ctx.packet_blocks;
+    d.colour_skip = ctx.colour_skip; d.colour_defer = ctx.colour_defer;
+    d.net_width = ctx.net[a.n_importance > 0 ? 1 : 0].W;
     return d;
+}
+
+bool provide_defer(nwe_ctx* ctx, RenderSlot& slot, int64_t bytes, hipStream_t stream) {
+    const size_t need = (size_t)bytes;
+    nwe_ctx::DeferRegion* pick = nullptr;
+    for (nwe_ctx::DeferRegion& g : ctx->defer_regions) {
+        bool is_free = !g.user || g.user == &slot || g.stream == stream;
+        if (!is_free) {
+            is_free = hipEventQuery(g.user->ev1) == hipSuccess;
+            (void)hipGetLastError();
+        }
+        if (!is_free) continue;
+        if (!pick || (pick->buf.cap < need && g.buf.cap > pick->buf.cap)) pick = &g;
+        if (pick->buf.cap >= need) break;
+    }
+    if (!pick) return false;
+    if (pick->buf.reserve(need) != hipSuccess) { (void)hipGetLastError(); pick->user = nullptr; return false; }
+    if (hipMemsetAsync(pick->buf.get(), 0, (size_t)kDeferScratchHead, stream) != hipSuccess) { (void)hipGetLastError(); return false; }
+    pick->user = &slot; pick->stream = stream; ++pick->seq;
+    slot.defer = pick->buf.get();
+    slot.defer_region = (int)(pick - ctx->defer_regions);
+    slot.defer_seq = pick->seq;
+    return true;
 }
 
 int provide(nwe_ctx* ctx, RenderSlot& slot, const CallPlan& p, hipStream_t stream) {
@@ -405,17 +443,24 @@
 int launch(nwe_ctx* ctx, const ContextDesc& desc, RenderSlot& slot, RenderArgs& a, int precision, hipStream_t stream) {
     context_args(ctx, a);
     if (a.n_rays <= 0) return NWE_OK;
-    const CallPlan p = plan_call(describe_call(desc, a, precision), ctx->cus);
+    CallPlan p = plan_call(describe_call(desc, a, precision), ctx->cus);
     const bool mfma = precision != NWE_PREC_F32, three_pass = precision == NWE_PREC_F16X3;
+    slot.defer = nullptr;
+    if (p.defer && !provide_defer(ctx, slot, p.defer_bytes, stream)) {
+        slot.defer = nullptr;
+        p.defer = false; p.defer_bytes = 0;
+        ctx->warn = "deferred colour: the scratch could not be allocated; this call runs without deferral";
+    }
     TRY(provide(ctx, slot, p, stream));
     const RenderArgs prod = stage_args(p, slot, a);
     if (p.occ) a.occ = ctx->d_occ.get();
     if (p.blocks) a.ray_cols |= kPacketBlocksBit;
     ctx->last_packet_blocks = p.blocks ? 1 : 0;
+    ctx->last_plan_defer = p.defer ? p.defer_bytes : -1;
     const NetState &nc = ctx->net[0], &nf = ctx->net[ctx->ni > 0 ? 1 : 0];
     const auto with_skip = [&](const NetState& n) {
         NetMfma m = n.mf;
-        m.colour_skip = ctx->colour_skip == 2 || (ctx->colour_skip == 1 && n.p.colour_finite) ? 1 : 0;
+        m.colour_skip = ctx->colour_skip == 2 || (ctx->colour_skip == 1 && (n.p.colour_finite || (p.defer && ctx->colour_defer == 2))) ? 1 : 0;
         return m;
     };
     const NetMfma mf[2] = {with_skip(nc), with_skip(nf)};
@@ -455,6 +500,7 @@
             res.counters = slot.queue.get();
             res.side = slot.side; res.fork = slot.ev_fork; res.join = slot.ev_join;
         }
+        if (p.defer) res.defer = reinterpret_cast<char*>(slot.defer);
         report = {};
         if (!run(p.main, a, res, &report)) {
             if (!report.side_used) return fail(ctx, NWE_ERR_UNSUPPORTED, shapes_differ);
@@ -755,6 +801,7 @@
     if (const int v = env_switch("NWE_WORK_QUEUE_TAIL"); v >= 0) c->tail = v == 1;
     if (const int v = env_switch("NWE_COLOUR_SKIP"); v >= 0) c->colour_skip = v;
     if (const int v = env_switch("NWE_PACKET_BLOCKS"); v >= 0) c->packet_blocks = v == 1;
+    if (const int v = env_switch("NWE_COLOUR_DEFER"); v >= 0) c->colour_defer = v;
     if (!c->host_only) {
         const hipError_t e = hipSetDevice(device);
         if (e != hipSuccess) { delete c; return fail(nullptr, NWE_ERR_HIP, std::string("nwe_create: ") + hipGetErrorString(e)); }
@@ -996,6 +1043,31 @@
 int nwe_debug_get_work_queue(const nwe_ctx* c) { return c ? c->work_queue : -2; }
 int nwe_debug_set_colour_skip(nwe_ctx* c, int mode) { return set_on(mode < 0 || mode > 2 ? nullptr : c, [&] { c->colour_skip = mode; }); }
 int nwe_debug_get_colour_skip(const nwe_ctx* c) { return c ? c->colour_skip : -1; }
+int nwe_debug_set_colour_defer(nwe_ctx* c, int mode) { return set_on(mode < 0 || mode > 2 ? nullptr : c, [&] { c->colour_defer = mode; }); }
+int nwe_debug_get_colour_defer(const nwe_ctx* c) { return c ? c->colour_defer : -1; }
+int nwe_debug_last_defer(nwe_ctx* c, uint64_t* out4) {
+    if (!c || !out4) return NWE_ERR_INVALID;
+    for (int i = 0; i < 4; ++i) out4[i] = 0;
+    const RenderSlot* s = last_render(c);
+    if (!s) return fail(c, NWE_ERR_STATE, "nothing has been launched");
+    if (!s->defer) return NWE_OK;
+    if (c->defer_regions[s->defer_region].seq != s->defer_seq) return fail(c, NWE_ERR_STATE, "a later call has taken that launch's scratch: its counters are gone");
+    ON_DEVICE(c);
+    HIPCHK(c, hipEventSynchronize(s->ev1));
+    HIPCHK(c, hipMemcpy(out4, s->defer, 4 * sizeof(uint64_t), hipMemcpyDeviceToHost));
+    return NWE_OK;
+}
+int nwe_debug_last_plan_defer(const nwe_ctx* c, int64_t* scratch_bytes) {
+    if (!c) return -1;
+    if (scratch_bytes) *scratch_bytes = c->last_plan_defer < 0 ? 0 : c->last_plan_defer;
+    return c->last_plan_defer < 0 ? 0 : 1;
+}
+int64_t nwe_debug_defer_scratch_bytes(const nwe_ctx* c) {
+    if (!c) return -1;
+    int64_t total = 0;
+    for (const nwe_ctx::DeferRegion& g : c->defer_regions) total += (int64_t)g.buf.cap;
+    return total;
+}
 int nwe_debug_set_packet_blocks(nwe_ctx* c, int on) { return set_on(on < 0 || on > 1 ? nullptr : c, [&] { c->packet_blocks = on != 0; }); }
 int nwe_debug_last_packet_blocks(const nwe_ctx* c) { return c ? c->last_packet_blocks : -1; }
 int nwe_debug_packet_pixels(int64_t first, int64_t n, int W, int32_t* pixels) {
@@ -1032,6 +1104,7 @@
     if (a.n_rays <= 0) return NWE_OK;
     const CallPlan p = plan_call(describe_call(desc.d, a, precision), cus);
     c->last_packet_blocks = p.blocks ? 1 : 0;
+    c->last_plan_defer = p.defer ? p.defer_bytes : -1;
     report->separate = p.separate; report->share = p.share; report->full = p.full; report->coarse_launch = p.coarse_launch;
     report->may_queue = p.may_queue; report->need_side = p.need_side; report->need_evals = p.need_evals;
     report->coarse_flags = p.coarse_flags; report->share_k = p.share_k;
diff --git a/nerf-workspaces-explorer_amd/csrc/nwe_check.h b/nerf-workspaces-explorer_amd/csrc/nwe_check.h
--- a/nerf-workspaces-explorer_amd/csrc/nwe_check.h
+++ b/nerf-workspaces-explorer_amd/csrc/nwe_check.h
@@ -39,6 +39,7 @@
     bool stamps = false;
     int decomposition = -1, queue_mode = -1;
     bool backfill = true, tail = true, packet_blocks = true;
+    int colour_skip = 1, colour_defer = 1;
 };
 
 
diff --git a/nerf-workspaces-explorer_amd/csrc/nwe_device.h b/nerf-workspaces-explorer_amd/csrc/nwe_device.h
--- a/nerf-workspaces-explorer_amd/csrc/nwe_device.h
+++ b/nerf-workspaces-explorer_amd/csrc/nwe_device.h
@@ -42,6 +42,7 @@
     union {
         unsigned long long* stamps;
         const OccGrid* occ;
+        char* defer;
     };
     nwe_outputs out;
     float min_trans;
diff --git a/nerf-workspaces-explorer_amd/csrc/nwe_host.h b/nerf-workspaces-explorer_amd/csrc/nwe_host.h
--- a/nerf-workspaces-explorer_amd/csrc/nwe_host.h
+++ b/nerf-workspaces-explorer_amd/csrc/nwe_host.h
@@ -17,6 +17,7 @@
     unsigned* counters = nullptr;
     hipStream_t side = nullptr;
     hipEvent_t fork = nullptr, join = nullptr;
+    char* defer = nullptr;
 };
 struct LaunchReport {
     bool mid_recorded = false, side_used = false;
diff --git a/nerf-workspaces-explorer_amd/csrc/nwe_kernel_mfma.hip b/nerf-workspaces-explorer_amd/csrc/nwe_kernel_mfma.hip
--- a/nerf-workspaces-explorer_amd/csrc/nwe_kernel_mfma.hip
+++ b/nerf-workspaces-explorer_amd/csrc/nwe_kernel_mfma.hip
@@ -6,7 +6,7 @@
 #define NWE_DECLARE_SHAPE(W_, D_, SKIP_, FORM_)                                                                                   \
     NWE_EXTERN_SHAPE_LAUNCHER(W_, D_, SKIP_, FORM_, kVariantPlain) NWE_EXTERN_SHAPE_LAUNCHER(W_, D_, SKIP_, FORM_, kVariantTerm)   \
     NWE_EXTERN_SHAPE_LAUNCHER(W_, D_, SKIP_, FORM_, kVariantShare) NWE_EXTERN_SHAPE_LAUNCHER(W_, D_, SKIP_, FORM_, kVariantOcc)    \
-    NWE_EXTERN_SHAPE_LAUNCHER(W_, D_, SKIP_, FORM_, kVariantTail)                                                                \
+    NWE_EXTERN_SHAPE_LAUNCHER(W_, D_, SKIP_, FORM_, kVariantTail) NWE_EXTERN_SHAPE_LAUNCHER(W_, D_, SKIP_, FORM_, kVariantDefer)   \
     NWE_EXTERN_SHAPE_QUERY_LAUNCHER(W_, D_, SKIP_, FORM_)
 NWE_SHAPES(NWE_DECLARE_SHAPE)
 #undef NWE_DECLARE_SHAPE
@@ -30,7 +30,8 @@
 
 template <int W, int D, int SKIP, int FORM, int VARIANT>
 constexpr RenderLauncher render_launcher() {
-    if constexpr (linked(VARIANT) && variant_built(VARIANT, FORM)) return launch_one<W, D, SKIP, FORM, VARIANT>;
+    if constexpr (linked(VARIANT) && variant_built(VARIANT, FORM) && (VARIANT != kVariantDefer || colour_defer_built<D, SKIP>(FORM)))
+        return launch_one<W, D, SKIP, FORM, VARIANT>;
     else return nullptr;
 }
 template <int W, int D, int SKIP, int FORM>
@@ -48,9 +49,10 @@
     {W_, D_, SKIP_, FORM_, Shape<W_, D_>::n_chunks(FORM_),                                                                   \
      {render_launcher<W_, D_, SKIP_, FORM_, kVariantPlain>(), render_launcher<W_, D_, SKIP_, FORM_, kVariantTerm>(),         \
       render_launcher<W_, D_, SKIP_, FORM_, kVariantShare>(), render_launcher<W_, D_, SKIP_, FORM_, kVariantOcc>(),          \
-      render_launcher<W_, D_, SKIP_, FORM_, kVariantTail>()},                                                               \
+      render_launcher<W_, D_, SKIP_, FORM_, kVariantTail>(), render_launcher<W_, D_, SKIP_, FORM_, kVariantDefer>()},        \
      query_launcher<W_, D_, SKIP_, FORM_>()},
-static_assert(kVariantPlain == 0 && kVariantTerm == 1 && kVariantShare == 2 && kVariantOcc == 3 && kVariantTail == 4 && kVariants == 5,
+static_assert(kVariantPlain == 0 && kVariantTerm == 1 && kVariantShare == 2 && kVariantOcc == 3 && kVariantTail == 4 && kVariantDefer == 5 &&
+                  kVariants == 6,
               "a row lists its launchers in the order of Variant");
 static const ShapeRow kShapes[] = {NWE_SHAPES(NWE_SHAPE_ROW)};
 #undef NWE_SHAPE_ROW
@@ -88,7 +90,15 @@
         if (p.launch[i].grid) q.queue = res.counters + i;
         return q;
     };
+    const RenderLauncher deferring = res.defer ? shape->render[kVariantDefer] : nullptr;
+    if (res.defer && !deferring) return false;
     const auto issue = [&](const RenderArgs& q, int i, hipStream_t s) {
+        if (deferring && (p.tail || !p.launch[i].split)) {
+            RenderArgs d = q;
+            d.defer = res.defer;
+            deferring(d, nc, nf, three_pass, p.launch[i].split, p.launch[i].ray_first, p.launch[i].rays, s);
+            return;
+        }
         launch(q, nc, nf, three_pass, p.launch[i].split, p.launch[i].ray_first, p.launch[i].rays, s);
     };
     if (p.n_launches == 1) {
diff --git a/nerf-workspaces-explorer_amd/csrc/nwe_mfma_defer.h b/nerf-workspaces-explorer_amd/csrc/nwe_mfma_defer.h
--- /dev/null
+++ b/nerf-workspaces-explorer_amd/csrc/nwe_mfma_defer.h
@@ -0,0 +1,131 @@
+#pragma once
+#include "nwe_mfma_eval.h"
+
+namespace nwe {
+
+template <int D, int SKIP>
+constexpr bool colour_defer_built(int form) { return colour_skip_built<D, SKIP>(form); }
+
+constexpr int kDeferSlots = 64;
+constexpr int kDeferVoteOff = 0, kDeferWOff = 16, kDeferOwnerOff = kDeferWOff + kWaves * kDeferSlots * 4,
+              kDeferBatchOff = kDeferOwnerOff + kWaves * kDeferSlots * 4, kDeferLds = kDeferBatchOff + kWaves * kRaysPerWave * 16;
+constexpr int kDeferHeadBytes = 256;
+
+template <int W, int D, int SKIP>
+struct ColourStart {
+    using S = Shape<W, D>;
+    static constexpr int CHUNK = D * S::NT;
+    static constexpr int TILE = S::NT * 2 * S::KG + (D - 1) * S::NT * 2 * S::KH + (SKIP >= 0 ? S::NT * 2 * S::KG : 0);
+};
+
+template <int W, int D, int SKIP, bool X3, class WalkerT>
+__device__ __forceinline__ void trunk_eval(WalkerT& wk, Frags& F, int lane, float inv_scale, h8* Ghi, h8* Glo, const float* dot_tab,
+                                           h8* Bhi, h8* Blo, Pend& P1, float& sig, bool stream_view) {
+    using S = Shape<W, D>;
+    static_assert(colour_defer_built<D, SKIP>(kFormFolded), "the deferring kernels: shapes of colour_defer_built only");
+    h8 Ahi[S::KH], Alo[S::KH];
+    Pend P0;
+    constexpr int NPAIR = D / 2;
+    constexpr int SKIP_PAIR = SKIP < 0 ? -1 : SKIP / 2;
+    constexpr int PAIRS = NPAIR - 1;
+    static_assert(SKIP_PAIR != NPAIR - 1, "density_only_built: the last trunk layer takes no gamma(x) k-steps");
+    layer<S::NT, 0, S::KG, X3, false, S::N_H, true>(wk, F, lane, false, SKIP_PAIR == 0, nullptr, nullptr, Ghi, Glo, Ahi, Alo, P0, P1,
+                                                    inv_scale, 0.f, 0.f);
+    auto pair_body = [&](bool use_g, bool skip_next) __attribute__((always_inline)) {
+        layer<S::NT, S::KG, S::KH, X3, true, S::N_H, false>(wk, F, lane, use_g, false, Ghi, Glo, Ahi, Alo, Bhi, Blo, P0, P1, inv_scale,
+                                                            0.f, 0.f);
+        layer<S::NT, 0, S::KH, X3, true, S::N_H, false>(wk, F, lane, false, skip_next, nullptr, nullptr, Bhi, Blo, Ahi, Alo, P0, P1,
+                                                        inv_scale, 0.f, 0.f, -1);
+    };
+    if constexpr (kPeelSkip && SKIP_PAIR >= 0 && SKIP_PAIR < PAIRS) {
+#pragma unroll 1
+        for (int pair = 0; pair < SKIP_PAIR; ++pair) pair_body(false, pair + 1 == SKIP_PAIR);
+        pair_body(true, false);
+#pragma unroll 1
+        for (int pair = SKIP_PAIR + 1; pair < PAIRS; ++pair) pair_body(false, false);
+    } else {
+#pragma unroll 1
+        for (int pair = 0; pair < PAIRS; ++pair) pair_body(pair == SKIP_PAIR, pair + 1 == SKIP_PAIR);
+    }
+    sig = 0.f;
+    if (stream_view) {
+        layer<S::NT, 0, S::KH, X3, true, S::N_V, false, true>(wk, F, lane, false, false, nullptr, nullptr, Ahi, Alo, Bhi, Blo, P0, P1,
+                                                              inv_scale, 0.f, 0.f, -1, dot_tab, &sig);
+    } else {
+        layer<S::NT, 0, S::KH, X3, true, 0, false, true, 0, false>(wk, F, lane, false, false, nullptr, nullptr, Ahi, Alo, Bhi, Blo, P0, P1,
+                                                                   inv_scale, 0.f, 0.f, -1, dot_tab, &sig);
+    }
+}
+
+template <int W, int D, bool X3>
+__device__ __forceinline__ void finish_trunk(const Pend& P1, float inv_scale, h8* Bhi, h8* Blo) {
+    constexpr int L = 2 * Shape<W, D>::NT - 2;
+    float keep = 0.f;
+#pragma unroll
+    for (int e = 0; e < 16; ++e) finish_elem<X3>(P1, e, inv_scale, 0.f, keep, Bhi[L], Blo[L], Bhi[L + 1], Blo[L + 1]);
+}
+
+template <int W, int D, int SKIP, bool X3, class WalkerT>
+__device__ __forceinline__ void colour_prime(WalkerT& wk, const uint8_t* stream, const float* bias) {
+    using S = Shape<W, D>;
+    using CS = ColourStart<W, D, SKIP>;
+    asm volatile("" : "+s"(stream));
+    wk.start(stream, bias);
+    wk.next_tile = CS::TILE; wk.chunk = CS::CHUNK;
+    wk.begin(S::N_V, 0, 0);
+    static_for<0, S::N_V>([&](auto ic) __attribute__((always_inline)) { wk.piece(decltype(ic)::value, S::N_V >= kLongPieces ? S::N_V - 2 : -1); });
+    constexpr int N1 = ViewDma<W, D, X3>::nb(0);
+    wk.begin(N1, 1, 1);
+    static_for<0, (N1 < PD ? N1 : PD)>([&](auto ic) __attribute__((always_inline)) { wk.piece(decltype(ic)::value); });
+}
+
+template <bool X3, class WalkerT>
+__device__ __forceinline__ void colour_first_frags(WalkerT& wk, int lane, Frags& F) {
+#pragma unroll
+    for (int k = 0; k < PD; ++k) {
+        F.hi[k] = *reinterpret_cast<const h8*>(wk.cur() + lane * 16 + (2 * k) * kTileBytes);
+        if (X3) F.lo[k] = *reinterpret_cast<const h8*>(wk.cur() + lane * 16 + (2 * k + 1) * kTileBytes);
+    }
+}
+template <int W, int D, bool X3, class WalkerT>
+__device__ __forceinline__ void colour_eval(WalkerT& wk, Frags& F, int lane, float inv_scale, h8* Bhi, h8* Blo, const char* gd_col,
+                                            float& o_r, float& o_g, float& o_b) {
+    using S = Shape<W, D>;
+    static_assert((S::NTV * (S::KH + S::KD)) % (PD + 1) == 0, "the view tiles must restore the ring phase");
+    h8 GDhi[S::KD], GDlo[S::KD];
+#pragma unroll
+    for (int k = 0; k < S::KD; ++k) {
+        GDhi[k] = *reinterpret_cast<const h8*>(gd_col + (2 * k) * kTileBytes);
+        if (X3) GDlo[k] = *reinterpret_cast<const h8*>(gd_col + (2 * k + 1) * kTileBytes);
+    }
+    h8 Ahi[S::KV], Alo[S::KV];
+    Pend P0, P1;
+    constexpr int LV = 2 * S::NTV - 2;
+    view_tiles<0, W, D, X3, true>(wk, F, lane, Bhi, Blo, GDhi, GDlo, Ahi, Alo, P0, P1, inv_scale);
+    tile_mma<TileCfg<KSteps<0, S::KV>, X3, Chunks<0, 0, false>, kPend | kFeeds>>(wk, F, lane, P1, P0, inv_scale, 0.f, Ahi, Alo, Ahi, Alo, LV);
+    o_r = pend_value(P1, 0, inv_scale);
+    o_g = pend_value(P1, 1, inv_scale);
+    o_b = pend_value(P1, 2, inv_scale);
+}
+
+__device__ __forceinline__ float defer_weight(Composite& c, float raw_s, float z, float z_next, bool last, float dnorm) {
+    float dist = last ? 1e10f : __fsub_rn(z_next, z);
+    dist = __fmul_rn(dist, dnorm);
+    const float sig = __builtin_elementwise_maximum(__fadd_rn(raw_s, 0.f), 0.f);
+    const float alpha = __fsub_rn(1.f, expf(-__fmul_rn(sig, dist)));
+    const float w = __fmul_rn(alpha, (float)c.t_run);
+    c.t_run *= (double)__fadd_rn(__fsub_rn(1.f, alpha), 1e-10f);
+    c.depth = __fadd_rn(c.depth, __fmul_rn(w, z));
+    c.acc = __fadd_rn(c.acc, w);
+    return w;
+}
+__device__ __forceinline__ float defer_product(float w, float raw) { return __fmul_rn(w, __fdiv_rn(1.f, __fadd_rn(1.f, expf(-raw)))); }
+
+template <int W, int D, bool X3, class WalkerT>
+__device__ __forceinline__ void colour_pass(WalkerT& wk) {
+    using S = Shape<W, D>;
+    view_pass<0, W, D, X3>(wk);
+    tile_pass<TileCfg<KSteps<0, S::KV>, X3, Chunks<0, 0, false>, kNoEpi>>(wk);
+}
+
+}
diff --git a/nerf-workspaces-explorer_amd/csrc/nwe_mfma_defer_loop.h b/nerf-workspaces-explorer_amd/csrc/nwe_mfma_defer_loop.h
--- /dev/null
+++ b/nerf-workspaces-explorer_amd/csrc/nwe_mfma_defer_loop.h
@@ -0,0 +1,115 @@
+            float z_cur, z_next = 0.f;
+            {
+                const Ray ray = fresh_ray();
+                if (pass == 0) z_cur = fs.cd.z(ray, 0);
+                else { fs.prepare(ray); z_cur = fs.next(ray); }
+            }
+            const bool fine = pass == 1;
+            char* const dl = smem + SM::TOTAL;
+            int* const votes = reinterpret_cast<int*>(dl + kDeferVoteOff);
+            float* const ring_w = reinterpret_cast<float*>(dl + kDeferWOff) + wave * kDeferSlots;
+            int* const ring_o = reinterpret_cast<int*>(dl + kDeferOwnerOff) + wave * kDeferSlots;
+            float4* const batch = reinterpret_cast<float4*>(dl + kDeferBatchOff) + wave * kRaysPerWave;
+            constexpr int kStep = kDeferSlots * 32;
+            char* const ring = defer + kDeferHeadBytes + ((size_t)item * kWaves + wave) * (size_t)(2 * S::KH * kStep) + half * 16;
+            const int col = lane & 31;
+            int pending = 0, head = 0;
+            unsigned long long c_flush = 0, c_mfma = 0, c_mem = 0, c_place = 0;
+            for (int s = 0;; ++s) {
+                const bool walking = s < Stot;
+                if (!walking && !fine) break;
+                h8 Bhi[S::KH], Blo[S::KH];
+                Pend P1;
+                Frags F;
+                unsigned dense = 0;
+                float w = 0.f;
+                if (walking) {
+                    NWE_PRIME_STREAM();
+                    const Ray ray = fresh_ray();
+                    if (s + 1 < Stot) z_next = pass == 0 ? fs.cd.z(ray, s + 1) : fs.next(ray);
+                    float sig;
+                    NWE_EVAL_TRUNK(z_cur, sig, fine);
+                    drain_dot<typename ViewDma<W, D, X3>::Plan0, X3>(P1, net.inv_scale, dot_tab + (S::NT - 1) * 32 + 4 * half, sig);
+                    const float rs = __fadd_rn(__fadd_rn(sig, __shfl_xor(sig, 32, 64)), dot_tab[S::NT * 32]);
+                    w = defer_weight(comp, rs, z_cur, z_next, s + 1 == Stot, ray.dnorm);
+                    if (!fine) fs.wc[s * kRaysPerWave] = w;
+                    z_cur = z_next;
+                    if (!fine) continue;
+                    const int allow = *skip_word;
+                    dense = (unsigned)__ballot(!gone && !(allow != 0 && rs <= 0.f && rs >= -FLT_MAX));
+                    if (dense) finish_trunk<W, D, X3>(P1, net.inv_scale, Bhi, Blo);
+                }
+                const int cnt = __popc(dense);
+                if (lane == 0) votes[wave] = pending + cnt;
+                wk.template sync<false>();
+                const int v0 = votes[0], v1 = votes[1], v2 = votes[2], v3 = votes[3];
+                const int v01 = v0 > v1 ? v0 : v1, v23 = v2 > v3 ? v2 : v3;
+                const int most = __builtin_amdgcn_readfirstlane(v01 > v23 ? v01 : v23);
+                const bool flush = walking ? most >= kRaysPerWave : most > 0;
+                if (!walking && !flush) break;
+                const bool in_place = flush && pending == 0 && cnt > 0;
+                const bool mine = (dense >> col) & 1;
+                if (cnt > 0 && !in_place) {
+                    const int slot = (head + pending + __popc(dense & ((1u << col) - 1u))) & (kDeferSlots - 1);
+                    if (mine) {
+                        char* const p = ring + slot * 32;
+#pragma unroll
+                        for (int k = 0; k < S::KH; ++k) {
+                            *reinterpret_cast<h8*>(p + (2 * k) * kStep) = Bhi[k];
+                            if (X3) *reinterpret_cast<h8*>(p + (2 * k + 1) * kStep) = Blo[k];
+                        }
+                        if (half == 0) { ring_w[slot] = w; ring_o[slot] = col; }
+                    }
+                    pending += cnt;
+                }
+                if (!flush) continue;
+                if (!walking) colour_prime<W, D, SKIP, X3>(wk, net.stream, bias);
+                if (wave == 0) ++c_flush;
+                const int take = in_place ? kRaysPerWave : (pending < kRaysPerWave ? pending : kRaysPerWave);
+                if (take == 0) {
+                    if (!walking) wk.template sync<false>();
+                    colour_pass<W, D, X3>(wk);
+                    continue;
+                }
+                ++c_mfma;
+                const int slot = (head + col) & (kDeferSlots - 1);
+                int owner = col;
+                float wj = w;
+                if (!in_place) {
+                    asm volatile("s_waitcnt vmcnt(0) lgkmcnt(0)" ::: "memory");
+                    const char* const p = ring + slot * 32;
+#pragma unroll
+                    for (int k = 0; k < S::KH; ++k) {
+                        Bhi[k] = *reinterpret_cast<const h8*>(p + (2 * k) * kStep);
+                        if (X3) Blo[k] = *reinterpret_cast<const h8*>(p + (2 * k + 1) * kStep);
+                    }
+                    owner = col < take ? ring_o[slot] : col;
+                    wj = ring_w[slot];
+                }
+                if (!walking) {
+                    wk.template sync<false>();
+                    colour_first_frags<X3>(wk, lane, F);
+                }
+                float o_r, o_g, o_b;
+                colour_eval<W, D, X3>(wk, F, lane, net.inv_scale, Bhi, Blo, gd_lds + (owner - col) * 16, o_r, o_g, o_b);
+                const float pr = defer_product(wj, o_r), pg = defer_product(wj, o_g), pb = defer_product(wj, o_b);
+                if (in_place) {
+                    if (mine) { comp.r = __fadd_rn(comp.r, pr); comp.g = __fadd_rn(comp.g, pg); comp.b = __fadd_rn(comp.b, pb); }
+                    c_place += cnt;
+                    continue;
+                }
+                if (half == 0) batch[col] = make_float4(pr, pg, pb, __int_as_float(owner));
+                asm volatile("s_waitcnt lgkmcnt(0)" ::: "memory");
+                for (int j = 0; j < take; ++j) {
+                    const float4 e = batch[j];
+                    if (__float_as_int(e.w) == col) { comp.r = __fadd_rn(comp.r, e.x); comp.g = __fadd_rn(comp.g, e.y); comp.b = __fadd_rn(comp.b, e.z); }
+                }
+                asm volatile("s_waitcnt lgkmcnt(0)" ::: "memory");
+                head = (head + take) & (kDeferSlots - 1);
+                pending -= take;
+                c_mem += take;
+            }
+            if (fine) {
+                const unsigned long long mine_c = lane == 0 ? c_flush : (lane == 1 ? c_mfma : (lane == 2 ? c_mem : c_place));
+                if (lane < 4 && mine_c) atomicAdd(reinterpret_cast<unsigned long long*>(defer) + lane, mine_c);
+            }
diff --git a/nerf-workspaces-explorer_amd/csrc/nwe_mfma_render.h b/nerf-workspaces-explorer_amd/csrc/nwe_mfma_render.h
--- a/nerf-workspaces-explorer_amd/csrc/nwe_mfma_render.h
+++ b/nerf-workspaces-explorer_amd/csrc/nwe_mfma_render.h
@@ -1,4 +1,5 @@
 #pragma once
+#include "nwe_mfma_defer.h"
 #include "nwe_mfma_eval.h"
 
 namespace nwe {
@@ -65,6 +66,17 @@
         NWE_STAMP(st_mlp += __builtin_amdgcn_s_memtime() - t2;)                                                                    \
     }
 
+#define NWE_EVAL_TRUNK(Z, SIG, STREAM_VIEW)                                                                                     \
+    {                                                                                                              \
+        float px, py, pz;                                                                                          \
+        point_at(ray, Z, px, py, pz);                                                                              \
+        h8 Ghi[S::KG], Glo[S::KG];                                                                                 \
+        encode<5, S::KG, X3>(__fdiv_rn(px, 10.f), __fdiv_rn(py, 10.f), __fdiv_rn(pz, 10.f), half, Ghi, Glo);       \
+        wk.template sync<false>();                                                                                 \
+        colour_first_frags<X3>(wk, lane, F);     \
+        trunk_eval<W, D, SKIP, X3>(wk, F, lane, net.inv_scale, Ghi, Glo, dot_tab, Bhi, Blo, P1, SIG, STREAM_VIEW); \
+    }
+
 constexpr int kVoteBytes = 2 * kWaves * 4;
 
 template <int W, int D, int SKIP, bool X3, bool SPLIT, int FORM, bool LEAN, bool TERM = false, bool SHARE = false>
@@ -183,8 +195,96 @@
 #include "nwe_mfma_render_item.h"
 #undef NWE_ITEM_OCC
 }
+
+template <int W, int D, int SKIP, bool X3, int FORM>
+__global__ void __launch_bounds__(256) render_mfma_defer_kernel(RenderArgs a_in, NetMfma nc, NetMfma nf) {
+    static_assert(colour_defer_built<D, SKIP>(FORM), "deferred colour: the shapes that have the hollow path");
+    constexpr bool LEAN = true, TERM = false, SHARE = false, SPLIT = false;
+    RenderArgs a = a_in;
+    char* const defer = a_in.defer;
+    a.out.raw_coarse = a.out.raw_fine = a.out.z_fine = a.out.weights_coarse = nullptr;
+    a.out.disp = a.out.z_std = a.out.rgb_coarse = a.out.depth_coarse = a.out.acc_coarse = a.out.disp_coarse = nullptr;
+    a.out.sample_cond = a.out.sample_amp = a.out.sample_switch = a.out.feat_map = nullptr;
+    a.z_fine_in = a.raw_in_c = a.raw_in_f = a.w_in = a.t_rand = a.noise_c = a.noise_f = a.u_rand = nullptr;
+    a.stamps = nullptr; a.rays = nullptr;
+    using S = Shape<W, D>;
+    using SM = Smem<W, D, SPLIT>;
+    static_assert(SM::TOTAL + kDeferLds <= 160 * 1024, "LDS budget");
+    __shared__ __attribute__((aligned(16))) char smem[SM::TOTAL + kDeferLds];
+    unsigned item = blockIdx.x;
+    if (a.queue) {
+        unsigned* s_item = reinterpret_cast<unsigned*>(smem);
+        if (threadIdx.x == 0) *s_item = atomicAdd(a.queue, 1u);
+        __syncthreads();
+        const unsigned ticket = *s_item;
+        if (ticket >= a.queue_items) return;
+        item = __builtin_amdgcn_readfirstlane(ticket);
+    }
+#define NWE_ITEM_DEFER
+#include "nwe_mfma_render_item.h"
+#undef NWE_ITEM_DEFER
+}
+
+template <int W, int D, int SKIP, bool X3, int FORM>
+__global__ void __launch_bounds__(256) render_mfma_tail_defer_kernel(RenderArgs a_in, NetMfma nc, NetMfma nf) {
+    static_assert(colour_defer_built<D, SKIP>(FORM), "deferred colour: the shapes that have the hollow path");
+    constexpr bool LEAN = true, TERM = false, SHARE = false;
+    RenderArgs a = a_in;
+    unsigned* const tail = a.tail;
+    char* const defer = a_in.defer;
+    const bool second = a.share == kTailSecond;
+    a.w_in = nullptr; a.share = kShareOff;
+    a.out.raw_coarse = a.out.raw_fine = a.out.z_fine = a.out.weights_coarse = nullptr;
+    a.out.disp = a.out.z_std = a.out.rgb_coarse = a.out.depth_coarse = a.out.acc_coarse = a.out.disp_coarse = nullptr;
+    a.out.sample_cond = a.out.sample_amp = a.out.sample_switch = a.out.feat_map = nullptr;
+    a.z_fine_in = a.raw_in_c = a.raw_in_f = a.t_rand = a.noise_c = a.noise_f = a.u_rand = nullptr;
+    a.stamps = nullptr; a.rays = nullptr;
+    using SP = Smem<W, D, false>;
+    using SS = Smem<W, D, true>;
+    static_assert(SP::TOTAL + kDeferLds <= 160 * 1024, "LDS budget");
+    __shared__ __attribute__((aligned(16))) char smem[SP::TOTAL + kDeferLds > SS::TOTAL ? SP::TOTAL + kDeferLds : SS::TOTAL];
+    const int64_t split_first = second ? a.ray_first : a.ray_first + (int64_t)a.queue_items * (kWaves * kRaysPerWave);
+    unsigned* s_item = reinterpret_cast<unsigned*>(smem);
+    if (threadIdx.x == 0) {
+        unsigned t;
+        if (!second) {
+            t = atomicAdd(a.queue, 1u);
+            if (t >= a.queue_items) {
+                const unsigned items1 = (unsigned)((a.n_rays - split_first + kRaysPerWave - 1) / kRaysPerWave);
+                const unsigned s = atomicAdd(tail, 1u);
+                t = s < items1 ? kTailSplit | s : kTailNone;
+            }
+        } else {
+            t = a.queue ? atomicAdd(a.queue, 1u) : blockIdx.x;
+            const unsigned n = a.queue ? a.queue_items : gridDim.x;
+            t = t < n && t >= *tail ? kTailSplit | t : kTailNone;
+            if (t != kTailNone) atomicAdd(tail + 1, 1u);
+        }
+        *s_item = t;
+    }
+    __syncthreads();
+    const unsigned ticket = *s_item;
+    if (ticket == kTailNone) return;
+    const unsigned t = __builtin_amdgcn_readfirstlane(ticket);
+    using S = Shape<W, D>;
+    if (t & kTailSplit) {
+        constexpr bool SPLIT = true;
+        using SM = SS;
+        const unsigned item = t & ~kTailSplit;
+        a.ray_first = split_first;
+#include "nwe_mfma_render_item.h"
+    } else {
+        constexpr bool SPLIT = false;
+        using SM = SP;
+        const unsigned item = t;
+#define NWE_ITEM_DEFER
+#include "nwe_mfma_render_item.h"
+#undef NWE_ITEM_DEFER
+    }
+}
 #undef NWE_PRIME_STREAM
 #undef NWE_EVAL_POINT
+#undef NWE_EVAL_TRUNK
 
 #ifdef NWE_STAMPS
 constexpr bool kTailLean = false;
@@ -202,7 +302,7 @@
         if (rays <= 0) return;
         a.ray_first = ray_first;
         const unsigned items = mfma_workgroups(rays, split);
-        const bool queued = (VARIANT == kVariantPlain || VARIANT == kVariantTail) && a.queue;
+        const bool queued = (VARIANT == kVariantPlain || VARIANT == kVariantTail || VARIANT == kVariantDefer) && a.queue;
         if (queued) a.queue_items = items;
         const unsigned grid = queued ? queue_grid(items) : items;
         RenderKernel kernel;
@@ -217,6 +317,14 @@
             const RenderKernel kernels[2] = {render_mfma_tail_kernel<W, D, SKIP, true, FORM, kTailLean>,
                                              render_mfma_tail_kernel<W, D, SKIP, false, FORM, kTailLean>};
             kernel = kernels[three_pass ? 0 : 1];
+        } else if constexpr (VARIANT == kVariantDefer) {
+            if constexpr (colour_defer_built<D, SKIP>(FORM)) {
+                const RenderKernel kernels[4] = {render_mfma_defer_kernel<W, D, SKIP, true, FORM>, render_mfma_defer_kernel<W, D, SKIP, false, FORM>,
+                                                 render_mfma_tail_defer_kernel<W, D, SKIP, true, FORM>, render_mfma_tail_defer_kernel<W, D, SKIP, false, FORM>};
+                kernel = kernels[(a.tail ? 2 : 0) + (three_pass ? 0 : 1)];
+            } else {
+                return;
+            }
         } else if constexpr (VARIANT == kVariantOcc) {
 #define NWE_KERNEL(X3_, SPLIT_) render_mfma_occ_kernel<W, D, SKIP, X3_, SPLIT_, FORM>
             const RenderKernel kernels[4] = {NWE_KERNEL(true, true), NWE_KERNEL(true, false), NWE_KERNEL(false, true), NWE_KERNEL(false, false)};
diff --git a/nerf-workspaces-explorer_amd/csrc/nwe_mfma_render_item.h b/nerf-workspaces-explorer_amd/csrc/nwe_mfma_render_item.h
--- a/nerf-workspaces-explorer_amd/csrc/nwe_mfma_render_item.h
+++ b/nerf-workspaces-explorer_amd/csrc/nwe_mfma_render_item.h
@@ -242,6 +242,9 @@
                 }
             }
         } else {
+#ifdef NWE_ITEM_DEFER
+#include "nwe_mfma_defer_loop.h"
+#else
             float z_cur, z_next = 0.f;
             {
                 const Ray ray = fresh_ray();
@@ -332,6 +335,7 @@
                     if (lane == 0 && mine) atomicAdd(a.evals, mine * (unsigned long long)((ni > 0 ? ns : 0) + s_end));
                 }
             }
+#endif
         }
         if (live) {
             flags |= store_ray(a.out, ridx, comp, pass == 1, a.white_bkgd != 0) & (density_only ? ~(uint32_t)NWE_FLAG_RGB_COARSE : ~0u);
diff --git a/nerf-workspaces-explorer_amd/csrc/nwe_plan.cpp b/nerf-workspaces-explorer_amd/csrc/nwe_plan.cpp
--- a/nerf-workspaces-explorer_amd/csrc/nwe_plan.cpp
+++ b/nerf-workspaces-explorer_amd/csrc/nwe_plan.cpp
@@ -114,6 +114,11 @@
     p.may_queue = m.pass.queued();
     p.need_side = p.may_queue && c.backfill;
     p.blocks = c.packet_blocks && lean && plain_only && m.pass.ok && m.pass.variant == kVariantPlain && packet_blocks_fit(c.rows, c.width);
+    const unsigned packet_items = m.pass.plan == 1 ? 0 : m.pass.launch[0].items;
+    p.defer = c.colour_defer != 0 && c.colour_skip == 1 && lean && plain_only && c.n_importance > 0 && m.pass.ok &&
+              m.pass.variant == kVariantPlain && packet_items > 0 && c.built[1][kVariantDefer] && c.built[0][kVariantDefer] &&
+              defer_scratch_bytes(packet_items, c.net_width) <= kDeferScratchCap;
+    p.defer_bytes = p.defer ? defer_scratch_bytes(packet_items, c.net_width) : 0;
     return p;
 }
 
diff --git a/nerf-workspaces-explorer_amd/csrc/nwe_plan.h b/nerf-workspaces-explorer_amd/csrc/nwe_plan.h
--- a/nerf-workspaces-explorer_amd/csrc/nwe_plan.h
+++ b/nerf-workspaces-explorer_amd/csrc/nwe_plan.h
@@ -18,10 +18,18 @@
 
 constexpr int kShareOff = 0, kShareProducer = 1, kShareConsumer = 2;
 
-enum Variant { kVariantPlain, kVariantTerm, kVariantShare, kVariantOcc, kVariantTail, kVariants };
+enum Variant { kVariantPlain, kVariantTerm, kVariantShare, kVariantOcc, kVariantTail, kVariantDefer, kVariants };
 
 constexpr bool variant_built(int variant, int form) {
-    return variant == kVariantTerm || variant == kVariantShare || variant == kVariantOcc ? form != kFormReference : true;
+    return variant == kVariantDefer ? form == kFormFolded
+                                    : (variant == kVariantTerm || variant == kVariantShare || variant == kVariantOcc ? form != kFormReference : true);
+}
+
+constexpr int kDeferRingSlots = 64;
+constexpr int64_t kDeferScratchHead = 256;
+constexpr int64_t kDeferScratchCap = (int64_t)2 << 30;
+inline int64_t defer_scratch_bytes(unsigned items, int width) {
+    return kDeferScratchHead + (int64_t)items * kWaves * kDeferRingSlots * (4 * (int64_t)width);
 }
 
 inline unsigned queue_grid(unsigned n) { return (unsigned)(((uint64_t)n + (n + 3) / 4 + 7) / 8 * 8); }
@@ -89,6 +97,9 @@
     bool backfill = true, tail = true;
     int rows = 0, width = 0;
     bool packet_blocks = false;
+    int colour_skip = 1;
+    int colour_defer = 1;
+    int net_width = 0;
 };
 
 struct StagePlan {
@@ -112,6 +123,8 @@
     bool baked = false;
     int share_k = 1;
     bool blocks = false;
+    bool defer = false;
+    int64_t defer_bytes = 0;
     int64_t table_elems = 0;
     bool coarse_flags = false;
     int64_t evals_full = 0, evals_run = 0, share_rays = 0;
diff --git a/nerf-workspaces-explorer_amd/renderer.py b/nerf-workspaces-explorer_amd/renderer.py
--- a/nerf-workspaces-explorer_amd/renderer.py
+++ b/nerf-workspaces-explorer_amd/renderer.py
@@ -286,6 +286,24 @@
     def debug_get_colour_skip(self) -> int:
         return int(self._lib.nwe_debug_get_colour_skip(self._ctx))
 
+    def debug_set_colour_defer(self, mode: int) -> None:
+        self._check(self._lib.nwe_debug_set_colour_defer(self._ctx, int(mode)), "nwe_debug_set_colour_defer")
+
+    def debug_get_colour_defer(self) -> int:
+        return int(self._lib.nwe_debug_get_colour_defer(self._ctx))
+
+    def debug_last_defer(self) -> tuple:
+        out = (C.c_uint64 * 4)()
+        self._check(self._lib.nwe_debug_last_defer(self._ctx, out), "nwe_debug_last_defer")
+        return tuple(int(v) for v in out)
+
+    def debug_last_plan_defer(self) -> tuple:
+        n = C.c_int64(0)
+        return int(self._lib.nwe_debug_last_plan_defer(self._ctx, C.byref(n))), int(n.value)
+
+    def debug_defer_scratch_bytes(self) -> int:
+        return int(self._lib.nwe_debug_defer_scratch_bytes(self._ctx))
+
     def debug_set_packet_blocks(self, on: bool) -> None:
         self._check(self._lib.nwe_debug_set_packet_blocks(self._ctx, 1 if on else 0), "nwe_debug_set_packet_blocks")
 
```
